# Xharlie/pointnerf

Measured on AMD Instinct MI355X. Metric: rays/sec (render+bwd) NeRF-synth lego 800^2, K=8, 128 samp/ray, higher is better.
Workload: dtype f32 in / out / accumulate; forward GEMM operands as 2 x f16 planes (22-bit) on the f16 MFMA, 3 products per multiply-add; input-gradient GEMMs: f16 leading product + e4m3 cross terms (csrc/mixq.h), 2 product equivalents; weight-gradient GEMM operands as one f16 plane each

## Files before the change

include/pnerf.h:

```cpp
#ifndef PNERF_H
#define PNERF_H
#include <stddef.h>
#include <stdint.h>

#ifdef __cplusplus
extern "C" {
#endif

#define PNERF_E_INVAL   (-1)
#define PNERF_E_WS      (-2)
#define PNERF_E_LAUNCH  (-3)
#define PNERF_E_UNSUP   (-4)

#define PNERF_MAX_K 16

typedef struct pnerf_grid_params {
    float ranges[6];
    float vsize[3];
    int32_t vdim[3];
    int32_t kernel_size[3];
    int32_t query_size[3];
    int32_t P;
    int32_t max_o;
    float radius;
} pnerf_grid_params;

enum { PNERF_GI_N_IN_GRID = 0, PNERF_GI_N_OCC = 1, PNERF_GI_MAX_CNT = 2, PNERF_GI_CELL0 = 3,
       PNERF_GI_FIRST_IDX = 4, PNERF_GI_OSTART_OFF = 5 , PNERF_GI_LEN = 8 };

int pnerf_version(void);
const char *pnerf_arch(void);

size_t pnerf_grid_workspace_bytes(const pnerf_grid_params *gp, int n_points);
int pnerf_grid_build(const pnerf_grid_params *gp, const float *d_xyz, int n_points,
                     void *d_grid_ws, size_t ws_bytes, void *stream);
int pnerf_grid_info(const void *d_grid_ws, int32_t *host_info, void *stream);
int pnerf_points_minmax(const float *d_xyz, int64_t n_points, float *d_out6, void *stream);

size_t pnerf_query_workspace_bytes(int R, int SR);
int pnerf_query(const pnerf_grid_params *gp, const void *d_grid_ws,
                const float *d_raypos,
                const float *campos3_host, const float *d_raydir, const float *d_mid,
                float near_depth, float far_depth, float jitter, uint64_t seed,
                int R, int D, int SR, int K,
                float *d_sample_loc, int32_t *d_sample_pidx, int32_t *d_sample_nn,
                int32_t *d_ray_hit, int32_t *d_valid_list, int32_t *d_counters,
                void *d_query_ws, size_t ws_bytes, void *stream);

int pnerf_gather_rows(const float *d_src, int n_src, int width, const int32_t *d_idx, int64_t n_idx,
                      float *d_dst, void *stream);
int pnerf_scatter_add_rows(const float *d_grad_rows, const int32_t *d_idx, int64_t n_idx, int width,
                           float *d_grad_src, int n_src, void *stream);

int pnerf_zero_one_blocks(int64_t n_idx);
int pnerf_zero_one_forward(const float *d_conf, int n_points, const int32_t *d_idx, int64_t n_idx, float eps,
                           float *d_partial, void *stream);
int pnerf_zero_one_backward(const float *d_conf, int n_points, const int32_t *d_idx, int64_t n_idx, float eps,
                            const float *d_gscale, float *d_grad_conf, void *stream);
int pnerf_zero_one_forward_rays(const float *d_conf, int n_points, const int32_t *d_idx, const int32_t *d_ray_hit, int R, int slots_per_ray, float eps,
                                float *d_partial, void *stream);
int pnerf_zero_one_backward_rays(const float *d_conf, int n_points, const int32_t *d_idx, const int32_t *d_ray_hit, int R, int slots_per_ray, float eps,
                                 const float *d_gscale, float *d_grad_conf, void *stream);
int pnerf_color_loss_blocks(int R);
int pnerf_color_loss_forward_rays(const float *d_ray_color, const float *d_gt, const int32_t *d_ray_hit, int R, float *d_partial, void *stream);
int pnerf_color_loss_backward_rays(const float *d_ray_color, const float *d_gt, const int32_t *d_ray_hit, int R, const float *d_gscale,
                                   float *d_grad_ray_color, void *stream);


#define PNERF_MLP_NTENSORS 18
int pnerf_mlp_layout(int feat_dim, int64_t *offsets );
size_t pnerf_mlp_packed_bytes(void);
int pnerf_mlp_pack(const float *d_params, void *d_packed, void *stream);

typedef struct pnerf_camera {
    float campos[3];
    float camrot[9];
    float rw2c[9];
    float vsize_z;
    int32_t raydist_mode_unit;
    float bg[3];
    int32_t has_bg;
} pnerf_camera;

typedef struct pnerf_points {
    const float *xyz;
    const float *embedding;
    const float *conf;
    const float *dir;
    const float *color;
    int32_t n, feat_dim;
    const float *frames;
} pnerf_points;

typedef struct pnerf_point_grads {
    float *embedding, *conf, *dir, *color;
    void *ready_event;
    const float *zero_one_gscale;
    float zero_one_eps;
    float *xyz;
} pnerf_point_grads;

typedef struct pnerf_step {
    const float *raydir;
    const float *sample_loc;
    const int32_t *sample_pidx;
    const int32_t *sample_nn;
    const int32_t *valid_list;
    const int32_t *counters;
    const float *xyz_pers;
    const float *loc_pers;
    const float *params;
    const void *packed_mlp;
    int32_t R, SR, K;
    int64_t n_valid_max;
} pnerf_step;

size_t pnerf_agg_saved_bytes(int64_t n_valid_samples, int K);
size_t pnerf_agg_workspace_bytes(int64_t n_valid_max, int K);
size_t pnerf_render_backward_workspace_bytes(int R, int SR);

int pnerf_render_forward(const pnerf_camera *cam, const pnerf_points *pts, const pnerf_step *step,
                         float *d_decoded, float *d_weight, float *d_ray_color, float *d_opacity,
                         float *d_bg_trans, float *d_blend_w,
                         void *d_saved, void *d_ws, size_t ws_bytes, void *stream);

size_t pnerf_render_cut_workspace_bytes(int R, int SR);
int pnerf_render_forward_cut(const pnerf_camera *cam, const pnerf_points *pts, const pnerf_step *step, float cutoff, int stage_samples,
                             float *d_decoded, float *d_weight, float *d_ray_color, float *d_opacity, float *d_bg_trans, float *d_blend_w,
                             int32_t *d_cut_counters, void *d_ws, size_t ws_bytes, void *d_cut_ws, size_t cut_ws_bytes, void *stream);
int pnerf_cut_stage(const pnerf_camera *cam, const float *d_sample_loc, const int32_t *d_sample_nn, const int32_t *d_ray_hit,
                    const float *d_decoded, int R, int SR, float cutoff, int stage_samples, int stage,
                    float *d_trans, float *d_depth_max, int32_t *d_alive, int32_t *d_flags, int32_t *d_list, int32_t *d_counters,
                    void *d_ws, size_t ws_bytes, void *stream);

int pnerf_set_inference_products(int n);

int pnerf_set_wgrad_planes(int n);
int pnerf_set_cross_terms(int bits);
int pnerf_set_cross_terms_where(int mask);
int pnerf_get_arithmetic(int32_t out[4]);

int pnerf_render_backward(const pnerf_camera *cam, const pnerf_points *pts, const pnerf_step *step,
                          const float *d_decoded, const float *d_weight, const float *d_grad_ray_color,
                          void *d_saved, float *d_grad_params, const pnerf_point_grads *pg,
                          void *d_ws, size_t ws_bytes, void *stream);


size_t pnerf_compact_workspace_bytes(int64_t n);
int pnerf_touched_flags(const int32_t *d_pidx, int64_t n, int32_t n_points, int32_t *d_flags, void *stream);
int pnerf_compact_valid(const int32_t *d_nn, int64_t n, int32_t *d_list, int32_t *d_counters, void *d_ws, size_t ws_bytes, void *stream);

int pnerf_agg_forward(const pnerf_camera *cam, const pnerf_points *pts, const pnerf_step *step, float *d_decoded, float *d_weight,
                      void *d_saved, void *d_ws, size_t ws_bytes, void *stream);
int pnerf_agg_backward(const pnerf_camera *cam, const pnerf_points *pts, const pnerf_step *step,
                       const float *d_decoded, const float *d_weight, const float *d_grad_decoded,
                       void *d_saved, float *d_grad_params, const pnerf_point_grads *pg, void *d_ws, size_t ws_bytes, void *stream);

int pnerf_raymarch_forward(const float *d_ray_dist, const uint8_t *d_ray_valid, const float *d_features, const float *bg3_host,
                           int R, int SR, float *d_ray_color, float *d_opacity, float *d_acc_trans, float *d_blend_w,
                           float *d_bg_trans, void *stream);
int pnerf_raymarch_backward(const float *d_ray_dist, const uint8_t *d_ray_valid, const float *d_features, const float *bg3_host,
                            int R, int SR, const float *d_grad_ray_color, float *d_grad_features, void *stream);

int pnerf_adam_step(float *d_param, const float *d_grad, float *d_exp_avg, float *d_exp_avg_sq, int64_t n,
                    double lr, double beta1, double beta2, double eps, int64_t step, void *stream);
typedef struct pnerf_adam_tensor {
    float *param; const float *grad; float *exp_avg; float *exp_avg_sq;
    int64_t n; double lr; int64_t step;
} pnerf_adam_tensor;
int pnerf_adam_step_multi(const pnerf_adam_tensor *tensors, int count, double beta1, double beta2, double eps, void *stream);

size_t pnerf_voxel_downsample_workspace_bytes(int64_t n_points, int rx, int ry, int rz);
int pnerf_voxel_downsample(const float *d_xyz, int64_t n_points, const float *space_min3_host, const float *vox_size3_host,
                           int rx, int ry, int rz, float *d_centroid, int32_t *d_grid_idx, int64_t *d_min_idx, int32_t *d_counts,
                           void *d_ws, size_t ws_bytes, void *stream);

#define PNERF_EX2D_MAX_VIEWS 8
#define PNERF_EX2D_MAX_MAPS 32
typedef struct pnerf_view_desc {
    float c2w[16];
    float w2c[16];
    float intrinsic[9];
    int32_t has_w2c;
} pnerf_view_desc;
typedef struct pnerf_map_desc {
    const float *d_map;
    int32_t view;
    int32_t C, H, W;
    int32_t out_col;
    int32_t is_color;
    int32_t first_of_view;
} pnerf_map_desc;
size_t pnerf_extract_2d_workspace_bytes(int64_t n_points, int n_views, int HD, int WD, int depth_occ);
int pnerf_extract_2d(const float *d_cam_xyz, int64_t n_points, const pnerf_view_desc *views, int n_views, const pnerf_map_desc *maps,
                     int n_maps, int HD, int WD, int depth_occ, float tolerate, float *d_feats, int feat_cols, float *d_colors,
                     int color_cols, uint8_t *d_mask, void *d_ws, size_t ws_bytes, void *stream);
int pnerf_point_dirs(const float *d_cam_xyz, int64_t n_points, const float *cam_pos_cam_host, int n_views, const float *rot1_host9,
                     const float *rot2_host9, float *d_dirs, void *stream);

size_t pnerf_image_metrics_workspace_bytes(int H, int W, int win);
int pnerf_image_metrics(const float *d_img, const float *d_gt, int H, int W, int win, double data_range, int quantize8, double *d_out4,
                        void *d_ws, size_t ws_bytes, void *stream);

int pnerf_probe_rays(const pnerf_points *pts, const float *d_opacity, const float *d_weight, const float *d_sample_loc,
                     const int32_t *d_sample_pidx, const int32_t *d_ray_hit, int R, int SR, int K, float *d_max_opacity, float *d_loc3,
                     float *d_far_dist, float *d_avg_color3, float *d_avg_dir3, float *d_avg_conf, float *d_avg_emb32, void *stream);
int pnerf_probe_hole_mask(const int8_t *d_ray_mask, const float *d_max_opacity, const float *d_far_dist, const float *d_raycolor,
                          const float *d_gt, const uint8_t *d_edge, const float *bg3_host, int H, int W, float opacity_thresh,
                          float far_thresh, int32_t *d_flags, void *stream);

int pnerf_ray_geometry(const pnerf_camera *cam, const float *d_sample_loc, const int32_t *d_sample_nn, const int32_t *d_ray_hit,
                       const float *d_opacity, const float *d_blend_w, int R, int SR, float *d_acc, float *d_depth_sum, float *d_depth,
                       float *d_median_depth, int32_t *d_median_slot, void *stream);
int pnerf_geometry_canvas(const int32_t *d_pixel_idx, const int8_t *d_ray_mask, const float *d_depth, const float *d_median_depth,
                          const float *d_acc, int n_rays, int H, int W, float *d_depth_canvas, float *d_median_canvas, float *d_acc_canvas,
                          int32_t *d_flag, void *stream);

int pnerf_debug_mfma_f16(const void *d_a, const void *d_b, float *d_out, void *stream);
int pnerf_debug_mix_gemm(const float *d_w, int K, const float *d_x, void *d_img, float *d_out, void *stream);
int pnerf_debug_mfma_rate(int mode, int iters, float *d_scratch, double *flop_out, void *stream);
int pnerf_debug_uniform(uint64_t seed, uint64_t first, int64_t n, float *d_out, void *stream);
int pnerf_debug_split(const float *d_x, int64_t n, void *d_h, void *d_m, int sat, void *stream);
int pnerf_debug_pe(const float *d_x, int64_t n, int nfreq, float *d_out, void *stream);

int pnerf_prof_enable(int on);
int pnerf_prof_kernel_count(void);
const char *pnerf_prof_kernel_name(int id);
int pnerf_prof_collect(double *total_ms, int64_t *launches);

#ifdef __cplusplus
}
#endif
#endif
```

pointnerf_amd/_lib.py:

```python
import ctypes
import os

import torch

_HERE = os.path.dirname(os.path.abspath(__file__))
LIB_PATH = os.path.join(_HERE, "libpnerf_hip.so")

c_int, c_i64, c_f32, c_void_p, c_size_t = ctypes.c_int, ctypes.c_int64, ctypes.c_float, ctypes.c_void_p, ctypes.c_size_t

ABI_VERSION = 1003
PNERF_MAX_K = 16
GI_N_IN_GRID, GI_N_OCC, GI_MAX_CNT, GI_CELL0, GI_FIRST_IDX, GI_LEN = 0, 1, 2, 3, 4, 8
MLP_NTENSORS = 18

ERRORS = {-1: "PNERF_E_INVAL (bad argument)", -2: "PNERF_E_WS (workspace too small)",
          -3: "PNERF_E_LAUNCH (HIP launch/runtime error)", -4: "PNERF_E_UNSUP (unsupported configuration)"}


class GridParams(ctypes.Structure):
    _fields_ = [("ranges", c_f32 * 6), ("vsize", c_f32 * 3), ("vdim", ctypes.c_int32 * 3),
                ("kernel_size", ctypes.c_int32 * 3), ("query_size", ctypes.c_int32 * 3),
                ("P", ctypes.c_int32), ("max_o", ctypes.c_int32), ("radius", c_f32)]


class Camera(ctypes.Structure):
    _fields_ = [("campos", c_f32 * 3), ("camrot", c_f32 * 9), ("rw2c", c_f32 * 9), ("vsize_z", c_f32),
                ("raydist_mode_unit", ctypes.c_int32), ("bg", c_f32 * 3), ("has_bg", ctypes.c_int32)]


class Points(ctypes.Structure):
    _fields_ = [("xyz", c_void_p), ("embedding", c_void_p), ("conf", c_void_p), ("dir", c_void_p),
                ("color", c_void_p), ("n", ctypes.c_int32), ("feat_dim", ctypes.c_int32), ("frames", c_void_p)]


class AdamTensor(ctypes.Structure):
    _fields_ = [("param", c_void_p), ("grad", c_void_p), ("exp_avg", c_void_p), ("exp_avg_sq", c_void_p),
                ("n", ctypes.c_int64), ("lr", ctypes.c_double), ("step", ctypes.c_int64)]


class ViewDesc(ctypes.Structure):
    _fields_ = [("c2w", c_f32 * 16), ("w2c", c_f32 * 16), ("intrinsic", c_f32 * 9), ("has_w2c", ctypes.c_int32)]


class MapDesc(ctypes.Structure):
    _fields_ = [("d_map", c_void_p), ("view", ctypes.c_int32), ("C", ctypes.c_int32), ("H", ctypes.c_int32), ("W", ctypes.c_int32),
                ("out_col", ctypes.c_int32), ("is_color", ctypes.c_int32), ("first_of_view", ctypes.c_int32)]


class PointGrads(ctypes.Structure):
    _fields_ = [("embedding", c_void_p), ("conf", c_void_p), ("dir", c_void_p), ("color", c_void_p), ("ready_event", c_void_p),
                ("zero_one_gscale", c_void_p), ("zero_one_eps", c_f32), ("xyz", c_void_p)]


class Step(ctypes.Structure):
    _fields_ = [("raydir", c_void_p), ("sample_loc", c_void_p), ("sample_pidx", c_void_p), ("sample_nn", c_void_p), ("valid_list", c_void_p),
                ("counters", c_void_p), ("xyz_pers", c_void_p), ("loc_pers", c_void_p), ("params", c_void_p), ("packed_mlp", c_void_p),
                ("R", ctypes.c_int32), ("SR", ctypes.c_int32), ("K", ctypes.c_int32), ("n_valid_max", ctypes.c_int64)]


_STEP_ARGS = [ctypes.POINTER(Camera), ctypes.POINTER(Points), ctypes.POINTER(Step)]
PROTOTYPES = {
    "pnerf_version": (c_int, []),
    "pnerf_arch": (ctypes.c_char_p, []),
    "pnerf_grid_workspace_bytes": (c_size_t, [ctypes.POINTER(GridParams), c_int]),
    "pnerf_grid_build": (c_int, [ctypes.POINTER(GridParams), c_void_p, c_int, c_void_p, c_size_t, c_void_p]),
    "pnerf_grid_info": (c_int, [c_void_p, ctypes.POINTER(ctypes.c_int32), c_void_p]),
    "pnerf_points_minmax": (c_int, [c_void_p, c_i64, c_void_p, c_void_p]),
    "pnerf_query_workspace_bytes": (c_size_t, [c_int, c_int]),
    "pnerf_query": (c_int, [ctypes.POINTER(GridParams), c_void_p, c_void_p, ctypes.POINTER(c_f32), c_void_p, c_void_p,
                            c_f32, c_f32, c_f32, ctypes.c_uint64, c_int, c_int, c_int, c_int,
                            c_void_p, c_void_p, c_void_p, c_void_p, c_void_p, c_void_p, c_void_p, c_size_t, c_void_p]),
    "pnerf_gather_rows": (c_int, [c_void_p, c_int, c_int, c_void_p, c_i64, c_void_p, c_void_p]),
    "pnerf_scatter_add_rows": (c_int, [c_void_p, c_void_p, c_i64, c_int, c_void_p, c_int, c_void_p]),
    "pnerf_zero_one_blocks": (c_int, [c_i64]),
    "pnerf_zero_one_forward": (c_int, [c_void_p, c_int, c_void_p, c_i64, c_f32, c_void_p, c_void_p]),
    "pnerf_zero_one_backward": (c_int, [c_void_p, c_int, c_void_p, c_i64, c_f32, c_void_p, c_void_p, c_void_p]),
    "pnerf_color_loss_blocks": (c_int, [c_int]),
    "pnerf_color_loss_forward_rays": (c_int, [c_void_p, c_void_p, c_void_p, c_int, c_void_p, c_void_p]),
    "pnerf_color_loss_backward_rays": (c_int, [c_void_p, c_void_p, c_void_p, c_int, c_void_p, c_void_p, c_void_p]),
    "pnerf_zero_one_forward_rays": (c_int, [c_void_p, c_int, c_void_p, c_void_p, c_int, c_int, c_f32, c_void_p, c_void_p]),
    "pnerf_zero_one_backward_rays": (c_int, [c_void_p, c_int, c_void_p, c_void_p, c_int, c_int, c_f32, c_void_p, c_void_p, c_void_p]),
    "pnerf_voxel_downsample_workspace_bytes": (c_size_t, [c_i64, c_int, c_int, c_int]),
    "pnerf_voxel_downsample": (c_int, [c_void_p, c_i64, c_void_p, c_void_p, c_int, c_int, c_int, c_void_p, c_void_p, c_void_p, c_void_p, c_void_p, c_size_t, c_void_p]),
    "pnerf_extract_2d_workspace_bytes": (c_size_t, [c_i64, c_int, c_int, c_int, c_int]),
    "pnerf_extract_2d": (c_int, [c_void_p, c_i64, ctypes.POINTER(ViewDesc), c_int, ctypes.POINTER(MapDesc), c_int, c_int, c_int, c_int, c_f32,
                                 c_void_p, c_int, c_void_p, c_int, c_void_p, c_void_p, c_size_t, c_void_p]),
    "pnerf_point_dirs": (c_int, [c_void_p, c_i64, ctypes.POINTER(c_f32), c_int, ctypes.POINTER(c_f32), ctypes.POINTER(c_f32), c_void_p, c_void_p]),
    "pnerf_adam_step": (c_int, [c_void_p, c_void_p, c_void_p, c_void_p, c_i64, ctypes.c_double, ctypes.c_double, ctypes.c_double, ctypes.c_double, c_i64, c_void_p]),
    "pnerf_adam_step_multi": (c_int, [ctypes.POINTER(AdamTensor), c_int, ctypes.c_double, ctypes.c_double, ctypes.c_double, c_void_p]),
    "pnerf_mlp_layout": (c_int, [c_int, ctypes.POINTER(c_i64)]),
    "pnerf_mlp_packed_bytes": (c_size_t, []),
    "pnerf_mlp_pack": (c_int, [c_void_p, c_void_p, c_void_p]),
    "pnerf_agg_saved_bytes": (c_size_t, [c_i64, c_int]),
    "pnerf_agg_workspace_bytes": (c_size_t, [c_i64, c_int]),
    "pnerf_render_backward_workspace_bytes": (c_size_t, [c_int, c_int]),
    "pnerf_render_forward": (c_int, _STEP_ARGS + [c_void_p, c_void_p, c_void_p, c_void_p, c_void_p, c_void_p, c_void_p, c_void_p, c_size_t, c_void_p]),
    "pnerf_render_cut_workspace_bytes": (c_size_t, [c_int, c_int]),
    "pnerf_render_forward_cut": (c_int, _STEP_ARGS + [c_f32, c_int, c_void_p, c_void_p, c_void_p, c_void_p, c_void_p, c_void_p, c_void_p,
                                                      c_void_p, c_size_t, c_void_p, c_size_t, c_void_p]),
    "pnerf_cut_stage": (c_int, [ctypes.POINTER(Camera), c_void_p, c_void_p, c_void_p, c_void_p, c_int, c_int, c_f32, c_int, c_int,
                                c_void_p, c_void_p, c_void_p, c_void_p, c_void_p, c_void_p, c_void_p, c_size_t, c_void_p]),
    "pnerf_set_inference_products": (c_int, [c_int]),
    "pnerf_set_wgrad_planes": (c_int, [c_int]),
    "pnerf_set_cross_terms": (c_int, [c_int]),
    "pnerf_set_cross_terms_where": (c_int, [c_int]),
    "pnerf_get_arithmetic": (c_int, [ctypes.POINTER(ctypes.c_int32)]),
    "pnerf_compact_workspace_bytes": (c_size_t, [c_i64]),
    "pnerf_touched_flags": (c_int, [c_void_p, c_i64, c_int, c_void_p, c_void_p]),
    "pnerf_compact_valid": (c_int, [c_void_p, c_i64, c_void_p, c_void_p, c_void_p, c_size_t, c_void_p]),
    "pnerf_agg_forward": (c_int, _STEP_ARGS + [c_void_p, c_void_p, c_void_p, c_void_p, c_size_t, c_void_p]),
    "pnerf_agg_backward": (c_int, _STEP_ARGS + [c_void_p, c_void_p, c_void_p, c_void_p, c_void_p, ctypes.POINTER(PointGrads), c_void_p, c_size_t, c_void_p]),
    "pnerf_raymarch_forward": (c_int, [c_void_p, c_void_p, c_void_p, ctypes.POINTER(c_f32), c_int, c_int,
                                       c_void_p, c_void_p, c_void_p, c_void_p, c_void_p, c_void_p]),
    "pnerf_raymarch_backward": (c_int, [c_void_p, c_void_p, c_void_p, ctypes.POINTER(c_f32), c_int, c_int,
                                        c_void_p, c_void_p, c_void_p]),
    "pnerf_image_metrics_workspace_bytes": (c_size_t, [c_int, c_int, c_int]),
    "pnerf_image_metrics": (c_int, [c_void_p, c_void_p, c_int, c_int, c_int, ctypes.c_double, c_int, c_void_p, c_void_p, c_size_t, c_void_p]),
    "pnerf_probe_rays": (c_int, [ctypes.POINTER(Points), c_void_p, c_void_p, c_void_p, c_void_p, c_void_p, c_int, c_int, c_int,
                                 c_void_p, c_void_p, c_void_p, c_void_p, c_void_p, c_void_p, c_void_p, c_void_p]),
    "pnerf_probe_hole_mask": (c_int, [c_void_p, c_void_p, c_void_p, c_void_p, c_void_p, c_void_p, ctypes.POINTER(c_f32), c_int, c_int,
                                      c_f32, c_f32, c_void_p, c_void_p]),
    "pnerf_ray_geometry": (c_int, [ctypes.POINTER(Camera), c_void_p, c_void_p, c_void_p, c_void_p, c_void_p, c_int, c_int,
                                   c_void_p, c_void_p, c_void_p, c_void_p, c_void_p, c_void_p]),
    "pnerf_geometry_canvas": (c_int, [c_void_p, c_void_p, c_void_p, c_void_p, c_void_p, c_int, c_int, c_int,
                                      c_void_p, c_void_p, c_void_p, c_void_p, c_void_p]),
    "pnerf_debug_mfma_f16": (c_int, [c_void_p, c_void_p, c_void_p, c_void_p]),
    "pnerf_debug_mix_gemm": (c_int, [c_void_p, c_int, c_void_p, c_void_p, c_void_p, c_void_p]),
    "pnerf_debug_mfma_rate": (c_int, [c_int, c_int, c_void_p, ctypes.POINTER(ctypes.c_double), c_void_p]),
    "pnerf_debug_uniform": (c_int, [ctypes.c_uint64, ctypes.c_uint64, c_i64, c_void_p, c_void_p]),
    "pnerf_debug_split": (c_int, [c_void_p, c_i64, c_void_p, c_void_p, c_int, c_void_p]),
    "pnerf_debug_pe": (c_int, [c_void_p, c_i64, c_int, c_void_p, c_void_p]),
    "pnerf_prof_enable": (c_int, [c_int]),
    "pnerf_prof_kernel_count": (c_int, []),
    "pnerf_prof_kernel_name": (ctypes.c_char_p, [c_int]),
    "pnerf_prof_collect": (c_int, [ctypes.POINTER(ctypes.c_double), ctypes.POINTER(c_i64)]),
    "pnerf_render_backward": (c_int, _STEP_ARGS + [c_void_p, c_void_p, c_void_p, c_void_p, c_void_p, ctypes.POINTER(PointGrads), c_void_p, c_size_t, c_void_p]),
}

_lib = None


def bind(handle, path):
    for name, (res, args) in PROTOTYPES.items():
        try:
            fn = getattr(handle, name)
        except AttributeError as e:
            raise RuntimeError("pointnerf_amd: %s lacks symbol %s (stale build?)" % (os.path.basename(path), name)) from e
        fn.restype, fn.argtypes = res, args
    got = handle.pnerf_version()
    if got != ABI_VERSION:
        raise RuntimeError("pointnerf_amd: %s reports pnerf_version() %d, this binding is written for %d (stale build?)"
                           % (os.path.basename(path), got, ABI_VERSION))
    return handle


def lib():
    global _lib
    if _lib is None:
        if not os.path.exists(LIB_PATH):
            raise RuntimeError(
                "pointnerf_amd: %s not found. Build it with `python -c 'import __graft_entry__ as g; g.build()'` "
                "(hipcc --offload-arch=gfx950). There is no CPU/PyTorch fallback for this path." % LIB_PATH)
        _lib = bind(ctypes.CDLL(LIB_PATH), LIB_PATH)
    return _lib


def check(rc, what):
    if rc != 0:
        raise RuntimeError("pointnerf_amd: %s failed: %s" % (what, ERRORS.get(rc, rc)))
```

pointnerf_amd/csrc/aggregate.hip:

```cpp
#include "mixq.h"
#include <stdlib.h>

extern "C" int pnerf_mlp_layout(int feat_dim, int64_t *offsets) {
    if (feat_dim != PN_F || !offsets) return PNERF_E_UNSUP;
    const int64_t o[PNERF_MLP_NTENSORS + 1] = {PO_W1, PO_B1, PO_W2, PO_B2, PO_W3, PO_B3, PO_W4, PO_B4, PO_W5, PO_B5,
                                               PO_WC1, PO_BC1, PO_WC2, PO_BC2, PO_WC3, PO_BC3, PO_WC4, PO_BC4, PO_TOTAL};
    for (int i = 0; i <= PNERF_MLP_NTENSORS; ++i) offsets[i] = o[i];
    return 0;
}
extern "C" size_t pnerf_mlp_packed_bytes(void) { return (size_t)PKX_END; }

namespace {
struct PackHDesc { int src, ld, trans, Mreal, Kreal, NCH, MB, dst; };
struct PackHTable { PackHDesc d[15]; };
__global__ __launch_bounds__(256) void k_pack_h(PackHTable t, const float *__restrict__ params, char *__restrict__ packed) {
    const PackHDesc d = t.d[blockIdx.y];
    const int total = d.NCH * d.MB * 64;
    for (int e = blockIdx.x * 256 + threadIdx.x; e < total; e += gridDim.x * 256) {
        const int lane = e & 63, mb = (e >> 6) % d.MB, c = (e >> 6) / d.MB;
        const int m = 32 * mb + (lane & 31), k0 = 16 * c + 8 * (lane >> 5);
        unsigned h[4], lo[4];
#pragma unroll
        for (int j = 0; j < 4; ++j) {
            float v[2];
// ... 105 lines not shown
        {PO_W2, PN_H, 1, PN_H, PN_H, 16, 8, PKH_D2},
        {PO_W1, PN_IN1, 1, 32 * PN_MB_D1, PN_H, 16, PN_MB_D1, PKH_D1},
        {PO_WC1, PN_INC, 0, PN_HC, PN_INC, 18, 4, PKH_FC1},
        {PO_WC2, PN_HC, 0, PN_HC, PN_HC, 8, 4, PKH_FC2},
        {PO_WC3, PN_HC, 0, PN_HC, PN_HC, 8, 4, PKH_FC3},
        {PO_WC3, PN_HC, 1, PN_HC, PN_HC, 8, 4, PKH_DC3},
        {PO_WC2, PN_HC, 1, PN_HC, PN_HC, 8, 4, PKH_DC2},
        {PO_WC1, PN_INC, 1, PN_H, PN_HC, 8, 8, PKH_DC1},
        {PO_W1 + 32 * PN_MB_D1, PN_IN1, 1, PN_IN1 - 32 * PN_MB_D1, PN_H, 16, 2, PKH_D1T},
    }};
    PnProfScope prof(PNK_PACK, (hipStream_t)stream);
    hipLaunchKernelGGL(k_pack_h, dim3(40, 15), dim3(256), 0, (hipStream_t)stream, th, d_params, (char *)d_packed);
    PackMTable tm = {{
        {PO_W1, PN_IN1, 0, PN_H, PN_IN1, 2, 8, PKM_F1},
        {PO_W2, PN_H, 0, PN_H, PN_H, 0, 8, PKM_F2},
        {PO_W3, PN_IN3, 0, PN_H, PN_IN3, 1, 8, PKM_F3},
        {PO_W4, PN_H, 0, PN_H, PN_H, 0, 8, PKM_F4},
        {PO_W4, PN_H, 1, PN_H, PN_H, 0, 8, PKM_D4},
        {PO_W3, PN_IN3, 1, PN_IN3, PN_H, 0, 9, PKM_D3},
        {PO_W2, PN_H, 1, PN_H, PN_H, 0, 8, PKM_D2},
        {PO_W1, PN_IN1, 1, 32 * PN_MB_D1, PN_H, 0, PN_MB_D1, PKM_D1},
        {PO_W1 + 32 * PN_MB_D1, PN_IN1, 1, PN_IN1 - 32 * PN_MB_D1, PN_H, 0, 2, PKM_D1T},
    }};
    hipLaunchKernelGGL(k_pack_mix, dim3(12, 9), dim3(256), 0, (hipStream_t)stream, tm, d_params, (char *)d_packed);
    PN_CHECK_LAUNCH();
    return 0;
}

namespace {
template <int NT>
__global__ __launch_bounds__(256) void k_debug_mix_gemm(const float *__restrict__ x, const char *__restrict__ img, float *__restrict__ out) {
    extern __shared__ __attribute__((aligned(16))) char smem_d[];
    pn_mode_saturate();
    constexpr int K = 256 + 16 * NT;
    char *X = smem_d;
    const int tid = threadIdx.x, lane = tid & 63, wave = __builtin_amdgcn_readfirstlane(tid >> 6);
    for (int e = tid; e < PN_TILE * (K / 4); e += 256) {
        const int row = e / (K / 4), col = 4 * (e % (K / 4));
        const float4 v = *reinterpret_cast<const float4 *>(x + row * K + col);
        if (col < 256) pn_xq_store4(X, row, col, v.x, v.y, v.z, v.w);
        else pn_xt_store4(X, row, col, v.x, v.y, v.z, v.w);
    }
    __syncthreads();
    f32x16 acc[2][2];
    pn_acc_zero(acc);
    pn_gemm_mix<PN_MIX_NS, NT, 8, 2>(X, img, 2 * wave, lane, acc);
#pragma unroll
    for (int fb = 0; fb < 2; ++fb)
#pragma unroll
        for (int rb = 0; rb < 2; ++rb)
#pragma unroll
            for (int g = 0; g < 4; ++g)
#pragma unroll
                for (int i = 0; i < 4; ++i) out[(32 * rb + (lane & 31)) * PN_H + pn_d_feat(2 * wave + fb, g, lane) + i] = acc[fb][rb][4 * g + i];
}
}

extern "C" int pnerf_debug_mix_gemm(const float *d_w, int K, const float *d_x, void *d_img, float *d_out, void *stream) {
    if (!d_w || !d_x || !d_img || !d_out || (K != 256 && K != 272 && K != 288)) return PNERF_E_INVAL;
    hipStream_t s = (hipStream_t)stream;
    const int NT = (K - 256) / 16;
    PackMTable tm = {{{0, K, 0, PN_H, K, NT, 8, 0}}};
    hipLaunchKernelGGL(k_pack_mix, dim3(12, 1), dim3(256), 0, s, tm, d_w, (char *)d_img);
    const void *fn = NT == 0 ? (const void *)k_debug_mix_gemm<0> : NT == 1 ? (const void *)k_debug_mix_gemm<1> : (const void *)k_debug_mix_gemm<2>;
    if (hipFuncSetAttribute(fn, hipFuncAttributeMaxDynamicSharedMemorySize, PN_XBYTES) != hipSuccess) return PNERF_E_LAUNCH;
    if (NT == 0) hipLaunchKernelGGL(k_debug_mix_gemm<0>, dim3(1), dim3(256), PN_XBYTES, s, d_x, (const char *)d_img, d_out);
    else if (NT == 1) hipLaunchKernelGGL(k_debug_mix_gemm<1>, dim3(1), dim3(256), PN_XBYTES, s, d_x, (const char *)d_img, d_out);
    else hipLaunchKernelGGL(k_debug_mix_gemm<2>, dim3(1), dim3(256), PN_XBYTES, s, d_x, (const char *)d_img, d_out);
    PN_CHECK_LAUNCH();
    return 0;
}

namespace {
__global__ __launch_bounds__(64) void k_debug_mfma_f16(const uint4 *__restrict__ a, const uint4 *__restrict__ b, float *__restrict__ d) {
    f32x16 acc;
#pragma unroll
    for (int r = 0; r < 16; ++r) acc[r] = 0.f;
    acc = __builtin_amdgcn_mfma_f32_32x32x16_f16(__builtin_bit_cast(pn_h8, a[threadIdx.x]), __builtin_bit_cast(pn_h8, b[threadIdx.x]), acc, 0, 0, 0);
#pragma unroll
    for (int r = 0; r < 16; ++r) d[threadIdx.x * 16 + r] = acc[r];
}
}
namespace {
__global__ __launch_bounds__(256) void k_debug_split(const float *__restrict__ x, long long n, unsigned *__restrict__ h, unsigned *__restrict__ m, int sat) {
    for (long long i = (long long)blockIdx.x * 256 + threadIdx.x; 2 * i < n; i += (long long)gridDim.x * 256) {
        unsigned hh, mm;
        if (sat) pn_split2_sat(x[2 * i], x[2 * i + 1], hh, mm);
        else pn_split2(x[2 * i], x[2 * i + 1], hh, mm);
        h[i] = hh; m[i] = mm;
    }
}
}
extern "C" int pnerf_debug_split(const float *d_x, int64_t n, void *d_h, void *d_m, int sat, void *stream) {
    if (!d_x || !d_h || !d_m || n < 0 || (n & 1)) return PNERF_E_INVAL;
    if (n == 0) return 0;
    hipLaunchKernelGGL(k_debug_split, dim3(64), dim3(256), 0, (hipStream_t)stream, d_x, (long long)n, (unsigned *)d_h, (unsigned *)d_m, sat);
    PN_CHECK_LAUNCH();
    return 0;
}

namespace {
template <int NF> __global__ __launch_bounds__(256) void k_debug_pe(const float *__restrict__ x, long long n, float *__restrict__ out) {
    for (long long i = (long long)blockIdx.x * 256 + threadIdx.x; i < n; i += (long long)gridDim.x * 256) {
        float s[NF], c[NF];
        pn_pe_octaves<NF>(x[i], s, c);
#pragma unroll
        for (int f = 0; f < NF; ++f) { out[(i * NF + f) * 2] = s[f]; out[(i * NF + f) * 2 + 1] = c[f]; }
    }
}
}
extern "C" int pnerf_debug_pe(const float *d_x, int64_t n, int nfreq, float *d_out, void *stream) {
    if (!d_x || !d_out || n < 0 || nfreq < 1 || nfreq > 5) return PNERF_E_INVAL;
    if (n == 0) return 0;
    hipStream_t s = (hipStream_t)stream;
    switch (nfreq) {
        case 1: hipLaunchKernelGGL(k_debug_pe<1>, dim3(64), dim3(256), 0, s, d_x, (long long)n, d_out); break;
        case 2: hipLaunchKernelGGL(k_debug_pe<2>, dim3(64), dim3(256), 0, s, d_x, (long long)n, d_out); break;
        case 3: hipLaunchKernelGGL(k_debug_pe<3>, dim3(64), dim3(256), 0, s, d_x, (long long)n, d_out); break;
        case 4: hipLaunchKernelGGL(k_debug_pe<4>, dim3(64), dim3(256), 0, s, d_x, (long long)n, d_out); break;
        default: hipLaunchKernelGGL(k_debug_pe<5>, dim3(64), dim3(256), 0, s, d_x, (long long)n, d_out); break;
    }
    PN_CHECK_LAUNCH();
    return 0;
}

extern "C" int pnerf_debug_mfma_f16(const void *d_a, const void *d_b, float *d_out, void *stream) {
    if (!d_a || !d_b || !d_out) return PNERF_E_INVAL;
    hipLaunchKernelGGL(k_debug_mfma_f16, dim3(1), dim3(64), 0, (hipStream_t)stream, (const uint4 *)d_a, (const uint4 *)d_b, d_out);
    PN_CHECK_LAUNCH();
    return 0;
}

size_t pn_saved_walk(void *base, long long n_valid, int K, PnSaved &s) {
    const int TS = pn_tile_samples(K);
    const long long tiles = (n_valid + TS - 1) / TS + 2 * PN_NCLS + 1;
    s.rows = tiles * PN_TILE;
    s.samples = ((tiles * TS + PN_CTILE - 1) / PN_CTILE + 1) * PN_CTILE;
    PnCarver cv(base);
    const size_t rg = (size_t)s.rows / 8, rgc = (size_t)s.samples / 8;
    auto planes = [&](uint4 *&x0, uint4 *&h2, uint4 *&h1, uint4 *&h3, uint4 *&dy1, uint4 *&dy2, uint4 *&dy3, uint4 *&dy4) {
        x0 = cv.take<uint4>(rg * PN_NF1); h2 = cv.take<uint4>(rg * PN_NF1);
        h1 = cv.take<uint4>(rg * PN_H); h3 = cv.take<uint4>(rg * PN_H);
        dy1 = cv.take<uint4>(rg * PN_H); dy2 = cv.take<uint4>(rg * PN_H);
        dy3 = cv.take<uint4>(rg * PN_H); dy4 = cv.take<uint4>(rg * PN_H);
    };
    auto cplanes = [&](uint4 *&xc, uint4 *&c1, uint4 *&c2, uint4 *&dc1, uint4 *&dc2, uint4 *&dc3) {
        xc = cv.take<uint4>(rgc * PN_NF1); c1 = cv.take<uint4>(rgc * PN_HC); c2 = cv.take<uint4>(rgc * PN_HC);
        dc1 = cv.take<uint4>(rgc * PN_HC); dc2 = cv.take<uint4>(rgc * PN_HC); dc3 = cv.take<uint4>(rgc * PN_HC);
    };
    planes(s.x0k, s.h2k, s.h1k, s.h3k, s.dy1k, s.dy2k, s.dy3k, s.dy4k);
    s.h4r = cv.take<uint4>((size_t)s.rows * 32 * 2);
    s.arow = cv.take<float>((size_t)s.rows); s.rmeta = cv.take<int4>((size_t)s.rows);
    s.lmask = cv.take<unsigned>((size_t)tiles * 3 * 512);
    s.gscale = cv.take<unsigned>(4);
    s.fs = cv.take<float>((size_t)s.samples * PN_H); s.dfs = cv.take<float>((size_t)s.samples * PN_H);
    s.c3 = cv.take<float>((size_t)s.samples * PN_HC);
    cplanes(s.xck, s.c1k, s.c2k, s.dc1k, s.dc2k, s.dc3k);
    s.cmask = cv.take<unsigned>((size_t)s.samples / PN_CTILE * 2 * 256);
    s.wg2 = pn_arith().wgrad_planes == 2 ? 1 : 0;
    s.x0m = s.h1m = s.h2m = s.h3m = s.dy1m = s.dy2m = s.dy3m = s.dy4m = nullptr;
    s.xcm = s.c1m = s.c2m = s.dc1m = s.dc2m = s.dc3m = nullptr;
    if (s.wg2) {
        planes(s.x0m, s.h2m, s.h1m, s.h3m, s.dy1m, s.dy2m, s.dy3m, s.dy4m);
        cplanes(s.xcm, s.c1m, s.c2m, s.dc1m, s.dc2m, s.dc3m);
    }
    pn_cls_walk(cv, s);
    return cv.off;
}
void pn_cls_walk(PnCarver &cv, PnSaved &s) {
    s.cls_list = cv.take<int>((size_t)s.samples);
    s.cls_info = cv.take<int>(PN_CI_WORDS);
    s.cls_tmp = cv.take<int>((size_t)2 * s.samples + pn_scan_scratch_ints(s.samples) + 8);
}
size_t pn_saved_bytes(long long n_valid, int K) { PnSaved s; return pn_saved_walk(nullptr, n_valid, K, s); }
PnSaved pn_saved_carve(void *base, long long n_valid, int K) { PnSaved s; pn_saved_walk(base, n_valid, K, s); return s; }

extern "C" size_t pnerf_agg_saved_bytes(int64_t n_valid_samples, int K) {
    if (K <= 0 || K > PNERF_MAX_K || n_valid_samples < 0) return 0;
    return pn_saved_bytes(n_valid_samples, K);
}

namespace {
struct FwdArgs {
    pnerf_camera cam;
    const float *xyz, *emb, *conf, *dir, *color;
    const float *params;
    const float4 *packed;
    const float *raydir, *sample_loc;
    const float *xyz_pers, *loc_pers;
    const int *pidx, *valid_list, *counters;
    const int *cls_list, *cls_info;
    int cls, Kstride;
    int save_x0;
    int R, SR, K, TS;
    long long cap_samples;
    float *decoded, *weight;
    PnSaved sv;
};
struct FwdArgsF : FwdArgs { const float *frames; };
template <bool FRAMES> struct FwdArgsOf { using type = FwdArgs; };
template <> struct FwdArgsOf<true> { using type = FwdArgsF; };

namespace {
struct ClsArgs { const int *valid_list, *counters, *pidx; int K, n, ncls; int kc[PN_NCLS], ts[PN_NCLS]; };

__global__ void k_cls_flags(ClsArgs c, int which, int *__restrict__ flags) {
    const int vs = blockIdx.x * blockDim.x + threadIdx.x;
    if (vs >= c.n) return;
    const int Ns = c.counters[0] < c.n ? c.counters[0] : c.n;
    int f = 0;
    if (vs < Ns) {
        const long long si = c.valid_list[vs];
        int hv = 0;
        for (int k = 0; k < c.K; ++k)
            if (c.pidx[si * c.K + k] >= 0) hv = k + 1;
        int cl = 0;
        for (int j = 1; j < c.ncls; ++j)
            if (hv <= c.kc[j]) cl = j;
        f = cl == which;
    }
    flags[vs] = f;
}

__global__ void k_cls_gather(ClsArgs c, int which, const int *__restrict__ pos, const int *__restrict__ count, int *__restrict__ cls_list,
                             int *__restrict__ info) {
    const int n = *count, base = info[PN_CI_VBASE + which];
    for (int i = blockIdx.x * blockDim.x + threadIdx.x; i < n; i += gridDim.x * blockDim.x) cls_list[base + i] = c.valid_list[pos[i]];
    if (blockIdx.x == 0 && threadIdx.x == 0) {
        const int tiles = (n + c.ts[which] - 1) / c.ts[which], tb = info[PN_CI_TBASE + which];
        info[PN_CI_COUNT + which] = n;
        if (which + 1 < PN_NCLS) { info[PN_CI_VBASE + which + 1] = base + n; info[PN_CI_TBASE + which + 1] = tb + tiles + 1; }
        info[PN_CI_TILES] = tb + tiles + 1;
    }
}

__global__ void k_cls_zero_gaps(PnSaved sv, int ncls, int save_x0) {
    const int c = blockIdx.y;
    if (c >= ncls) return;
    if ((blockIdx.x == 0 && !save_x0) || (blockIdx.x == 8 && save_x0)) return;
    const long long gap = (c + 1 < PN_NCLS ? sv.cls_info[PN_CI_TBASE + c + 1] : sv.cls_info[PN_CI_TILES]) - 1;
    uint4 *arrs[9] = {sv.x0k, sv.h2k, sv.h1k, sv.h3k, sv.dy1k, sv.dy2k, sv.dy3k, sv.dy4k, sv.x0k};
    uint4 *arrm[9] = {sv.x0m, sv.h2m, sv.h1m, sv.h3m, sv.dy1m, sv.dy2m, sv.dy3m, sv.dy4m, nullptr};
    const int which = blockIdx.x;
    const int nf = which == 8 ? 64 : which < 2 ? PN_NF1 : PN_H;
    uint4 *p = arrs[which] + gap * 8 * nf;
    for (int i = threadIdx.x; i < 8 * nf; i += blockDim.x) p[i] = make_uint4(0u, 0u, 0u, 0u);
    if (sv.wg2 && arrm[which]) {
        uint4 *pm = arrm[which] + gap * 8 * nf;
        for (int i = threadIdx.x; i < 8 * nf; i += blockDim.x) pm[i] = make_uint4(0u, 0u, 0u, 0u);
    }
}
}

}

int pn_class_slots(int K, int kc[PN_NCLS]) {
    if (K % 4 == 0) { kc[0] = K; kc[1] = K / 2; kc[2] = K / 4; return 3; }
    kc[0] = K; kc[1] = kc[2] = 0;
    return 1;
}

int pn_classify(const PnSaved &sv, const int32_t *d_valid_list, const int32_t *d_counters, const int32_t *d_pidx, int K, long long n_valid,
                bool train, bool save_x0, hipStream_t s) {
    ClsArgs c;
    c.valid_list = d_valid_list; c.counters = d_counters; c.pidx = d_pidx; c.K = K; c.n = (int)n_valid;
    c.ncls = pn_class_slots(K, c.kc);
    for (int j = 0; j < PN_NCLS; ++j) c.ts[j] = c.kc[j] > 0 ? pn_tile_samples(c.kc[j]) : 1;
    if (hipMemsetAsync(sv.cls_info, 0, PN_CI_WORDS * sizeof(int), s) != hipSuccess) return PNERF_E_LAUNCH;
    if (n_valid <= 0) return 0;
    int *flags = sv.cls_tmp, *pos = flags + n_valid, *cnt = pos + n_valid, *scratch = cnt + 8;
    PnProfScope prof(PNK_COMPACT, s);
    for (int j = 0; j < c.ncls; ++j) {
        hipLaunchKernelGGL(k_cls_flags, dim3(pn_cdiv(n_valid, 256)), dim3(256), 0, s, c, j, flags);
        int rc = pn_compact_gt0_i32(flags, n_valid, pos, cnt, scratch, s);
        if (rc) return rc;
        hipLaunchKernelGGL(k_cls_gather, dim3(256), dim3(256), 0, s, c, j, pos, cnt, sv.cls_list, sv.cls_info);
    }
    if (train) hipLaunchKernelGGL(k_cls_zero_gaps, dim3(9, c.ncls), dim3(256), 0, s, sv, c.ncls, save_x0 ? 1 : 0);
    PN_CHECK_LAUNCH();
    return 0;
}


namespace {

constexpr int FL_EX = PN_XBYTES, FL_W5 = FL_EX + PN_TILE * 8 * 4, FL_ROW = FL_W5 + PN_H * 4, FL_BYTES = FL_ROW + 4 * PN_TILE * 4;
static_assert(2 * FL_BYTES <= 160 * 1024, "two forward workgroups must fit the 160 KB LDS");

struct FGather {
    float4 e0, e1;
    float px, py, pz, lx, ly, lz, cf;
    float ppx, ppy, ppz, lpx, lpy, lpz;
    float dxv, dyv, dzv, cx, cy, cz, rx, ry, rz;
    float fx, fy, fz, gx, gy, gz;
};

__device__ __forceinline__ int f_sample_of(const FwdArgs &a, long long tile, int row, int Ns, unsigned kinv) {
    const int ls = pn_row_div(row, kinv);
    const long long vs = tile * a.TS + ls;
    return (ls < a.TS && vs < Ns) ? a.valid_list[vs] : -1;
}

template <bool PERS, bool FRAMES = false>
__device__ __forceinline__ void f_gather(const FwdArgs &a, FGather &G, int si_, int p_, int q, const float *frames = nullptr) {
    const int p = p_ > 0 ? p_ : 0, si = si_ > 0 ? si_ : 0;
    const float *ep = a.emb + (long long)p * PN_F + PN_EPT * q;
    G.e0 = *reinterpret_cast<const float4 *>(ep); G.e1 = *reinterpret_cast<const float4 *>(ep + 4);
    G.px = a.xyz[3 * p]; G.py = a.xyz[3 * p + 1]; G.pz = a.xyz[3 * p + 2];
    G.lx = a.sample_loc[(long long)si * 3]; G.ly = a.sample_loc[(long long)si * 3 + 1]; G.lz = a.sample_loc[(long long)si * 3 + 2];
    if (PERS) {
        G.ppx = a.xyz_pers[3 * p]; G.ppy = a.xyz_pers[3 * p + 1]; G.ppz = a.xyz_pers[3 * p + 2];
        G.lpx = a.loc_pers[(long long)si * 3]; G.lpy = a.loc_pers[(long long)si * 3 + 1]; G.lpz = a.loc_pers[(long long)si * 3 + 2];
    }
    G.cf = a.conf[p];
    if (FRAMES) {
        const int r = si / a.SR, fr = q < 3 ? q : 2;
        const int ps_ = a.pidx[(long long)si * a.Kstride], ps = ps_ > 0 ? ps_ : 0;
        const float *fp = frames + (long long)p * 9 + 3 * fr, *gp = frames + (long long)ps * 9 + 3 * fr;
        G.fx = fp[0]; G.fy = fp[1]; G.fz = fp[2];
        G.gx = gp[0]; G.gy = gp[1]; G.gz = gp[2];
        G.dxv = a.dir[3 * p]; G.dyv = a.dir[3 * p + 1]; G.dzv = a.dir[3 * p + 2];
        G.rx = a.raydir[3 * r]; G.ry = a.raydir[3 * r + 1]; G.rz = a.raydir[3 * r + 2];
        if (q == 0) { G.cx = a.color[3 * p]; G.cy = a.color[3 * p + 1]; G.cz = a.color[3 * p + 2]; }
    } else if (q == 0) {
        const int r = si / a.SR;
        G.dxv = a.dir[3 * p]; G.dyv = a.dir[3 * p + 1]; G.dzv = a.dir[3 * p + 2];
        G.cx = a.color[3 * p]; G.cy = a.color[3 * p + 1]; G.cz = a.color[3 * p + 2];
        G.rx = a.raydir[3 * r]; G.ry = a.raydir[3 * r + 1]; G.rz = a.raydir[3 * r + 2];
    }
}

template <bool PERS, bool MIX = false, bool FRAMES = false>
__device__ __forceinline__ void f_build(const FwdArgs &a, const FGather &G, char *X, float *exb, float *wraw, int *sidx, int si, int p, int row, int q) {
    const float dwx = G.px - G.lx, dwy = G.py - G.ly, dwz = G.pz - G.lz;
    float ppx, ppy, pcz, spx, spy, scz;
    if (PERS) {
        ppx = G.ppx; ppy = G.ppy; pcz = G.ppz; spx = G.lpx; spy = G.lpy; scz = G.lpz;
    } else {
        float pcx, pcy, scx, scy;
        if (FRAMES) {
            const float *M = a.cam.camrot;
            const float x = G.px - a.cam.campos[0], y = G.py - a.cam.campos[1], z = G.pz - a.cam.campos[2];
            const float u = G.lx - a.cam.campos[0], v = G.ly - a.cam.campos[1], w = G.lz - a.cam.campos[2];
            pcx = __builtin_fmaf(z, M[6], __builtin_fmaf(y, M[3], x * M[0]));
            pcy = __builtin_fmaf(z, M[7], __builtin_fmaf(y, M[4], x * M[1]));
            pcz = __builtin_fmaf(z, M[8], __builtin_fmaf(y, M[5], x * M[2]));
            scx = __builtin_fmaf(w, M[6], __builtin_fmaf(u, M[0], v * M[3]));
            scy = __builtin_fmaf(w, M[7], __builtin_fmaf(u, M[1], v * M[4]));
            scz = __builtin_fmaf(w, M[8], __builtin_fmaf(u, M[2], v * M[5]));
        } else {
        rot3(a.cam.camrot, G.px - a.cam.campos[0], G.py - a.cam.campos[1], G.pz - a.cam.campos[2], false, pcx, pcy, pcz);
        rot3(a.cam.camrot, G.lx - a.cam.campos[0], G.ly - a.cam.campos[1], G.lz - a.cam.campos[2], false, scx, scy, scz);
        }
        ppx = pcx / pcz; ppy = pcy / pcz; spx = scx / scz; spy = scy / scz;
    }
    float d0, d1, d2;
    if (FRAMES) d0 = d1 = d2 = dwx * G.fx + dwy * G.fy + dwz * G.fz;
    else rot3(a.cam.rw2c, dwx, dwy, dwz, true, d0, d1, d2);
    const float d3 = ppx * pcz - spx * scz, d4 = ppy * pcz - spy * scz, d5 = pcz - scz;
    const float da = q == 0 ? d0 : q == 1 ? d1 : q == 2 ? d2 : d3;
    const float db = q == 0 ? d4 : d5;
    const float e[8] = {G.e0.x, G.e0.y, G.e0.z, G.e0.w, G.e1.x, G.e1.y, G.e1.z, G.e1.w};
    if (MIX) {
        pn_xq_store4(X, row, PN_EPT * q, e[0], e[1], e[2], e[3]);
        pn_xq_store4(X, row, PN_EPT * q + 4, e[4], e[5], e[6], e[7]);
#pragma unroll
        for (int i = 0; i < 8; i += 2) {
            const int col = PN_F + (PN_EPT * q + i) * 6;
            float s0[3], c0[3], s1[3], c1[3];
            pn_pe_octaves<3>(e[i], s0, c0);
            pn_pe_octaves<3>(e[i + 1], s1, c1);
            pn_xq_store4(X, row, col, s0[0], c0[0], s0[1], c0[1]);
            pn_xq_store4(X, row, col + 4, s0[2], c0[2], s1[0], c1[0]);
            pn_xq_store4(X, row, col + 8, s1[1], c1[1], s1[2], c1[2]);
        }
    } else {
    pn_xt_store4(X, row, PN_EPT * q, e[0], e[1], e[2], e[3]); pn_xt_store4(X, row, PN_EPT * q + 4, e[4], e[5], e[6], e[7]);
#pragma unroll
    for (int i = 0; i < 8; ++i) {
        const int dd = PN_EPT * q + i;
        float s[3], c[3];
        pn_pe_octaves<3>(e[i], s, c);
        pn_xt_store2(X, row, PN_F + dd * 6, s[0], c[0]);
        pn_xt_store2(X, row, PN_F + dd * 6 + 2, s[1], c[1]);
        pn_xt_store2(X, row, PN_F + dd * 6 + 4, s[2], c[2]);
    }
    }
#pragma unroll
    for (int j = 0; j < 2; ++j) {
        const int comp = q + 4 * j;
        if (comp < 6) {
            float s[5], c[5];
            pn_pe_octaves<5>(j == 0 ? da : db, s, c);
#pragma unroll
            for (int f = 0; f < 5; ++f) {
                if (MIX) pn_xa_store2(X, row, PN_F * 7 + (comp * 5 + f) * 2, s[f], c[f]);
                else pn_xt_store2(X, row, PN_F * 7 + (comp * 5 + f) * 2, s[f], c[f]);
            }
        }
    }
    if (q == 3) pn_xt_store4(X, row, PN_ONES1, 1.f, 0.f, 0.f, 0.f);
    float fvx = 0.f, fvy = 0.f, fvz = 0.f, fqx = 0.f, fqy = 0.f, fqz = 0.f;
    if (FRAMES) {
        fvx = G.rx * G.gx + G.ry * G.gy + G.rz * G.gz;
        fqx = G.dxv * G.fx + G.dyv * G.fy + G.dzv * G.fz;
        fvy = __shfl_down(fvx, 1, 64); fvz = __shfl_down(fvx, 2, 64);
        fqy = __shfl_down(fqx, 1, 64); fqz = __shfl_down(fqx, 2, 64);
    }
    if (q == 0) {
        float vx, vy, vz, qx, qy, qz;
        if (FRAMES) { vx = fvx; vy = fvy; vz = fvz; qx = fqx; qy = fqy; qz = fqz; }
        else {
        rot3(a.cam.rw2c, G.rx, G.ry, G.rz, true, vx, vy, vz);
        rot3(a.cam.rw2c, G.dxv, G.dyv, G.dzv, true, qx, qy, qz);
        }
        float *ex = exb + row * 8;
        *reinterpret_cast<float4 *>(ex) = make_float4(G.cx, G.cy, G.cz, qx - vx);
        if (FRAMES) {
            *reinterpret_cast<float4 *>(ex + 4) = make_float4(qy - vy, qz - vz, __builtin_fmaf(qz, vz, __builtin_fmaf(qx, vx, qy * vy)), 1.f);
            wraw[row] = p >= 0 ? 1.0f / fmaxf(sqrtf(__builtin_fmaf(dwz, dwz, __builtin_fmaf(dwx, dwx, dwy * dwy))), 1e-6f) : 0.f;
        } else {
        *reinterpret_cast<float4 *>(ex + 4) = make_float4(qy - vy, qz - vz, qx * vx + qy * vy + qz * vz, 1.f);
        wraw[row] = p >= 0 ? 1.0f / fmaxf(sqrtf(dwx * dwx + dwy * dwy + dwz * dwz), 1e-6f) : 0.f;
        }
        sidx[row] = si;
    }
}

__device__ __forceinline__ void f_acc_bias(const float *__restrict__ bias, int wave, int lane, f32x16 (&acc)[PN_NFB][2]) {
#pragma unroll
    for (int fb = 0; fb < PN_NFB; ++fb)
#pragma unroll
        for (int g = 0; g < 4; ++g) {
            const float4 b = *reinterpret_cast<const float4 *>(bias + pn_d_feat(PN_NFB * wave + fb, g, lane));
#pragma unroll
            for (int rb = 0; rb < 2; ++rb) { acc[fb][rb][4 * g] = b.x; acc[fb][rb][4 * g + 1] = b.y; acc[fb][rb][4 * g + 2] = b.z; acc[fb][rb][4 * g + 3] = b.w; }
        }
}
template <bool BITS, bool MIX = false, bool HR = false>
__device__ __forceinline__ void f_epilogue(const f32x16 (&acc)[PN_NFB][2], char *X, int wave, int lane, unsigned (&mw)[PN_NFB]) {
#pragma unroll
    for (int fb = 0; fb < PN_NFB; ++fb) mw[fb] = 0u;
#pragma unroll
    for (int fb = 0; fb < PN_NFB; ++fb)
#pragma unroll
        for (int rb = 0; rb < 2; ++rb)
#pragma unroll
            for (int g = 0; g < 4; ++g) {
                const int f0 = pn_d_feat(PN_NFB * wave + fb, g, lane);
                float v[4] = {acc[fb][rb][4 * g], acc[fb][rb][4 * g + 1], acc[fb][rb][4 * g + 2], acc[fb][rb][4 * g + 3]};
                if (BITS) {
#pragma unroll
                    for (int i = 0; i < 4; ++i) mw[fb] = __builtin_amdgcn_alignbit(mw[fb], __float_as_uint(v[i]), 31);
                }
#pragma unroll
                for (int i = 0; i < 4; ++i) v[i] = fmaxf(v[i], 0.01f * v[i]);
                if (MIX) pn_xq_store4(X, 32 * rb + (lane & 31), f0, v[0], v[1], v[2], v[3]);
                else if (HR) pn_xt_store4(X, 32 * rb + (lane & 31), f0, v[0], v[1], v[2], v[3]);
                else pn_x_store4<false>(X, 32 * rb + (lane & 31), f0, v[0], v[1], v[2], v[3]);
            }
}
__device__ __forceinline__ void f_store_masks(unsigned *__restrict__ lmask, long long gtile, int layer, int wave, int lane, const unsigned (&mw)[PN_NFB]) {
#pragma unroll
    for (int fb = 0; fb < PN_NFB; ++fb) lmask[((gtile * 3 + layer) * 8 + PN_NFB * wave + fb) * 64 + lane] = mw[fb];
}

template <int KC, bool TRAIN>
__device__ __forceinline__ void f_tail(const FwdArgs &a, const char *X, const float *w5s, const float *wrow, const int *sidx, float b5,
                                       long long tile, long long gtile, int tid, float *wraw = nullptr) {
    constexpr int NS = KC == 0 ? 1 : 8 / (KC == 0 ? 1 : KC);
    const int lane = tid & 63, cg = tid & 31, r0 = 8 * (tid >> 5);
    const float4 wa = *reinterpret_cast<const float4 *>(w5s + 8 * cg), wb = *reinterpret_cast<const float4 *>(w5s + 8 * cg + 4);
    float pa[8];
    float4 fa[NS], fb[NS];
#pragma unroll
    for (int j = 0; j < NS; ++j) fa[j] = fb[j] = make_float4(0.f, 0.f, 0.f, 0.f);
#pragma unroll
    for (int i = 0; i < 8; ++i) {
        const int r = r0 + i;
        const uint4 h = *reinterpret_cast<const uint4 *>(X + r * PN_XRS + cg * 16);
        const uint4 m = *reinterpret_cast<const uint4 *>(X + PN_XPLANE + r * PN_XRS + cg * 16);
        if (TRAIN) {
            pn_f4 th = {__uint_as_float(h.x), __uint_as_float(h.y), __uint_as_float(h.z), __uint_as_float(h.w)};
            pn_f4 tm = {__uint_as_float(m.x), __uint_as_float(m.y), __uint_as_float(m.z), __uint_as_float(m.w)};
            PN_STREAM_STORE(th, reinterpret_cast<pn_f4 *>(a.sv.h4r + (gtile * PN_TILE + r) * 32 + cg));
            PN_STREAM_STORE(tm, reinterpret_cast<pn_f4 *>(a.sv.h4r + (a.sv.rows + gtile * PN_TILE + r) * 32 + cg));
        }
        float s = 0.f;
        s = pn_fma2_lo(h.x, m.x, wa.x, s); s = pn_fma2_hi(h.x, m.x, wa.y, s); s = pn_fma2_lo(h.y, m.y, wa.z, s); s = pn_fma2_hi(h.y, m.y, wa.w, s);
        s = pn_fma2_lo(h.z, m.z, wb.x, s); s = pn_fma2_hi(h.z, m.z, wb.y, s); s = pn_fma2_lo(h.w, m.w, wb.z, s); s = pn_fma2_hi(h.w, m.w, wb.w, s);
        pa[i] = s;
        if (KC != 0) {
            const float w = wrow[r];
            float4 &f0 = fa[i / (KC == 0 ? 1 : KC)], &f1 = fb[i / (KC == 0 ? 1 : KC)];
            f0.x = pn_fma2_lo(h.x, m.x, w, f0.x); f0.y = pn_fma2_hi(h.x, m.x, w, f0.y); f0.z = pn_fma2_lo(h.y, m.y, w, f0.z); f0.w = pn_fma2_hi(h.y, m.y, w, f0.w);
            f1.x = pn_fma2_lo(h.z, m.z, w, f1.x); f1.y = pn_fma2_hi(h.z, m.z, w, f1.y); f1.z = pn_fma2_lo(h.w, m.w, w, f1.z); f1.w = pn_fma2_hi(h.w, m.w, w, f1.w);
        }
    }
#pragma unroll
    for (int j = 0; j < (KC == 0 ? 0 : NS); ++j) {
        const long long vs = tile * (PN_TILE / (KC == 0 ? 1 : KC)) + (r0 / (KC == 0 ? 1 : KC)) + j;
        if (vs < a.cap_samples) {
            *reinterpret_cast<float4 *>(a.sv.fs + vs * PN_H + 8 * cg) = fa[j];
            *reinterpret_cast<float4 *>(a.sv.fs + vs * PN_H + 8 * cg + 4) = fb[j];
        }
    }
    {
        const bool b4 = lane & 16, b3 = lane & 8, b2 = lane & 4;
#pragma unroll
        for (int j = 0; j < 4; ++j) { const float send = b4 ? pa[j] : pa[j + 4], keep = b4 ? pa[j + 4] : pa[j]; pa[j] = keep + __shfl_xor(send, 16, 64); }
#pragma unroll
        for (int j = 0; j < 2; ++j) { const float send = b3 ? pa[j] : pa[j + 2], keep = b3 ? pa[j + 2] : pa[j]; pa[j] = keep + __shfl_xor(send, 8, 64); }
        { const float send = b2 ? pa[0] : pa[1], keep = b2 ? pa[1] : pa[0]; pa[0] = keep + __shfl_xor(send, 4, 64); }
        pa[0] += __shfl_xor(pa[0], 2, 64);
        pa[0] += __shfl_xor(pa[0], 1, 64);
        const int i = ((lane >> 4) & 1) * 4 + ((lane >> 3) & 1) * 2 + ((lane >> 2) & 1), r = r0 + i;
        const float x = pa[0] + b5 - 1.0f;
        float sg = pn_softplus(x) * wrow[r];
        if (TRAIN && (lane & 3) == 0) a.sv.arow[gtile * PN_TILE + r] = x;
        if (KC == 0) {
            if ((lane & 3) == 0) wraw[r] = sg;
            return;
        }
        if (KC >= 2) sg += __shfl_xor(sg, 4, 64);
        if (KC >= 4) sg += __shfl_xor(sg, 8, 64);
        if (KC >= 8) sg += __shfl_xor(sg, 16, 64);
        if ((lane & 3) == 0 && (i % (KC == 0 ? 1 : KC)) == 0) {
            const int si = sidx[r];
            if (si >= 0) a.decoded[(long long)si * 4] = sg;
        }
    }
}

#ifdef PN_PHASE_TRACE
PN_TR_DECL(pn_trace_fwd);
#endif
template <bool TRAIN, bool PERS, int NP, bool WG2 = false, bool FRAMES = false>
__global__ __launch_bounds__(PN_NTHR, PN_NW / 2) void k_agg_forward(typename FwdArgsOf<FRAMES>::type a) {
    constexpr bool MIX = NP == 4;
    static_assert(!FRAMES || (!TRAIN && NP == 3), "per-point frames: the default inference arithmetic only");
    constexpr bool HR = !MIX;
    constexpr bool HC = TRAIN && !WG2;
    static_assert(!(MIX && WG2), "the two-plane weight-gradient mode keeps f16x3.h's arithmetic everywhere");
    pn_mode_saturate();
    extern __shared__ __attribute__((aligned(16))) char smem_f[];
    char *X = smem_f;
    float *exb = reinterpret_cast<float *>(smem_f + FL_EX), *w5s = reinterpret_cast<float *>(smem_f + FL_W5);
    float *wraw = reinterpret_cast<float *>(smem_f + FL_ROW), *wrow = wraw + PN_TILE, *wnrm = wrow + PN_TILE;
    int *sidx = reinterpret_cast<int *>(wnrm + PN_TILE);
    const float *frames = nullptr;
    if constexpr (FRAMES) frames = a.frames;
    const int tid0 = threadIdx.x;
    const int K = a.K, TS = a.TS;
    const unsigned kinv = pn_kinv(K);
    const int Ns = a.cls_info[PN_CI_COUNT + a.cls];
    const long long vb = a.cls_info[PN_CI_VBASE + a.cls], tb = a.cls_info[PN_CI_TBASE + a.cls];
    a.valid_list = a.cls_list + vb; a.cap_samples = Ns;
    a.sv.fs += vb * PN_H;
    const long long ntiles = ((long long)Ns + TS - 1) / TS;
    const float *P = a.params;
    const char *img = reinterpret_cast<const char *>(a.packed);
    if (tid0 < PN_H) w5s[tid0] = P[PO_W5 + tid0];
    const float b5 = P[PO_B5];
    const long long stride = gridDim.x, tile_first = blockIdx.x, tile_last = ntiles;
    if (tile_first >= tile_last) return;

    long long tile = tile_first;
    int si0, si1, si2, p0, p1;
    FGather G;
    {
        const int row = tid0 / PN_TPR, q = tid0 % PN_TPR, k = row - pn_row_div(row, kinv) * K;
        si0 = f_sample_of(a, tile, row, Ns, kinv); si1 = tile + stride < tile_last ? f_sample_of(a, tile + stride, row, Ns, kinv) : -1;
        si2 = tile + 2 * stride < tile_last ? f_sample_of(a, tile + 2 * stride, row, Ns, kinv) : -1;
        p0 = si0 >= 0 ? a.pidx[(long long)si0 * a.Kstride + k] : -1;
        p1 = si1 >= 0 ? a.pidx[(long long)si1 * a.Kstride + k] : -1;
        f_gather<PERS, FRAMES>(a, G, si0, p0, q, frames);
    }

    f32x16 acc[PN_NFB][2];
    PN_TR_ITER_DECL;
    for (; tile < tile_last; tile += stride) {
        PN_TR_ITER_NEXT;
        int tid = threadIdx.x;
        asm volatile("" : "+v"(tid));
        const int lane = tid & 63, wave = __builtin_amdgcn_readfirstlane(tid >> 6);
        const int row = tid / PN_TPR, q = tid % PN_TPR, k = row - pn_row_div(row, kinv) * K;
        const long long gtile = tb + tile;
        PN_LDS_BARRIER();
        PN_TR(pn_trace_fwd, 0); PN_TR_HWID(pn_trace_fwd);
        f_build<PERS, MIX, FRAMES>(a, G, X, exb, wraw, sidx, si0, p0, row, q);
        f_acc_bias(P + PO_B1, wave, lane, acc);
        PnTileW<MIX, 2, 8, NP> W1;
        W1.prefetch(img, PKH_F1, PKM_F1, PN_NFB * wave, lane);
        PN_LDS_BARRIER();
        if (q == 0) {
            const int ls = pn_row_div(row, kinv);
            float wn = 0.f, w = 0.f;
            if (si0 >= 0) {
                float sum = 0.f;
                for (int kk = 0; kk < K; ++kk) sum += wraw[ls * K + kk];
                wn = wraw[row] / fmaxf(sum, 1e-8f);
                w = wn * fminf(fmaxf(G.cf, 1e-4f), 1.0f);
                a.weight[(long long)si0 * a.Kstride + k] = wn;
            }
            wnrm[row] = wn; wrow[row] = w;
            if (TRAIN) a.sv.rmeta[gtile * PN_TILE + row] = make_int4(si0, si0 >= 0 ? p0 : -1, __float_as_int(wn), __float_as_int(w));
        }
        unsigned mask[PN_NFB];
        PN_TR(pn_trace_fwd, 1);
        PN_TR(pn_trace_fwd, 2);
        W1.run(X, lane, acc);
        if (TRAIN) {
            if (HC) {
                if (a.save_x0) pn_copy_out_kmajor_h<PN_NF1>(X, a.sv.x0k, gtile * 8, tid);
                else pn_copy_out_kmajor_cols64_h<224>(X, a.sv.x0k, gtile * 8, tid);
            } else if (WG2) pn_copy_out_kmajor<PN_NF1, true>(X, a.sv.x0k, gtile * 8, tid, a.sv.x0m);
            else if (a.save_x0) pn_copy_out_kmajor<PN_NF1, false>(X, a.sv.x0k, gtile * 8, tid);
            else pn_copy_out_kmajor_cols64<224>(X, a.sv.x0k, gtile * 8, tid);
        }
        PN_LDS_BARRIER();
        PN_TR(pn_trace_fwd, 3);
        f_epilogue<TRAIN, MIX, HR>(acc, X, wave, lane, mask);
        if (TRAIN) f_store_masks(a.sv.lmask, gtile, 0, wave, lane, mask);
        f_acc_bias(P + PO_B2, wave, lane, acc);
        PnTileW<MIX, 0, 8, NP> W2;
        W2.prefetch(img, PKH_F2, PKM_F2, PN_NFB * wave, lane);
        PN_LDS_BARRIER();
        PN_TR(pn_trace_fwd, 4);
        PN_TR(pn_trace_fwd, 5);
        W2.run(X, lane, acc);
        if (TRAIN) {
            if (HC) pn_copy_out_kmajor_h<PN_H>(X, a.sv.h1k, gtile * 8, tid);
            else pn_copy_out_kmajor<PN_H, WG2>(X, a.sv.h1k, gtile * 8, tid, a.sv.h1m);
        }
        PN_LDS_BARRIER();
        PN_TR(pn_trace_fwd, 6);
        f_epilogue<TRAIN, MIX, HR>(acc, X, wave, lane, mask);
        if (TRAIN) f_store_masks(a.sv.lmask, gtile, 1, wave, lane, mask);
        if (tid < PN_TILE) {
            const float4 u = *reinterpret_cast<const float4 *>(exb + tid * 8), v = *reinterpret_cast<const float4 *>(exb + tid * 8 + 4);
            pn_xt_store4(X, tid, PN_H, u.x, u.y, u.z, u.w);
            pn_xt_store4(X, tid, PN_H + 4, v.x, v.y, v.z, v.w);
            pn_xt_store4(X, tid, PN_H + 8, 0.f, 0.f, 0.f, 0.f);
            pn_xt_store4(X, tid, PN_H + 12, 0.f, 0.f, 0.f, 0.f);
        }
        f_acc_bias(P + PO_B3, wave, lane, acc);
        PnTileW<MIX, 1, 8, NP> W3;
        W3.prefetch(img, PKH_F3, PKM_F3, PN_NFB * wave, lane);
        PN_LDS_BARRIER();
        PN_TR(pn_trace_fwd, 7);
        PN_TR(pn_trace_fwd, 8);
        W3.run(X, lane, acc);
        if (TRAIN) {
            if (HC) pn_copy_out_kmajor_h<PN_NF1>(X, a.sv.h2k, gtile * 8, tid);
            else pn_copy_out_kmajor<PN_NF1, WG2>(X, a.sv.h2k, gtile * 8, tid, a.sv.h2m);
        }
        PN_LDS_BARRIER();
        PN_TR(pn_trace_fwd, 9);
        f_epilogue<TRAIN, MIX, HR>(acc, X, wave, lane, mask);
        if (TRAIN) f_store_masks(a.sv.lmask, gtile, 2, wave, lane, mask);
        f_acc_bias(P + PO_B4, wave, lane, acc);
        PnTileW<MIX, 0, 8, NP> W4;
        W4.prefetch(img, PKH_F4, PKM_F4, PN_NFB * wave, lane);
        PN_LDS_BARRIER();
        PN_TR(pn_trace_fwd, 10);
        PN_TR(pn_trace_fwd, 11);
        W4.run(X, lane, acc);
        if (TRAIN) {
            if (HC) pn_copy_out_kmajor_h<PN_H>(X, a.sv.h3k, gtile * 8, tid);
            else pn_copy_out_kmajor<PN_H, WG2>(X, a.sv.h3k, gtile * 8, tid, a.sv.h3m);
        }
        PN_TR(pn_trace_fwd, 12);
        const int si_next = si1, p_next = p1;
        if (tile + stride < tile_last) f_gather<PERS, FRAMES>(a, G, si1, p1, q, frames);
        const int p2 = si2 >= 0 ? a.pidx[(long long)si2 * a.Kstride + k] : -1;
        const int si3 = tile + 3 * stride < tile_last ? f_sample_of(a, tile + 3 * stride, row, Ns, kinv) : -1;
        PN_LDS_BARRIER();
        PN_TR(pn_trace_fwd, 13);
        f_epilogue<false>(acc, X, wave, lane, mask);
        PN_LDS_BARRIER();
        PN_TR(pn_trace_fwd, 14);
        if (K == 8 || K == 4 || K == 2 || K == 1) {
            if (K == 8) f_tail<8, TRAIN>(a, X, w5s, wrow, sidx, b5, tile, gtile, tid);
            else if (K == 4) f_tail<4, TRAIN>(a, X, w5s, wrow, sidx, b5, tile, gtile, tid);
            else if (K == 2) f_tail<2, TRAIN>(a, X, w5s, wrow, sidx, b5, tile, gtile, tid);
            else f_tail<1, TRAIN>(a, X, w5s, wrow, sidx, b5, tile, gtile, tid);
            PN_TR(pn_trace_fwd, 15);
        } else {
        f_tail<0, TRAIN>(a, X, w5s, wrow, sidx, b5, tile, gtile, tid, wraw);
        PN_LDS_BARRIER();
        PN_TR(pn_trace_fwd, 15);
        for (int e = tid; e < TS * 32; e += PN_NTHR) {
            const int ls = e >> 5, cg = e & 31;
            float4 f0 = make_float4(0.f, 0.f, 0.f, 0.f), f1 = f0;
            for (int kk = 0; kk < K; ++kk) {
                const int r = ls * K + kk;
                const uint4 h = *reinterpret_cast<const uint4 *>(X + r * PN_XRS + cg * 16);
                const uint4 m = *reinterpret_cast<const uint4 *>(X + PN_XPLANE + r * PN_XRS + cg * 16);
                const float w = wrow[r];
                f0.x = pn_fma2_lo(h.x, m.x, w, f0.x); f0.y = pn_fma2_hi(h.x, m.x, w, f0.y); f0.z = pn_fma2_lo(h.y, m.y, w, f0.z); f0.w = pn_fma2_hi(h.y, m.y, w, f0.w);
                f1.x = pn_fma2_lo(h.z, m.z, w, f1.x); f1.y = pn_fma2_hi(h.z, m.z, w, f1.y); f1.z = pn_fma2_lo(h.w, m.w, w, f1.z); f1.w = pn_fma2_hi(h.w, m.w, w, f1.w);
            }
            const long long vs = tile * TS + ls;
            if (vs < a.cap_samples) {
                *reinterpret_cast<float4 *>(a.sv.fs + vs * PN_H + 8 * cg) = f0;
                *reinterpret_cast<float4 *>(a.sv.fs + vs * PN_H + 8 * cg + 4) = f1;
            }
        }
        if (tid < TS) {
            const int si = sidx[tid * K];
            if (si >= 0) {
                float sg = 0.f;
                for (int kk = 0; kk < K; ++kk) sg += wraw[tid * K + kk];
                a.decoded[(long long)si * 4] = sg;
            }
        }
        }
        si0 = si_next; p0 = p_next; si1 = si2; p1 = p2; si2 = si3;
        PN_TR(pn_trace_fwd, 16);
    }
}

constexpr int CL_W4 = PN_XBYTES, CL_BYTES = CL_W4 + 3 * PN_HC * 4;
static_assert(2 * CL_BYTES <= 160 * 1024, "two colour workgroups must fit the 160 KB LDS");

__device__ __forceinline__ void c_load_bias(const float *__restrict__ bias, int wave, int lane, float4 (&b)[4]) {
#pragma unroll
    for (int g = 0; g < 4; ++g) {
        const float *p = bias + pn_d_feat(wave, g, lane);
        b[g] = make_float4(p[0], p[1], p[2], p[3]);
    }
}
template <bool TRAIN, bool SAVE32>
__device__ __forceinline__ unsigned c_epilogue(const f32x16 (&acc)[2][2], const float4 (&bias)[4], char *X, int wave, int lane, float *__restrict__ save, long long grow0) {
    unsigned mw = 0u;
#pragma unroll
    for (int rb = 0; rb < 2; ++rb)
#pragma unroll
        for (int g = 0; g < 4; ++g) {
            const int f0 = pn_d_feat(wave, g, lane), row = 32 * rb + (lane & 31);
            const float4 b = bias[g];
            float v[4] = {acc[0][rb][4 * g] + b.x, acc[0][rb][4 * g + 1] + b.y, acc[0][rb][4 * g + 2] + b.z, acc[0][rb][4 * g + 3] + b.w};
            if (TRAIN && !SAVE32) {
#pragma unroll
                for (int i = 0; i < 4; ++i) mw = __builtin_amdgcn_alignbit(mw, __float_as_uint(v[i]), 31);
            }
#pragma unroll
            for (int i = 0; i < 4; ++i) v[i] = fmaxf(v[i], 0.01f * v[i]);
            if (TRAIN && SAVE32) {
                pn_f4 t = {v[0], v[1], v[2], v[3]};
                PN_REG_STORE(t, reinterpret_cast<pn_f4 *>(save + (grow0 + row) * PN_HC + f0));
            }
            pn_x_store4<false>(X, row, f0, v[0], v[1], v[2], v[3]);
        }
    return mw;
}

template <bool TRAIN, int NP, bool WG2 = false, bool FRAMES = false>
__global__ __launch_bounds__(256, 2) void k_color_forward(typename FwdArgsOf<FRAMES>::type a) {
    extern __shared__ __attribute__((aligned(16))) char smem_c[];
    char *X = smem_c;
    float *w4s = reinterpret_cast<float *>(smem_c + CL_W4);
    const int Ns = a.counters[0] < a.cap_samples ? a.counters[0] : (int)a.cap_samples;
    const float *P = a.params;
    const char *img = reinterpret_cast<const char *>(a.packed);
    for (int i = threadIdx.x; i < 3 * PN_HC; i += 256) w4s[i] = P[PO_WC4 + i];
    const float b40 = P[PO_BC4], b41 = P[PO_BC4 + 1], b42 = P[PO_BC4 + 2];

    f32x16 acc[2][2];
    for (long long tile = blockIdx.x; tile * PN_CTILE < Ns; tile += gridDim.x) {
        int tid = threadIdx.x;
        asm volatile("" : "+v"(tid));
        const int lane = tid & 63, wave = __builtin_amdgcn_readfirstlane(tid >> 6), row = tid >> 2, q = tid & 3;
        const long long grow0 = tile * PN_CTILE, vs = grow0 + row;
        const int si = vs < Ns ? a.valid_list[vs] : -1;
        PnGemmW<18, 4, 1, 7, NP> WC1;
        WC1.prefetch(reinterpret_cast<const uint4 *>(img + PKH_FC1), wave, lane);
        PN_LDS_BARRIER();
        if (si >= 0) {
            const float4 *f = reinterpret_cast<const float4 *>(a.sv.fs + vs * PN_H);
            float4 fv[16];
#pragma unroll
            for (int c = 0; c < 16; ++c) fv[c] = f[4 * c + q];
#pragma unroll
            for (int c = 0; c < 16; ++c) pn_x_store4<false>(X, row, 16 * c + 4 * q, fv[c].x, fv[c].y, fv[c].z, fv[c].w);
            {
                const int r = si / a.SR;
                float v[3], sn[4], cs[4];
                if constexpr (FRAMES) {
                    const int ps_ = a.pidx[(long long)si * a.Kstride], ps = ps_ > 0 ? ps_ : 0;
                    const float *fp = a.frames + (long long)ps * 9;
                    const float fm[9] = {fp[0], fp[1], fp[2], fp[3], fp[4], fp[5], fp[6], fp[7], fp[8]};
                    rot3(fm, a.raydir[3 * r], a.raydir[3 * r + 1], a.raydir[3 * r + 2], true, v[0], v[1], v[2]);
                } else
                rot3(a.cam.rw2c, a.raydir[3 * r], a.raydir[3 * r + 1], a.raydir[3 * r + 2], true, v[0], v[1], v[2]);
                const float vq = q == 0 ? v[0] : (q == 1 ? v[1] : v[2]);
                pn_pe_octaves<4>(vq, sn, cs);
                if (q < 3) {
                    pn_x_store4<false>(X, row, PN_H + 4 * q, sn[0], sn[1], sn[2], sn[3]);
                    pn_x_store4<false>(X, row, PN_H + 12 + 4 * q, cs[0], cs[1], cs[2], cs[3]);
                } else {
                    pn_x_store4<false>(X, row, PN_H + 24, 0.f, 0.f, 0.f, 0.f);
                    pn_x_store4<false>(X, row, PN_H + 28, 0.f, 0.f, 0.f, 0.f);
                }
            }
        } else {
#pragma unroll
            for (int c = 0; c < 18; ++c) pn_x_store4<false>(X, row, 16 * c + 4 * q, 0.f, 0.f, 0.f, 0.f);
        }
        PN_LDS_BARRIER();
        float4 bias[4];
        if (TRAIN) pn_copy_out_kmajor<PN_NF1, WG2>(X, a.sv.xck, tile * 8, tid, a.sv.xcm);
        pn_acc_zero(acc);
        pn_gemm_f16x3_run<18, 4, 1, 7, NP>(X, WC1, lane, acc);
        c_load_bias(P + PO_BC1, wave, lane, bias);
        PN_LDS_BARRIER();
        unsigned mw = c_epilogue<TRAIN, false>(acc, bias, X, wave, lane, nullptr, grow0);
        if (TRAIN) a.sv.cmask[(tile * 2 + 0) * 256 + tid] = mw;
        PnGemmW<8, 4, 1, 7, NP> WC2;
        WC2.prefetch(reinterpret_cast<const uint4 *>(img + PKH_FC2), wave, lane);
        PN_LDS_BARRIER();
        if (TRAIN) pn_copy_out_kmajor<PN_HC, WG2>(X, a.sv.c1k, tile * 8, tid, a.sv.c1m);
        pn_acc_zero(acc);
        pn_gemm_f16x3_run<8, 4, 1, 7, NP>(X, WC2, lane, acc);
        c_load_bias(P + PO_BC2, wave, lane, bias);
        PN_LDS_BARRIER();
        mw = c_epilogue<TRAIN, false>(acc, bias, X, wave, lane, nullptr, grow0);
        if (TRAIN) a.sv.cmask[(tile * 2 + 1) * 256 + tid] = mw;
        PnGemmW<8, 4, 1, 7, NP> WC3;
        WC3.prefetch(reinterpret_cast<const uint4 *>(img + PKH_FC3), wave, lane);
        PN_LDS_BARRIER();
        if (TRAIN) pn_copy_out_kmajor<PN_HC, WG2>(X, a.sv.c2k, tile * 8, tid, a.sv.c2m);
        pn_acc_zero(acc);
        pn_gemm_f16x3_run<8, 4, 1, 7, NP>(X, WC3, lane, acc);
        c_load_bias(P + PO_BC3, wave, lane, bias);
        PN_LDS_BARRIER();
        c_epilogue<TRAIN, true>(acc, bias, X, wave, lane, a.sv.c3, grow0);
        PN_LDS_BARRIER();
        {
            float o0 = 0.f, o1 = 0.f, o2 = 0.f;
#pragma unroll
            for (int j = 0; j < 4; ++j) {
                const int c0 = q * 32 + 8 * j;
                o0 = pn_x_dot8(X, row, c0, *reinterpret_cast<const float4 *>(w4s + c0), *reinterpret_cast<const float4 *>(w4s + c0 + 4), o0);
                o1 = pn_x_dot8(X, row, c0, *reinterpret_cast<const float4 *>(w4s + PN_HC + c0), *reinterpret_cast<const float4 *>(w4s + PN_HC + c0 + 4), o1);
                o2 = pn_x_dot8(X, row, c0, *reinterpret_cast<const float4 *>(w4s + 2 * PN_HC + c0), *reinterpret_cast<const float4 *>(w4s + 2 * PN_HC + c0 + 4), o2);
            }
            o0 = group_sum<4>(o0); o1 = group_sum<4>(o1); o2 = group_sum<4>(o2);
            if (q == 0 && si >= 0) {
                float *o = a.decoded + (long long)si * 4;
                o[1] = 1.0f / (1.0f + expf(-(o0 + b40))) * 1.002f - 0.001f;
                o[2] = 1.0f / (1.0f + expf(-(o1 + b41))) * 1.002f - 0.001f;
                o[3] = 1.0f / (1.0f + expf(-(o2 + b42))) * 1.002f - 0.001f;
            }
        }
    }
}
}

#ifndef PN_MIX_DEFAULT_MASK
#define PN_MIX_DEFAULT_MASK 4
#endif
static PnArith &pn_arith_record() {
    static PnArith a = [] {
        const char *e = getenv("PNERF_MIX_MASK");
        return PnArith{3, 1, 8, e ? atoi(e) & 7 : PN_MIX_DEFAULT_MASK};
    }();
    return a;
}
PnArith pn_arith() { return pn_arith_record(); }
static int pn_arith_set(int PnArith::*field, int v, bool valid) {
    if (!valid) return PNERF_E_INVAL;
    const int old = pn_arith_record().*field;
    pn_arith_record().*field = v;
    return old;
}
extern "C" int pnerf_set_inference_products(int n) { return pn_arith_set(&PnArith::products, n, n == 2 || n == 3); }
extern "C" int pnerf_set_wgrad_planes(int n) { return pn_arith_set(&PnArith::wgrad_planes, n, n == 1 || n == 2); }
extern "C" int pnerf_set_cross_terms(int bits) { return pn_arith_set(&PnArith::cross_terms, bits, bits == 8 || bits == 16); }
extern "C" int pnerf_set_cross_terms_where(int mask) { return pn_arith_set(&PnArith::mix_where, mask, mask >= 0 && mask <= 7); }
extern "C" int pnerf_get_arithmetic(int32_t out[4]) {
    if (!out) return PNERF_E_INVAL;
    const PnArith a = pn_arith();
    out[0] = a.products; out[1] = a.wgrad_planes; out[2] = a.cross_terms; out[3] = a.mix_where;
    return 0;
}

int pn_agg_forward_launch(const pnerf_camera *cam, const pnerf_points *pts, const pnerf_step &st, float *d_decoded, float *d_weight,
                          const PnSaved &sv, bool train, bool save_x0, hipStream_t s) {
    const int K = st.K;
    const long long cap_samples = st.n_valid_max;
    const PnArith ar = pn_arith();
    FwdArgs a;
    const bool wg2 = train && sv.wg2;
    if (wg2) save_x0 = true;
    a.save_x0 = save_x0 ? 1 : 0;
    a.cam = *cam;
    a.xyz = pts->xyz; a.emb = pts->embedding; a.conf = pts->conf; a.dir = pts->dir; a.color = pts->color;
    a.params = st.params; a.packed = (const float4 *)st.packed_mlp;
    a.raydir = st.raydir; a.sample_loc = st.sample_loc; a.xyz_pers = st.xyz_pers; a.loc_pers = st.loc_pers; a.pidx = st.sample_pidx; a.valid_list = st.valid_list; a.counters = st.counters;
    a.R = st.R; a.SR = st.SR; a.K = K; a.TS = pn_tile_samples(K);
    a.cap_samples = cap_samples;
    a.decoded = d_decoded; a.weight = d_weight; a.sv = sv;
    const bool frames = pts->frames != nullptr;
    if (frames && train) return PNERF_E_INVAL;
    const int ncu = pn_cu_count();
    if (!ncu) return PNERF_E_LAUNCH;
    const int grid_c = pn_capped_grid((cap_samples + PN_CTILE - 1) / PN_CTILE, 2LL * ncu);
    const size_t lds_a = FL_BYTES, lds_c = CL_BYTES;
    const bool pers = st.xyz_pers != nullptr;
    const bool np2 = !train && ar.products == 2;
    const bool mix = !wg2 && !np2 && (ar.mix_mask() & (train ? 2 : 1));
    if (frames && (np2 || mix)) return PNERF_E_UNSUP;
    using FwdKernel = void (*)(FwdArgs);
    using FwdKernelF = void (*)(FwdArgsF);
    const FwdKernelF kfnf = pers ? k_agg_forward<false, true, 3, false, true> : k_agg_forward<false, false, 3, false, true>;
    const FwdKernelF cfnf = k_color_forward<false, 3, false, true>;
    const FwdKernel kfn = wg2   ? (pers ? k_agg_forward<true, true, 3, true> : k_agg_forward<true, false, 3, true>)
                        : mix   ? (train ? (pers ? k_agg_forward<true, true, 4> : k_agg_forward<true, false, 4>)
                                         : (pers ? k_agg_forward<false, true, 4> : k_agg_forward<false, false, 4>))
                        : train ? (pers ? k_agg_forward<true, true, 3> : k_agg_forward<true, false, 3>)
                        : np2   ? (pers ? k_agg_forward<false, true, 2> : k_agg_forward<false, false, 2>)
                                : (pers ? k_agg_forward<false, true, 3> : k_agg_forward<false, false, 3>);
    const FwdKernel cfn = wg2 ? k_color_forward<true, 3, true> : train ? k_color_forward<true, 3> : np2 ? k_color_forward<false, 2> : k_color_forward<false, 3>;
    if (hipFuncSetAttribute(frames ? reinterpret_cast<const void *>(kfnf) : reinterpret_cast<const void *>(kfn), hipFuncAttributeMaxDynamicSharedMemorySize, (int)lds_a) != hipSuccess) return PNERF_E_LAUNCH;
    if (hipFuncSetAttribute(frames ? reinterpret_cast<const void *>(cfnf) : reinterpret_cast<const void *>(cfn), hipFuncAttributeMaxDynamicSharedMemorySize, (int)lds_c) != hipSuccess) return PNERF_E_LAUNCH;
    int rc = pn_classify(sv, st.valid_list, st.counters, st.sample_pidx, K, cap_samples, train, save_x0, s);
    if (rc) return rc;
    a.cls_list = sv.cls_list; a.cls_info = sv.cls_info; a.Kstride = K;
    int kc[PN_NCLS];
    const int ncls = pn_class_slots(K, kc);
    {
        PnProfScope prof(PNK_AGG_FWD, s);
        for (int j = 0; j < ncls; ++j) {
            a.cls = j; a.K = kc[j]; a.TS = pn_tile_samples(kc[j]);
            const int grid_a = pn_capped_grid((cap_samples + a.TS - 1) / a.TS, 2LL * ncu);
            if (frames) { FwdArgsF af; static_cast<FwdArgs &>(af) = a; af.frames = pts->frames; hipLaunchKernelGGL(kfnf, dim3(grid_a), dim3(PN_NTHR), lds_a, s, af); }
            else hipLaunchKernelGGL(kfn, dim3(grid_a), dim3(PN_NTHR), lds_a, s, a);
        }
    }
    a.K = K; a.TS = pn_tile_samples(K); a.valid_list = sv.cls_list;
    {
        PnProfScope prof(PNK_COLOR_FWD, s);
        if (frames) { FwdArgsF af; static_cast<FwdArgs &>(af) = a; af.frames = pts->frames; hipLaunchKernelGGL(cfnf, dim3(grid_c), dim3(256), lds_c, s, af); }
        else hipLaunchKernelGGL(cfn, dim3(grid_c), dim3(256), lds_c, s, a);
    }
    PN_CHECK_LAUNCH();
    return 0;
}

#ifdef PN_PHASE_TRACE
extern "C" int pnerf_debug_trace_fwd(void *host, size_t bytes) {
    return hipMemcpyFromSymbol(host, HIP_SYMBOL(pn_trace_fwd), bytes < sizeof(pn_trace_fwd) ? bytes : sizeof(pn_trace_fwd)) == hipSuccess ? 0 : -1;
}
#endif
```

pointnerf_amd/csrc/backward.hip:

```cpp
#include "mixq.h"

namespace {
constexpr int WG_CHUNKS = 256;
constexpr size_t PARTIAL_FLOATS = (size_t)WG_CHUNKS * PN_H * PN_IN1P;

struct BwdArgs {
    pnerf_camera cam;
    const float *params;
    const float4 *packed;
    const float *raydir;
    const int *pidx, *valid_list, *counters;
    const int *cls_list, *cls_info;
    int cls;
    int SR, K, TS;
    long long cap_samples;
    const float *decoded, *weight, *grad_decoded;
    PnSaved sv;
    const float *emb;
    float *gparams;
    float *g_emb, *g_conf, *g_dir, *g_color;
    const float *conf, *zo_gs;
    float zo_eps;
};
struct BwdXArgs : BwdArgs {
// ... 117 lines not shown
}

template <bool WG2>
__global__ __launch_bounds__(256, 3) void k_color_backward(BwdArgs a) {
    extern __shared__ __attribute__((aligned(16))) char smem_cb[];
    char *X = smem_cb;
    float *draw = reinterpret_cast<float *>(smem_cb + CB_DRAW);
    const PnRowScale rs{reinterpret_cast<float *>(smem_cb + CB_RSC)};
    const int Ns = a.counters[0] < a.cap_samples ? a.counters[0] : (int)a.cap_samples;
    const float *P = a.params;
    const char *img = reinterpret_cast<const char *>(a.packed);
    float S, invS;
    pn_scale_from_bits(a.sv.gscale[0], S, invS);
    if (blockIdx.x == 0 && threadIdx.x == 0) a.sv.cls_info[PN_CI_CTILES] = (Ns + PN_CTILE - 1) / PN_CTILE;
    float *gacc = reinterpret_cast<float *>(smem_cb + CB_GACC);
    for (int i = threadIdx.x; i < 4 * CB_GSUMS; i += 256) gacc[i] = 0.f;
    float *gaccw = gacc + (threadIdx.x >> 6) * CB_GSUMS;
    float gb4x = 0.f, gb4y = 0.f, gb4z = 0.f;
    auto row_sample = [&](long long t) -> long long {
        const long long vs = t * PN_CTILE + threadIdx.x;
        return (threadIdx.x < PN_CTILE && vs < Ns) ? (long long)a.valid_list[vs] : -1;
    };
    float po[3] = {0.f, 0.f, 0.f}, pg[3] = {0.f, 0.f, 0.f}, pgs = 0.f;
    auto row_values = [&](long long si) {
        if (si >= 0) {
            const float *o = a.decoded + si * 4, *g = a.grad_decoded + si * 4;
            po[0] = o[1]; po[1] = o[2]; po[2] = o[3]; pgs = g[0]; pg[0] = g[1]; pg[1] = g[2]; pg[2] = g[3];
        }
    };
    long long si_cur = row_sample(blockIdx.x);
    row_values(si_cur);
    float *w4s = reinterpret_cast<float *>(smem_cb + CB_W4);
    for (int i = threadIdx.x; i < 3 * PN_HC; i += 256) w4s[i] = P[PO_WC4 + i];

    f32x16 acc[2][2];
    for (long long tile = blockIdx.x; tile * PN_CTILE < Ns; tile += gridDim.x) {
        int tid = threadIdx.x;
        asm volatile("" : "+v"(tid));
        const int lane = tid & 63, wave = __builtin_amdgcn_readfirstlane(tid >> 6);
        const long long grow0 = tile * PN_CTILE;
        float4 c3v[8];
#pragma unroll
        for (int rr = 0; rr < 8; ++rr) c3v[rr] = *reinterpret_cast<const float4 *>(a.sv.c3 + (grow0 + 8 * (tid >> 5) + rr) * PN_HC + 4 * (tid & 31));
        const unsigned mw2 = a.sv.cmask[(tile * 2 + 1) * 256 + tid], mw1 = a.sv.cmask[(tile * 2 + 0) * 256 + tid];
        PN_LDS_BARRIER();
        if (tid < PN_CTILE) {
            float d0 = 0.f, d1 = 0.f, d2 = 0.f, Si = S, invSi = invS;
            if (si_cur >= 0) {
                pn_sample_scale(make_float4(pgs, pg[0], pg[1], pg[2]), S, invS, Si, invSi);
                const float s0 = (po[0] + 0.001f) / 1.002f, s1 = (po[1] + 0.001f) / 1.002f, s2 = (po[2] + 0.001f) / 1.002f;
                d0 = pg[0] * 1.002f * s0 * (1.f - s0); d1 = pg[1] * 1.002f * s1 * (1.f - s1); d2 = pg[2] * 1.002f * s2 * (1.f - s2);
            }
            *reinterpret_cast<float4 *>(draw + tid * 4) = make_float4(d0, d1, d2, Si);
            rs.set(tid, Si, invSi, S);
            gb4x += d0; gb4y += d1; gb4z += d2;
        }
        const long long si_next = row_sample(tile + gridDim.x);
        PN_LDS_BARRIER();
        {
            const int c4 = tid & 31, rg = tid >> 5;
            float w4[3][4], gw4[3][4], gb3[4] = {0.f, 0.f, 0.f, 0.f};
#pragma unroll
            for (int k = 0; k < 3; ++k) {
                const float4 w = *reinterpret_cast<const float4 *>(w4s + k * PN_HC + 4 * c4);
                w4[k][0] = w.x; w4[k][1] = w.y; w4[k][2] = w.z; w4[k][3] = w.w;
#pragma unroll
                for (int i = 0; i < 4; ++i) gw4[k][i] = 0.f;
            }
#pragma unroll
            for (int rr = 0; rr < 8; ++rr) {
                const int row = 8 * rg + rr;
                const float4 d = *reinterpret_cast<const float4 *>(draw + row * 4);
                const float c[4] = {c3v[rr].x, c3v[rr].y, c3v[rr].z, c3v[rr].w};
                float u[4];
#pragma unroll
                for (int i = 0; i < 4; ++i) {
                    u[i] = (d.x * w4[0][i] + d.y * w4[1][i] + d.z * w4[2][i]) * pn_lrelu_grad(c[i]);
                    gw4[0][i] += d.x * c[i]; gw4[1][i] += d.y * c[i]; gw4[2][i] += d.z * c[i];
                    gb3[i] += u[i];
                }
                pn_x_store4<true, CB_XRS, CB_XPL>(X, row, 4 * c4, u[0] * d.w, u[1] * d.w, u[2] * d.w, u[3] * d.w);
            }
#pragma unroll
            for (int i = 0; i < 4; ++i) {
#pragma unroll
                for (int k = 0; k < 3; ++k) gw4[k][i] += __shfl_xor(gw4[k][i], 32, 64);
                gb3[i] += __shfl_xor(gb3[i], 32, 64);
            }
            if (lane < 32) {
#pragma unroll
                for (int k = 0; k < 3; ++k) cb_add4(gaccw + k * PN_HC + 4 * c4, gw4[k]);
                cb_add4(gaccw + 3 * PN_HC + 4 * c4, gb3);
            }
        }
        PnGemmW<8, 4, 1, 4, 3> WD3;
        WD3.prefetch(reinterpret_cast<const uint4 *>(img + PKH_DC3), wave, lane);
        PN_LDS_BARRIER();
        pn_copy_out_kmajor_hs<PN_HC, CB_XRS>(X, rs, a.sv.dc3k, tile * 8, tid);
        if (WG2) pn_copy_out_kmajor_hs<PN_HC, CB_XRS>(X + CB_XPL, rs, a.sv.dc3m, tile * 8, tid);
        pn_acc_zero(acc);
        pn_gemm_f16x3_run<8, 4, 1, 4, 3, CB_XRS, CB_XPL>(X, WD3, lane, acc);
        row_values(si_next);
        si_cur = si_next;
        PN_LDS_BARRIER();
        cb_epilogue(acc, mw2, X, wave, lane);
        PnGemmW<8, 4, 1, 4, 3> WD2;
        WD2.prefetch(reinterpret_cast<const uint4 *>(img + PKH_DC2), wave, lane);
        PN_LDS_BARRIER();
        cb_bias_sums(X, rs, tid, gaccw + 4 * PN_HC);
        pn_copy_out_kmajor_hs<PN_HC, CB_XRS>(X, rs, a.sv.dc2k, tile * 8, tid);
        if (WG2) pn_copy_out_kmajor_hs<PN_HC, CB_XRS>(X + CB_XPL, rs, a.sv.dc2m, tile * 8, tid);
        pn_acc_zero(acc);
        pn_gemm_f16x3_run<8, 4, 1, 4, 3, CB_XRS, CB_XPL>(X, WD2, lane, acc);
        PN_LDS_BARRIER();
        cb_epilogue(acc, mw1, X, wave, lane);
        PnGemmW<8, 8, 2, 1, 3> WD1;
        WD1.prefetch(reinterpret_cast<const uint4 *>(img + PKH_DC1), 2 * wave, lane);
        PN_LDS_BARRIER();
        cb_bias_sums(X, rs, tid, gaccw + 5 * PN_HC);
        pn_copy_out_kmajor_hs<PN_HC, CB_XRS>(X, rs, a.sv.dc1k, tile * 8, tid);
        if (WG2) pn_copy_out_kmajor_hs<PN_HC, CB_XRS>(X + CB_XPL, rs, a.sv.dc1m, tile * 8, tid);
        pn_acc_zero(acc);
        pn_gemm_f16x3_run<8, 8, 2, 1, 3, CB_XRS, CB_XPL>(X, WD1, lane, acc);
#pragma unroll
        for (int fb = 0; fb < 2; ++fb)
#pragma unroll
            for (int rb = 0; rb < 2; ++rb) {
                const float ri = rs.inv(32 * rb + (lane & 31));
#pragma unroll
                for (int g = 0; g < 4; ++g) {
                    pn_f4 t = {acc[fb][rb][4 * g] * ri, acc[fb][rb][4 * g + 1] * ri, acc[fb][rb][4 * g + 2] * ri, acc[fb][rb][4 * g + 3] * ri};
                    PN_REG_STORE(t, reinterpret_cast<pn_f4 *>(a.sv.dfs + (grow0 + 32 * rb + (lane & 31)) * PN_H + pn_d_feat(2 * wave + fb, g, lane)));
                }
            }
    }
    PN_LDS_BARRIER();
    {
        const int tid = threadIdx.x;
        auto total = [&](int i) { return (gacc[i] + gacc[CB_GSUMS + i]) + (gacc[2 * CB_GSUMS + i] + gacc[3 * CB_GSUMS + i]); };
        for (int i = tid; i < 3 * PN_HC; i += 256) atomicAdd(&a.gparams[PO_WC4 + i], total(i));
        if (tid < PN_HC) {
            atomicAdd(&a.gparams[PO_BC3 + tid], total(3 * PN_HC + tid));
            atomicAdd(&a.gparams[PO_BC2 + tid], total(4 * PN_HC + tid) * invS);
            atomicAdd(&a.gparams[PO_BC1 + tid], total(5 * PN_HC + tid) * invS);
        }
        if (tid < PN_CTILE) {
#pragma unroll
            for (int off = 32; off > 0; off >>= 1) { gb4x += __shfl_xor(gb4x, off, 64); gb4y += __shfl_xor(gb4y, off, 64); gb4z += __shfl_xor(gb4z, off, 64); }
            if (tid == 0) { atomicAdd(&a.gparams[PO_BC4], gb4x); atomicAdd(&a.gparams[PO_BC4 + 1], gb4y); atomicAdd(&a.gparams[PO_BC4 + 2], gb4z); }
        }
    }
}

constexpr int BL_ROW = PN_XBYTES, BL_RSC = BL_ROW + 10 * PN_TILE * 4, BL_W5 = BL_RSC + PN_RSC_BYTES, BL_BYTES = BL_W5 + PN_H * 4;
constexpr int LDDX = 228;
static_assert(2 * BL_BYTES <= 160 * 1024, "two backward workgroups must fit the 160 KB LDS");
static_assert(PN_TILE * LDDX * 4 <= PN_XBYTES, "d X0 tile");
constexpr int LDDX_X = 292, BL_GW = BL_BYTES, BL_BYTES_X = BL_GW + PN_TILE * 4;
static_assert(2 * BL_BYTES_X <= 160 * 1024, "two xyz_grad backward workgroups must fit the 160 KB LDS");
static_assert(PN_TILE * LDDX_X * 4 <= PN_XBYTES, "d X0 tile (xyz_grad)");

template <bool MIX = false>
__device__ __forceinline__ void b_epilogue(const f32x16 (&acc)[PN_NFB][2], const unsigned (&mask)[PN_NFB], char *X, int wave, int lane) {
#pragma unroll
    for (int fb = 0; fb < PN_NFB; ++fb) {
        const unsigned mw = mask[fb];
#pragma unroll
        for (int rb = 0; rb < 2; ++rb)
#pragma unroll
            for (int g = 0; g < 4; ++g) {
                float v[4];
#pragma unroll
                for (int i = 0; i < 4; ++i) {
                    const int e = (rb * 4 + g) * 4 + i;
                    v[i] = acc[fb][rb][4 * g + i] * ((int)(mw << e) < 0 ? 0.01f : 1.f);
                }
                if (MIX) pn_xq_store4(X, 32 * rb + (lane & 31), pn_d_feat(PN_NFB * wave + fb, g, lane), v[0], v[1], v[2], v[3]);
                else pn_x_store4<true>(X, 32 * rb + (lane & 31), pn_d_feat(PN_NFB * wave + fb, g, lane), v[0], v[1], v[2], v[3]);
            }
    }
}

#ifdef PN_EMU
#define PN_WAVE_LDS_SYNC() __syncthreads()
#else
#define PN_WAVE_LDS_SYNC() asm volatile("s_waitcnt lgkmcnt(0)" ::: "memory")
#endif

template <int KC, bool MIX = false, bool XG = false>
__device__ __forceinline__ void b_front(const BwdArgs &a, char *X, const float *w5s, const float *wrow, const float *wnrm, const float *dsg, const float *xrow,
                                        float *draw, const int *sidx, const int *prow, const float4 (&dfr)[4], const float *dfb0, const PnRowScale &rs, int tid,
                                        float (&gw5)[8], float &gb5t, unsigned kinv = 0u, float *gwf = nullptr) {
    const int lane = tid & 63, cg = tid & 31, r0 = 8 * (tid >> 5);
    const int j0 = KC == 0 ? pn_row_div(r0, kinv) : 0;
    float zo_conf = 0.f;
    if (a.zo_gs && (lane & 3) == 0) {
        const int rz = prow[r0 + ((lane >> 4) & 1) * 4 + ((lane >> 3) & 1) * 2 + ((lane >> 2) & 1)];
        if (rz >= 0) zo_conf = a.conf[rz];
    }
    auto df_of = [&](int j, float4 &ga, float4 &gb) {
        if (KC >= 4) { ga = dfr[2 * j]; gb = dfr[2 * j + 1]; }
        else { ga = *reinterpret_cast<const float4 *>(dfb0 + j * PN_H); gb = *reinterpret_cast<const float4 *>(dfb0 + j * PN_H + 4); }
    };
    float pd[8];
#pragma unroll
    for (int i = 0; i < 8; ++i) {
        const int r = r0 + i, j = KC == 0 ? pn_row_div(r, kinv) - j0 : i / (KC == 0 ? 1 : KC);
        const uint4 h = *reinterpret_cast<const uint4 *>(X + r * PN_XRS + cg * 16);
        const uint4 m = *reinterpret_cast<const uint4 *>(X + PN_XPLANE + r * PN_XRS + cg * 16);
        float4 ga, gb;
        df_of(j, ga, gb);
        float s = 0.f;
        s = pn_fma2_lo(h.x, m.x, ga.x, s); s = pn_fma2_hi(h.x, m.x, ga.y, s); s = pn_fma2_lo(h.y, m.y, ga.z, s); s = pn_fma2_hi(h.y, m.y, ga.w, s);
        s = pn_fma2_lo(h.z, m.z, gb.x, s); s = pn_fma2_hi(h.z, m.z, gb.y, s); s = pn_fma2_lo(h.w, m.w, gb.z, s); s = pn_fma2_hi(h.w, m.w, gb.w, s);
        pd[i] = s;
    }
    {
        const bool b4 = lane & 16, b3 = lane & 8, b2 = lane & 4;
#pragma unroll
        for (int j = 0; j < 4; ++j) { const float send = b4 ? pd[j] : pd[j + 4], keep = b4 ? pd[j + 4] : pd[j]; pd[j] = keep + __shfl_xor(send, 16, 64); }
#pragma unroll
        for (int j = 0; j < 2; ++j) { const float send = b3 ? pd[j] : pd[j + 2], keep = b3 ? pd[j + 2] : pd[j]; pd[j] = keep + __shfl_xor(send, 8, 64); }
        { const float send = b2 ? pd[0] : pd[1], keep = b2 ? pd[1] : pd[0]; pd[0] = keep + __shfl_xor(send, 4, 64); }
        pd[0] += __shfl_xor(pd[0], 2, 64);
        pd[0] += __shfl_xor(pd[0], 1, 64);
        const int r = r0 + ((lane >> 4) & 1) * 4 + ((lane >> 3) & 1) * 2 + ((lane >> 2) & 1);
        if ((lane & 3) == 0) {
            float dr = 0.f, gw = 0.f;
            if (sidx[r] >= 0) {
                const float x = xrow[r], dotf = pd[0] * rs.S(r);
                const float alpha = pn_softplus(x), sg = pn_sigmoid(x);
                const int rp = prow[r];
                if (rp >= 0) atomicAdd(&a.g_conf[rp], (dsg[r] * alpha + dotf) * wnrm[r] * rs.inv(r) + (a.zo_gs ? PnZeroOne(zo_conf, a.zo_eps).grad(a.zo_gs[0]) : 0.f));
                if (XG && rp >= 0) gw = dsg[r] * alpha + dotf;
                dr = dsg[r] * wrow[r] * sg;
            }
            draw[r] = dr;
            if (XG) gwf[r] = gw;
        }
    }
    PN_WAVE_LDS_SYNC();
    const float4 wa = *reinterpret_cast<const float4 *>(w5s + 8 * cg), wb = *reinterpret_cast<const float4 *>(w5s + 8 * cg + 4);
    const float w5[8] = {wa.x, wa.y, wa.z, wa.w, wb.x, wb.y, wb.z, wb.w};
    float drsum = 0.f;
#pragma unroll
    for (int i = 0; i < 8; ++i) {
        const int r = r0 + i, j = KC == 0 ? pn_row_div(r, kinv) - j0 : i / (KC == 0 ? 1 : KC);
        const uint4 h = *reinterpret_cast<const uint4 *>(X + r * PN_XRS + cg * 16);
        const uint4 m = *reinterpret_cast<const uint4 *>(X + PN_XPLANE + r * PN_XRS + cg * 16);
        const bool live = sidx[r] >= 0;
        const float dr = draw[r], w = rs.wS(r), drc = dr * rs.to_call(r);
        drsum += drc;
        const float hv[8] = {pn_h_lo(h.x) + pn_h_lo(m.x), pn_h_hi(h.x) + pn_h_hi(m.x), pn_h_lo(h.y) + pn_h_lo(m.y), pn_h_hi(h.y) + pn_h_hi(m.y),
                             pn_h_lo(h.z) + pn_h_lo(m.z), pn_h_hi(h.z) + pn_h_hi(m.z), pn_h_lo(h.w) + pn_h_lo(m.w), pn_h_hi(h.w) + pn_h_hi(m.w)};
        float4 ga, gb;
        df_of(j, ga, gb);
        const float g[8] = {ga.x, ga.y, ga.z, ga.w, gb.x, gb.y, gb.z, gb.w};
        float o[8];
#pragma unroll
        for (int c = 0; c < 8; ++c) {
            o[c] = live ? (w * g[c] + dr * w5[c]) * pn_lrelu_grad(hv[c]) : 0.f;
            gw5[c] += drc * hv[c];
        }
        unsigned oh[4], om[4];
#pragma unroll
        for (int c = 0; c < 4; ++c) pn_split2_sat(o[2 * c], o[2 * c + 1], oh[c], om[c]);
        *reinterpret_cast<uint4 *>(X + r * PN_XRS + cg * 16) = make_uint4(oh[0], oh[1], oh[2], oh[3]);
        if (MIX) *reinterpret_cast<uint4 *>(X + PN_XPLANE + r * PN_XRS + cg * 16) =
                     make_uint4(pn_q8x4(oh[0], oh[1], 1.0f), pn_q8x4(oh[2], oh[3], 1.0f), pn_q8x4(om[0], om[1], PN_MIX_MSC), pn_q8x4(om[2], om[3], PN_MIX_MSC));
        else *reinterpret_cast<uint4 *>(X + PN_XPLANE + r * PN_XRS + cg * 16) = make_uint4(om[0], om[1], om[2], om[3]);
    }
    if (cg == 0) gb5t += drsum;
}

__device__ __forceinline__ void b_xyz_row(const BwdXArgs &a, const float *dxr, const float *gwf, const float *wrow, const float *wnrm, const int *sidx,
                                          int rp, int row, int q, int K, unsigned kinv, float invS) {
    float u[6] = {0.f, 0.f, 0.f, 0.f, 0.f, 0.f}, t = 0.f;
    float dwx = 0.f, dwy = 0.f, dwz = 0.f;
    if (rp >= 0) {
        const long long si = sidx[row];
        const float px = a.xyz[3 * rp], py = a.xyz[3 * rp + 1], pz = a.xyz[3 * rp + 2];
        const float lx = a.sample_loc[si * 3], ly = a.sample_loc[si * 3 + 1], lz = a.sample_loc[si * 3 + 2];
        dwx = px - lx; dwy = py - ly; dwz = pz - lz;
        float pcx, pcy, pcz, scx, scy, scz, d0, d1, d2;
        rot3(a.cam.camrot, px - a.cam.campos[0], py - a.cam.campos[1], pz - a.cam.campos[2], false, pcx, pcy, pcz);
        rot3(a.cam.camrot, lx - a.cam.campos[0], ly - a.cam.campos[1], lz - a.cam.campos[2], false, scx, scy, scz);
        rot3(a.cam.rw2c, dwx, dwy, dwz, true, d0, d1, d2);
        const float d3 = (pcx / pcz) * pcz - (scx / scz) * scz, d4 = (pcy / pcz) * pcz - (scy / scz) * scz, d5 = pcz - scz;
#pragma unroll
        for (int j = 0; j < 2; ++j) {
            const int c = q + 4 * j;
            if (c < 6) {
                float sn[5], cs[5];
                pn_pe_octaves<5>(j == 0 ? (q == 0 ? d0 : q == 1 ? d1 : q == 2 ? d2 : d3) : (q == 0 ? d4 : d5), sn, cs);
                float g = 0.f, fr = 1.f;
#pragma unroll
                for (int f = 0; f < 5; ++f) {
                    const float2 x = *reinterpret_cast<const float2 *>(dxr + PN_F * 7 + (c * 5 + f) * 2);
                    g += fr * (x.x * cs[f] - x.y * sn[f]);
                    fr *= 2.f;
                }
#pragma unroll
                for (int i = 0; i < 6; ++i) u[i] = c == i ? g : u[i];
            }
        }
        const int k0 = pn_row_div(row, kinv) * K;
        for (int k = q; k < K; k += 4) t += gwf[k0 + k] * wrow[k0 + k];
    }
#pragma unroll
    for (int i = 0; i < 6; ++i) u[i] = group_sum<4>(u[i]);
    t = group_sum<4>(t);
    if (rp >= 0 && q < 3) {
        float gx, gy, gz, hx, hy, hz;
        rot3(a.cam.rw2c, u[0], u[1], u[2], false, gx, gy, gz);
        rot3(a.cam.camrot, u[3], u[4], u[5], true, hx, hy, hz);
        const float len = sqrtf(dwx * dwx + dwy * dwy + dwz * dwz);
        const float cw = len >= 1e-6f ? -(gwf[row] * wrow[row] - t * wnrm[row]) / (len * len) : 0.f;
        const float v = q == 0 ? gx + hx + cw * dwx : q == 1 ? gy + hy + cw * dwy : gz + hz + cw * dwz;
        atomicAdd(&a.g_xyz[3 * rp + q], v * invS);
    }
}

#ifdef PN_PHASE_TRACE
PN_TR_DECL(pn_trace_bwd);
#endif
template <bool WG2, bool MIX = false, bool XYZG = false>
__global__ __launch_bounds__(PN_NTHR, PN_NW / 2) void k_agg_backward(typename BwdArgsOf<XYZG>::T a) {
    static_assert(!(MIX && WG2), "the two-plane weight-gradient mode keeps f16x3.h's arithmetic everywhere");
    constexpr int LDX = XYZG ? LDDX_X : LDDX;
    pn_mode_saturate();
    extern __shared__ __attribute__((aligned(16))) char smem_b[];
    char *X = smem_b;
    float *wrow = reinterpret_cast<float *>(smem_b + BL_ROW), *wnrm = wrow + PN_TILE, *draw = wnrm + PN_TILE, *dsg = draw + PN_TILE, *xrow = dsg + PN_TILE;
    const PnRowScale rs{reinterpret_cast<float *>(smem_b + BL_RSC)};
    int *sidx = reinterpret_cast<int *>(xrow + PN_TILE), *prow = sidx + PN_TILE;
    float *rdir = reinterpret_cast<float *>(prow + PN_TILE);
    float *w5s = reinterpret_cast<float *>(smem_b + BL_W5);
    float *dx = reinterpret_cast<float *>(smem_b);
    float *gwf = XYZG ? reinterpret_cast<float *>(smem_b + BL_GW) : nullptr;
    const int tid0 = threadIdx.x;
    const int K = a.K, TS = a.TS;
    const unsigned kinv = pn_kinv(K);
    const int Ns = a.cls_info[PN_CI_COUNT + a.cls];
    const long long vb = a.cls_info[PN_CI_VBASE + a.cls], tb = a.cls_info[PN_CI_TBASE + a.cls];
    a.sv.dfs += vb * PN_H;
    const long long ntiles = ((long long)Ns + TS - 1) / TS;
    const float *P = a.params;
    const char *img = reinterpret_cast<const char *>(a.packed);
    float S, invS;
    pn_scale_from_bits(a.sv.gscale[0], S, invS);
    if (tid0 < PN_H) w5s[tid0] = P[PO_W5 + tid0];
    float gw5[8] = {0.f, 0.f, 0.f, 0.f, 0.f, 0.f, 0.f, 0.f};
    float gb5t = 0.f;
    f32x16 acc[PN_NFB][2];
    const long long stride = gridDim.x, tile_first = blockIdx.x, tile_last = ntiles;
    int4 rm_cur = make_int4(-1, -1, 0, 0);
    float ar_cur = 0.f;
    if (tid0 < PN_TILE && tile_first < tile_last) {
        rm_cur = a.sv.rmeta[(tb + tile_first) * PN_TILE + tid0];
        ar_cur = a.sv.arow[(tb + tile_first) * PN_TILE + tid0];
    }
    PN_TR_ITER_DECL;
    for (long long tile = tile_first; tile < tile_last; tile += stride) {
        PN_TR_ITER_NEXT;
        int tid = threadIdx.x;
        asm volatile("" : "+v"(tid));
        const int lane = tid & 63, wave = __builtin_amdgcn_readfirstlane(tid >> 6);
        const int row = tid / PN_TPR, q = tid % PN_TPR;
        const long long gtile = tb + tile;
        PN_LDS_BARRIER();
        PN_TR(pn_trace_bwd, 0); PN_TR_HWID(pn_trace_bwd);
        unsigned m1[PN_NFB], m2[PN_NFB], m3[PN_NFB];
#pragma unroll
        for (int fb = 0; fb < PN_NFB; ++fb) {
            const long long o = (long long)(PN_NFB * wave + fb) * 64 + lane;
            m1[fb] = a.sv.lmask[(gtile * 3 + 0) * 512 + o]; m2[fb] = a.sv.lmask[(gtile * 3 + 1) * 512 + o]; m3[fb] = a.sv.lmask[(gtile * 3 + 2) * 512 + o];
        }
        float4 gd_v = make_float4(0.f, 0.f, 0.f, 0.f);
        float rdx = 0.f, rdy = 0.f, rdz = 0.f;
        if (tid < PN_TILE && rm_cur.x >= 0) {
            gd_v = *reinterpret_cast<const float4 *>(a.grad_decoded + (long long)rm_cur.x * 4);
            const int r = rm_cur.x / a.SR;
            rdx = a.raydir[3 * r]; rdy = a.raydir[3 * r + 1]; rdz = a.raydir[3 * r + 2];
        }
        pn_f4 h4v[2 * PN_TILE * 32 / PN_NTHR];
#pragma unroll
        for (int i = 0; i < 2 * PN_TILE * 32 / PN_NTHR; ++i) {
            const int e = tid + PN_NTHR * i, plane = e >> 11, r = (e >> 5) & 63, u = e & 31;
            h4v[i] = *reinterpret_cast<const pn_f4 *>(a.sv.h4r + ((long long)plane * a.sv.rows + gtile * PN_TILE + r) * 32 + u);
        }
        int4 rm_nxt = make_int4(-1, -1, 0, 0);
        float ar_nxt = 0.f;
        if (tid < PN_TILE && tile + stride < tile_last) {
            rm_nxt = a.sv.rmeta[(gtile + stride) * PN_TILE + tid];
            ar_nxt = a.sv.arow[(gtile + stride) * PN_TILE + tid];
        }
        __builtin_amdgcn_sched_barrier(0);
        if (tid < PN_TILE) {
            sidx[tid] = rm_cur.x; prow[tid] = rm_cur.y;
            wnrm[tid] = __int_as_float(rm_cur.z); wrow[tid] = __int_as_float(rm_cur.w);
            xrow[tid] = ar_cur;
            float Si, invSi;
            pn_sample_scale(gd_v, S, invS, Si, invSi);
            rs.set(tid, Si, invSi, S, __int_as_float(rm_cur.w));
            dsg[tid] = gd_v.x * Si;
            rdir[tid] = rdx; rdir[PN_TILE + tid] = rdy; rdir[2 * PN_TILE + tid] = rdz;
        }
#pragma unroll
        for (int i = 0; i < 2 * PN_TILE * 32 / PN_NTHR; ++i) {
            const int e = tid + PN_NTHR * i, plane = e >> 11, r = (e >> 5) & 63, u = e & 31;
            *reinterpret_cast<pn_f4 *>(X + plane * PN_XPLANE + r * PN_XRS + u * 16) = h4v[i];
        }
        __builtin_amdgcn_sched_barrier(0);
        float4 dfr[4];
        const float *dfb0 = a.sv.dfs + (tile * TS + pn_row_div(8 * ((tid >> 5) & 7), kinv)) * PN_H + 8 * (tid & 31);
        if (K == 8 || K == 4) {
            dfr[0] = *reinterpret_cast<const float4 *>(dfb0); dfr[1] = *reinterpret_cast<const float4 *>(dfb0 + 4);
            if (K == 4) { dfr[2] = *reinterpret_cast<const float4 *>(dfb0 + PN_H); dfr[3] = *reinterpret_cast<const float4 *>(dfb0 + PN_H + 4); }
        }
        __builtin_amdgcn_sched_barrier(0);
        rm_cur = rm_nxt; ar_cur = ar_nxt;
        PN_LDS_BARRIER();
        PN_TR(pn_trace_bwd, 1);
        const int rp = prow[row];
        float4 e0 = make_float4(0.f, 0.f, 0.f, 0.f), e1 = e0;
        if (rp >= 0) {
            const float *ep = a.emb + (long long)rp * PN_F + PN_EPT * q;
            e0 = *reinterpret_cast<const float4 *>(ep); e1 = *reinterpret_cast<const float4 *>(ep + 4);
        }
        {
            if (K == 8) b_front<8, MIX, XYZG>(a, X, w5s, wrow, wnrm, dsg, xrow, draw, sidx, prow, dfr, dfb0, rs, tid, gw5, gb5t, 0u, gwf);
            else if (K == 4) b_front<4, MIX, XYZG>(a, X, w5s, wrow, wnrm, dsg, xrow, draw, sidx, prow, dfr, dfb0, rs, tid, gw5, gb5t, 0u, gwf);
            else if (K == 2) b_front<2, MIX, XYZG>(a, X, w5s, wrow, wnrm, dsg, xrow, draw, sidx, prow, dfr, dfb0, rs, tid, gw5, gb5t, 0u, gwf);
            else if (K == 1) b_front<1, MIX, XYZG>(a, X, w5s, wrow, wnrm, dsg, xrow, draw, sidx, prow, dfr, dfb0, rs, tid, gw5, gb5t, 0u, gwf);
            else b_front<0, MIX, XYZG>(a, X, w5s, wrow, wnrm, dsg, xrow, draw, sidx, prow, dfr, dfb0, rs, tid, gw5, gb5t, kinv, gwf);
            PN_TR(pn_trace_bwd, 2);
        }
        PnTileW<MIX, 0, 8> W4;
        W4.prefetch(img, PKH_D4, PKM_D4, PN_NFB * wave, lane);
        PN_LDS_BARRIER();
        PN_TR(pn_trace_bwd, 3);
        pn_acc_zero(acc);
        PN_TR(pn_trace_bwd, 4);
        W4.run(X, lane, acc);
        pn_copy_out_kmajor_hs<PN_H>(X, rs, a.sv.dy4k, gtile * 8, tid);
        if (WG2) pn_copy_out_kmajor_hs<PN_H>(X + PN_XPLANE, rs, a.sv.dy4m, gtile * 8, tid);
        PN_LDS_BARRIER();
        PN_TR(pn_trace_bwd, 5);
        b_epilogue<MIX>(acc, m3, X, wave, lane);
        PnTileW<MIX, 0, 9> W3;
        W3.prefetch(img, PKH_D3, PKM_D3, PN_NFB * wave, lane);
        PN_LDS_BARRIER();
        PN_TR(pn_trace_bwd, 6);
        pn_acc_zero(acc);
        PN_TR(pn_trace_bwd, 7);
        if (wave < PN_NW) {
            f32x16 acce[1][2];
            pn_acc_zero(acce);
            if constexpr (MIX) pn_gemm_mix<1, 0, 9, 1>(X, img + PKM_D3, 8, lane, acce, wave);
            else pn_gemm_f16x3<4, 9, 1>(X, reinterpret_cast<const uint4 *>(img + PKH_D3), 8, lane, acce, 4 * wave);
#pragma unroll
            for (int rb = 0; rb < 2; ++rb)
                *reinterpret_cast<float4 *>(X + (wave >> 1) * PN_XPLANE + (32 * rb + (lane & 31)) * PN_XRS + 512 + (wave & 1) * 32 + (lane >> 5) * 16) =
                    make_float4(acce[0][rb][0], acce[0][rb][1], acce[0][rb][2], acce[0][rb][3]);
        }
        W3.run(X, lane, acc);
        pn_copy_out_kmajor_hs<PN_H>(X, rs, a.sv.dy3k, gtile * 8, tid);
        if (WG2) pn_copy_out_kmajor_hs<PN_H>(X + PN_XPLANE, rs, a.sv.dy3m, gtile * 8, tid);
        PN_LDS_BARRIER();
        PN_TR(pn_trace_bwd, 8);
        b_epilogue<MIX>(acc, m2, X, wave, lane);
        PN_LDS_BARRIER();
        if (tid < PN_TILE) {
            const int p = prow[tid];
            float4 u = make_float4(0.f, 0.f, 0.f, 0.f), v = u;
#pragma unroll
            for (int w = 0; w < 4; ++w) {
                const float4 a0 = *reinterpret_cast<const float4 *>(X + (w >> 1) * PN_XPLANE + tid * PN_XRS + 512 + (w & 1) * 32);
                const float4 a1 = *reinterpret_cast<const float4 *>(X + (w >> 1) * PN_XPLANE + tid * PN_XRS + 512 + (w & 1) * 32 + 16);
                u.x += a0.x; u.y += a0.y; u.z += a0.z; u.w += a0.w; v.x += a1.x; v.y += a1.y; v.z += a1.z; v.w += a1.w;
            }
            float vx, vy, vz, gx = 0.f, gy = 0.f, gz = 0.f;
            if (p >= 0) {
                rot3(a.cam.rw2c, rdir[tid], rdir[PN_TILE + tid], rdir[2 * PN_TILE + tid], true, vx, vy, vz);
                rot3(a.cam.rw2c, u.w + v.z * vx, v.x + v.z * vy, v.y + v.z * vz, false, gx, gy, gz);
            }
            float *slot = reinterpret_cast<float *>(X + tid * PN_XRS + 512);
            const float ri = rs.inv(tid);
            *reinterpret_cast<float4 *>(slot) = make_float4(u.x * ri, u.y * ri, u.z * ri, gx * ri);
            *reinterpret_cast<float2 *>(slot + 4) = make_float2(gy * ri, gz * ri);
        }
        PN_WAVE_LDS_SYNC();
        if (tid < PN_TILE) {
#pragma unroll
            for (int j = 0; j < 3; ++j) {
                const int e = 64 * j + tid, r = (e * 21846) >> 16, c = e - 3 * r;
                const int p = prow[r];
                if (p >= 0) {
                    const float *slot = reinterpret_cast<const float *>(X + r * PN_XRS + 512);
                    atomicAdd(&a.g_color[3 * p + c], slot[c]);
                    atomicAdd(&a.g_dir[3 * p + c], slot[3 + c]);
                }
            }
        }
        PnTileW<MIX, 0, 8> W2;
        W2.prefetch(img, PKH_D2, PKM_D2, PN_NFB * wave, lane);
        PN_LDS_BARRIER();
        PN_TR(pn_trace_bwd, 9);
        pn_acc_zero(acc);
        PN_TR(pn_trace_bwd, 10);
        W2.run(X, lane, acc);
        pn_copy_out_kmajor_hs<PN_H>(X, rs, a.sv.dy2k, gtile * 8, tid);
        if (WG2) pn_copy_out_kmajor_hs<PN_H>(X + PN_XPLANE, rs, a.sv.dy2m, gtile * 8, tid);
        PN_LDS_BARRIER();
        PN_TR(pn_trace_bwd, 11);
        b_epilogue<MIX>(acc, m1, X, wave, lane);
        PN_LDS_BARRIER();
        PN_TR(pn_trace_bwd, 12);
        pn_acc_zero(acc);
        PN_TR(pn_trace_bwd, 13);
        [[maybe_unused]] f32x16 acx[1][2];
        [[maybe_unused]] f32x16 (&acc1)[1][2] = *reinterpret_cast<f32x16 (*)[1][2]>(&acc[PN_NFB - 1]);
        if constexpr (MIX) {
            if (wave < 3) pn_gemm_mix<PN_MIX_NS, 0, PN_MB_D1, PN_NFB>(X, img + PKM_D1, 2 * wave, lane, acc);
            else {
                pn_gemm_mix<PN_MIX_NS, 0, PN_MB_D1, 1>(X, img + PKM_D1, 6, lane, acc);
                if constexpr (XYZG) {
                    pn_gemm_mix<PN_MIX_NS, 0, 2, 1>(X, img + PKM_D1T, 0, lane, acc1);
                    pn_acc_zero(acx);
                    pn_gemm_mix<PN_MIX_NS, 0, 2, 1>(X, img + PKM_D1T, 1, lane, acx);
                }
            }
        } else {
            if (wave < 3) pn_gemm_f16x3<16, PN_MB_D1, PN_NFB>(X, reinterpret_cast<const uint4 *>(img + PKH_D1), 2 * wave, lane, acc);
            else {
                pn_gemm_f16x3<16, PN_MB_D1, 1>(X, reinterpret_cast<const uint4 *>(img + PKH_D1), 6, lane, acc);
                if constexpr (XYZG) {
                    pn_gemm_f16x3<16, 2, 1>(X, reinterpret_cast<const uint4 *>(img + PKH_D1T), 0, lane, acc1);
                    pn_acc_zero(acx);
                    pn_gemm_f16x3<16, 2, 1>(X, reinterpret_cast<const uint4 *>(img + PKH_D1T), 1, lane, acx);
                }
            }
        }
        pn_copy_out_kmajor_hs<PN_H>(X, rs, a.sv.dy1k, gtile * 8, tid);
        if (WG2) pn_copy_out_kmajor_hs<PN_H>(X + PN_XPLANE, rs, a.sv.dy1m, gtile * 8, tid);
        PN_LDS_BARRIER();
        PN_TR(pn_trace_bwd, 14);
#pragma unroll
        for (int fb = 0; fb < PN_NFB; ++fb)
            if (PN_NFB * wave + fb < PN_MB_D1) {
#pragma unroll
                for (int rb = 0; rb < 2; ++rb)
#pragma unroll
                    for (int g = 0; g < 4; ++g)
                        *reinterpret_cast<float4 *>(dx + (32 * rb + (lane & 31)) * LDX + pn_d_feat(PN_NFB * wave + fb, g, lane)) =
                            make_float4(acc[fb][rb][4 * g], acc[fb][rb][4 * g + 1], acc[fb][rb][4 * g + 2], acc[fb][rb][4 * g + 3]);
            }
        if constexpr (XYZG) {
            if (wave == 3) {
#pragma unroll
                for (int fb = 0; fb < 2; ++fb)
#pragma unroll
                    for (int rb = 0; rb < 2; ++rb)
#pragma unroll
                        for (int g = 0; g < 4; ++g) {
                            const f32x16 &v = fb == 0 ? acc1[0][rb] : acx[0][rb];
                            *reinterpret_cast<float4 *>(dx + (32 * rb + (lane & 31)) * LDX + pn_d_feat(PN_MB_D1 + fb, g, lane)) =
                                make_float4(v[4 * g], v[4 * g + 1], v[4 * g + 2], v[4 * g + 3]);
                        }
            }
        }
        PN_LDS_BARRIER();
        PN_TR(pn_trace_bwd, 15);
        if (rp >= 0) {
            float *dr_ = dx + row * LDX;
            const float e[8] = {e0.x, e0.y, e0.z, e0.w, e1.x, e1.y, e1.z, e1.w};
            float go[PN_EPT];
            const float ri = rs.inv(row);
#pragma unroll
            for (int i = 0; i < PN_EPT; ++i) {
                const int dd = PN_EPT * q + i;
                float s[3], c[3];
                pn_pe_octaves<3>(e[i], s, c);
                float g = dr_[dd], fr = 1.f;
#pragma unroll
                for (int f = 0; f < 3; ++f) {
                    const float2 t = *reinterpret_cast<const float2 *>(dr_ + PN_F + dd * 6 + 2 * f);
                    g += fr * (t.x * c[f] - t.y * s[f]);
                    fr *= 2.f;
                }
                go[i] = g * ri;
            }
#pragma unroll
            for (int i = 0; i < PN_EPT; i += 4) *reinterpret_cast<float4 *>(dr_ + PN_EPT * q + i) = make_float4(go[i], go[i + 1], go[i + 2], go[i + 3]);
        }
        PN_WAVE_LDS_SYNC();
        const int r0w = (row & ~15) + (lane >> 5), col = lane & 31;
#pragma unroll
        for (int j = 0; j < 8; ++j) {
            const int r = r0w + 2 * j, p = prow[r];
            if (p >= 0) atomicAdd(&a.g_emb[(long long)p * PN_F + col], dx[r * LDX + col]);
        }
        if constexpr (XYZG) b_xyz_row(a, dx + row * LDX, gwf, wrow, wnrm, sidx, rp, row, q, K, kinv, rs.inv(row));
        PN_TR(pn_trace_bwd, 16);
    }
    if (tile_first >= tile_last) return;
    {
        const int cg = tid0 & 31, rs = tid0 >> 5;
        float *red = reinterpret_cast<float *>(smem_b);
        PN_LDS_BARRIER();
        if (tid0 < PN_NTHR) {
#pragma unroll
            for (int c = 0; c < 8; ++c) red[rs * PN_H + 8 * cg + c] = gw5[c];
            if (cg == 0) red[8 * PN_H + rs] = gb5t;
        }
        PN_LDS_BARRIER();
        if (tid0 >= PN_H) return;
        float t = 0.f;
#pragma unroll
        for (int r = 0; r < 8; ++r) t += red[r * PN_H + tid0];
        atomicAdd(&a.gparams[PO_W5 + tid0], t * invS);
        if (tid0 == 0) {
            float b = 0.f;
            for (int r = 0; r < 8; ++r) b += red[8 * PN_H + r];
            atomicAdd(&a.gparams[PO_B5], b * invS);
        }
    }
}

#ifdef PN_EMU
#define PN_WAIT_VMCNT(n) ((void)0)
#else
#define PN_WAIT_VMCNT(n) asm volatile("s_waitcnt vmcnt(%0)" ::"n"(n) : "memory")
#endif
#ifndef PN_WG_AUX
#define PN_WG_AUX 2
#endif
#ifndef PN_WX_AUX
#define PN_WX_AUX 2
#endif
#ifndef PN_WG_RS
#define PN_WG_RS 32
#endif
#ifndef PN_WG_NST
#define PN_WG_NST 4
#endif
#ifndef PN_WGC_RS
#define PN_WGC_RS 32
#endif
template <int N> __device__ __forceinline__ void pn_wait_vm_stages(int stages) {
    if (stages >= 3) PN_WAIT_VMCNT(3 * N);
    else if (stages == 2) PN_WAIT_VMCNT(2 * N);
    else if (stages == 1) PN_WAIT_VMCNT(N);
    else PN_WAIT_VMCNT(0);
}
template <int NFB, int MF, int RS, int NST, bool TWO = false>
__global__ __launch_bounds__(512) void k_wgrad_f16(const uint4 *__restrict__ A, const uint4 *__restrict__ B,
                                                   const int *__restrict__ d_tiles, float *__restrict__ partial,
                                                   const uint4 *__restrict__ Am = nullptr, const uint4 *__restrict__ Bm = nullptr) {
    constexpr int RG = RS / 8;
    constexpr int AU = RG * MF, BU = RG * NFB;
    constexpr int HALF = AU + BU;
    constexpr int STAGE = TWO ? 2 * HALF : HALF;
    constexpr int NI = STAGE / 64, NIW = (NI + 7) / 8;
    static_assert((NST - 2) * NIW <= 63 && NST >= 3 && NST <= 5, "vmcnt is a 6-bit count");
    constexpr int MTW = MF / 64, NTW = NFB >= 256 ? 2 : 1;
    constexpr int NMAIN = 4 * NTW * 32;
    constexpr bool TAIL_B = NFB > NMAIN, TAIL_ONES = !TAIL_B && MF == 256;
    static_assert(STAGE % 64 == 0, "a stage is a whole number of 1 KB wave copies");
    extern __shared__ __attribute__((aligned(16))) uint4 smem_w[];
    const int tid = threadIdx.x, lane = tid & 63, wave = __builtin_amdgcn_readfirstlane(tid >> 6);
    const int wm = wave >> 2, wn = wave & 3;
    const long long stages = (long long)(*d_tiles) * (PN_TILE / RS);
    const int nst = stages > (long long)blockIdx.x ? (int)((stages - blockIdx.x + gridDim.x - 1) / gridDim.x) : 0;
    f32x16 acc[MTW][NTW], acct;
#pragma unroll
    for (int r = 0; r < 16; ++r) {
        acct[r] = 0.f;
#pragma unroll
        for (int i = 0; i < MTW; ++i)
#pragma unroll
            for (int j = 0; j < NTW; ++j) acc[i][j][r] = 0.f;
    }
    auto issue = [&](int s, int buf) {
        const long long rg = (long long)RG * ((long long)blockIdx.x + (long long)gridDim.x * s);
#pragma unroll
        for (int i = 0; i < NIW; ++i) {
            const bool pad = wave + 8 * i >= NI;
            const int j = pad ? 0 : wave + 8 * i, u0 = 64 * j;
            const uint4 *dst = smem_w + (pad ? NST * STAGE : buf * STAGE + u0);
            const uint4 *src;
            if (u0 < AU) src = A + rg * MF + u0;
            else if (u0 < HALF) src = B + rg * NFB + (u0 - AU);
            else if (u0 < HALF + AU) src = Am + rg * MF + (u0 - HALF);
            else src = Bm + rg * NFB + (u0 - HALF - AU);
            __builtin_amdgcn_global_load_lds(src + lane, (__attribute__((address_space(3))) void *)dst, 16, 0, PN_WG_AUX);
        }
    };
    pn_h8 ones = {0, 0, 0, 0, 0, 0, 0, 0};
    if ((lane & 31) == 0) ones = pn_h8{1, 1, 1, 1, 1, 1, 1, 1};
    const bool has_tail = (TAIL_B || TAIL_ONES) && (MF == 256 || wn < 2);
    if (nst > 0) {
#pragma unroll
        for (int i = 0; i < NST - 1; ++i) if (nst > i) issue(i, i);
        for (int s = 0; s < nst; ++s) {
            pn_wait_vm_stages<NIW>(nst - 1 - s < NST - 2 ? nst - 1 - s : NST - 2);
            __builtin_amdgcn_s_barrier();
            if (s + NST - 1 < nst) issue(s + NST - 1, (s + NST - 1) % NST);
            const uint4 *st = smem_w + (s % NST) * STAGE;
#pragma unroll
            for (int kk = 0; kk < RS / 16; ++kk) {
                const uint4 *fa = st + (2 * kk + (lane >> 5)) * MF + (lane & 31);
                const uint4 *fb = st + AU + (2 * kk + (lane >> 5)) * NFB + (lane & 31);
                pn_h8 ah[MTW], bh[NTW], am[TWO ? MTW : 1], bm[TWO ? NTW : 1];
#pragma unroll
                for (int i = 0; i < MTW; ++i) ah[i] = __builtin_bit_cast(pn_h8, fa[(MTW * wm + i) * 32]);
#pragma unroll
                for (int i = 0; i < NTW; ++i) bh[i] = __builtin_bit_cast(pn_h8, fb[(NTW * wn + i) * 32]);
                if (TWO) {
#pragma unroll
                    for (int i = 0; i < MTW; ++i) am[i] = __builtin_bit_cast(pn_h8, fa[HALF + (MTW * wm + i) * 32]);
#pragma unroll
                    for (int i = 0; i < NTW; ++i) bm[i] = __builtin_bit_cast(pn_h8, fb[HALF + (NTW * wn + i) * 32]);
                }
#pragma unroll
                for (int i = 0; i < MTW; ++i)
#pragma unroll
                    for (int j = 0; j < NTW; ++j)
                        acc[i][j] = __builtin_amdgcn_mfma_f32_32x32x16_f16(ah[i], bh[j], acc[i][j], 0, 0, 0);
                if (TWO) {
#pragma unroll
                    for (int i = 0; i < MTW; ++i)
#pragma unroll
                        for (int j = 0; j < NTW; ++j)
                            acc[i][j] = __builtin_amdgcn_mfma_f32_32x32x16_f16(ah[i], bm[j], acc[i][j], 0, 0, 0);
#pragma unroll
                    for (int i = 0; i < MTW; ++i)
#pragma unroll
                        for (int j = 0; j < NTW; ++j)
                            acc[i][j] = __builtin_amdgcn_mfma_f32_32x32x16_f16(am[i], bh[j], acc[i][j], 0, 0, 0);
                }
                if (has_tail) {
                    pn_h8 tah, tam = ah[0];
                    if (MF == 256) tah = wn == 0 ? ah[0] : wn == 1 ? ah[1] : wn == 2 ? ah[MTW > 2 ? 2 : 0] : ah[MTW > 3 ? 3 : 0];
                    else tah = wn == 0 ? ah[0] : ah[MTW > 1 ? 1 : 0];
                    if (TWO) {
                        if (MF == 256) tam = wn == 0 ? am[0] : wn == 1 ? am[TWO && MTW > 1 ? 1 : 0] : wn == 2 ? am[TWO && MTW > 2 ? 2 : 0] : am[TWO && MTW > 3 ? 3 : 0];
                        else tam = wn == 0 ? am[0] : am[TWO && MTW > 1 ? 1 : 0];
                    }
                    if (TAIL_B) {
                        acct = __builtin_amdgcn_mfma_f32_32x32x16_f16(tah, __builtin_bit_cast(pn_h8, fb[NMAIN]), acct, 0, 0, 0);
                        if (TWO) {
                            acct = __builtin_amdgcn_mfma_f32_32x32x16_f16(tah, __builtin_bit_cast(pn_h8, fb[HALF + NMAIN]), acct, 0, 0, 0);
                            acct = __builtin_amdgcn_mfma_f32_32x32x16_f16(tam, __builtin_bit_cast(pn_h8, fb[NMAIN]), acct, 0, 0, 0);
                        }
                    } else {
                        acct = __builtin_amdgcn_mfma_f32_32x32x16_f16(tah, ones, acct, 0, 0, 0);
// ... 175 lines not shown
            const float e = __builtin_amdgcn_fmed3f(*reinterpret_cast<const float *>(slot + rg * 1024 + ((d >> 2) * 8 + rlow) * 16 + (d & 3) * 4), -65504.f, 65504.f);
            float sn[3], cs[3];
            pn_pe_octaves<3>(e, sn, cs);
            const int f = PN_F + d * 6;
            wx_store_h16(buf, rg, d, rlow, (_Float16)e);
#pragma unroll
            for (int o = 0; o < 3; ++o) { wx_store_h16(buf, rg, f + 2 * o, rlow, (_Float16)sn[o]); wx_store_h16(buf, rg, f + 2 * o + 1, rlow, (_Float16)cs[o]); }
        }
    };
    auto build = [&](int s) {
        build_into(lds + (size_t)(WX_OFF_B + (s & 1) * WX_BU) * 16, lds + (size_t)(WX_OFF_G + (s % WX_G_SLOTS) * WX_GU) * 16);
    };
    if (nst > 0) {
        if (wave == 0)
            for (int s = 0; s < WX_RM_SLOTS; ++s) issue_second(s, 0);
        PN_WAIT_VMCNT(0);
        __syncthreads();
        for (int s = 0; s < WX_D; ++s) issue_a(s);
        if (wave >= 1 && wave <= WX_RG)
            for (int s = 0; s < WX_GD; ++s) { next_point(s); issue_second(0, s); }
        PN_WAIT_VMCNT(0);
        __syncthreads();
        if (wave == 0)
            for (int s = WX_RM_SLOTS; s < WX_RMD; ++s) issue_second(s, 0);
        PN_WAIT_VMCNT(0);
        __syncthreads();
        build(0);
        next_point(WX_GD);
        const long long stride_a = (long long)WX_RG * gridDim.x * MF, stride_t = (long long)WX_RG * gridDim.x * 64, stride_rm = (long long)WX_RG * gridDim.x * 8;
        const uint4 *pa = A + stage_rg(WX_D) * MF + 64 * wave + lane;
        const uint4 *pt = g.x0t + (stage_rg(WX_D) + wave) * 64 + lane;
        const int4 *prm = g.rmeta + stage_rg(WX_RMD) * 8 + (lane & (WX_RS - 1));
        int ia = WX_D % WX_NST, ig = WX_GD % WX_G_SLOTS, irm = WX_RMD % WX_RM_SLOTS;
        int ra = 0, rgs = 1 % WX_G_SLOTS, rrm = (1 + WX_GD) % WX_RM_SLOTS;
        const int n_main = nst - WX_RMD > 0 ? nst - WX_RMD : 0;
        auto bump = [](int &c, int n) { c = c + 1 == n ? 0 : c + 1; };
        for (int s = 0; s < nst; ++s) {
            PN_WAIT_VMCNT(WX_L * (WX_D - 1));
            PN_LDS_BARRIER();
            if (s < n_main) {
#pragma unroll
                for (int i = 0; i < WX_NA; ++i)
                    __builtin_amdgcn_global_load_lds(pa + 512 * i, (__attribute__((address_space(3))) void *)(smem_x + ia * WX_AU + 64 * (wave + 8 * i)), 16, 0, PN_WX_AUX);
                if (wave < WX_RG) __builtin_amdgcn_global_load_lds(pt, (__attribute__((address_space(3))) void *)(smem_x + WX_OFF_T + ia * WX_TU + wave * 64), 16, 0, PN_WX_AUX);
                else __builtin_amdgcn_global_load_lds(A + lane, (__attribute__((address_space(3))) void *)(smem_x + WX_OFF_PAD), 16, 0, 0);
                if (wave == 0) {
                    if (lane < WX_RS) __builtin_amdgcn_global_load_lds(prm, (__attribute__((address_space(3))) void *)(smem_x + WX_OFF_RM + irm * WX_RS), 16, 0, 0);
                } else if (wave <= WX_RG) {
                    __builtin_amdgcn_global_load_lds(g.emb + (long long)p_gather * PN_F + (lane >> 3) * 4,
                                                     (__attribute__((address_space(3))) void *)(smem_x + WX_OFF_G + ig * WX_GU + (wave - 1) * 64), 16, 0, 0);
                } else {
                    __builtin_amdgcn_global_load_lds(A + lane, (__attribute__((address_space(3))) void *)(smem_x + WX_OFF_PAD), 16, 0, 0);
                }
            } else {
                issue_a(s + WX_D);
                issue_second(s + WX_RMD, s + WX_GD);
            }
            pa += stride_a; pt += stride_t; prm += stride_rm;
#pragma unroll
            for (int kk = 0; kk < WX_RS / 16; ++kk) {
                const uint4 *fa = smem_x + ra * WX_AU + (2 * kk + (lane >> 5)) * MF + (lane & 31);
                const uint4 *fb = smem_x + WX_OFF_B + (s & 1) * WX_BU + (2 * kk + (lane >> 5)) * WX_NB + (lane & 31);
                const uint4 *ft = smem_x + WX_OFF_T + ra * WX_TU + (2 * kk + (lane >> 5)) * 64 + (lane & 31);
                pn_h8 ah[MTW], bh[2];
#pragma unroll
                for (int i = 0; i < MTW; ++i) ah[i] = __builtin_bit_cast(pn_h8, fa[(MTW * wm + i) * 32]);
                const pn_h8 tah = __builtin_bit_cast(pn_h8, fa[(MTW * wm + wn) * 32]);
                bh[0] = __builtin_bit_cast(pn_h8, fb[(2 * wn) * 32]);
                bh[1] = __builtin_bit_cast(pn_h8, wn < 3 ? fb[(2 * wn + 1) * 32] : ft[0]);
#pragma unroll
                for (int i = 0; i < MTW; ++i)
#pragma unroll
                    for (int j = 0; j < 2; ++j)
                        acc[i][j] = __builtin_amdgcn_mfma_f32_32x32x16_f16(ah[i], bh[j], acc[i][j], 0, 0, 0);
                acct = __builtin_amdgcn_mfma_f32_32x32x16_f16(tah, __builtin_bit_cast(pn_h8, ft[32]), acct, 0, 0, 0);
            }
            build_into(lds + (size_t)(WX_OFF_B + ((s + 1) & 1) * WX_BU) * 16, lds + (size_t)(WX_OFF_G + rgs * WX_GU) * 16);
            if (wave >= 1 && wave <= WX_RG && s + 1 + WX_GD < nst) {
                const int p = reinterpret_cast<const int4 *>(smem_x + WX_OFF_RM + rrm * WX_RS)[8 * (wave - 1) + (lane & 7)].y;
                p_gather = p < 0 ? 0 : (p >= g.n_points ? g.n_points - 1 : p);
            }
            bump(ia, WX_NST); bump(ig, WX_G_SLOTS); bump(irm, WX_RM_SLOTS); bump(ra, WX_NST); bump(rgs, WX_G_SLOTS); bump(rrm, WX_RM_SLOTS);
        }
    }
    float *out = partial + (size_t)blockIdx.x * 256 * 288;
#pragma unroll
    for (int i = 0; i < MTW; ++i)
#pragma unroll
        for (int j = 0; j < 2; ++j)
#pragma unroll
            for (int r = 0; r < 16; ++r) {
                const int m = (MTW * wm + i) * 32 + (r & 3) + 8 * (r >> 2) + 4 * (lane >> 5);
                out[(size_t)m * 288 + (2 * wn + j) * 32 + (lane & 31)] = acc[i][j][r];
            }
#pragma unroll
    for (int r = 0; r < 16; ++r) {
        const int m = (MTW * wm + wn) * 32 + (r & 3) + 8 * (r >> 2) + 4 * (lane >> 5);
        out[(size_t)m * 288 + 256 + (lane & 31)] = acct[r];
    }
}

int launch_wgrad_x0(const uint4 *A, const WgX0Args &g, const int *d_tiles, long long rows_max, float *partial, const unsigned *gscale,
                    float *grad, hipStream_t s) {
    int chunks = WG_CHUNKS;
    const long long tiles = rows_max / PN_TILE;
    if (tiles < chunks) chunks = (int)(tiles > 0 ? tiles : 1);
    if ((size_t)chunks * 256 * 288 > PARTIAL_FLOATS) return PNERF_E_WS;
    constexpr size_t lds = (size_t)WX_UNITS * 16;
    if (hipFuncSetAttribute((const void *)k_wgrad_x0, hipFuncAttributeMaxDynamicSharedMemorySize, (int)lds) != hipSuccess) return PNERF_E_LAUNCH;
    { PnProfScope prof(PNK_WGRAD, s);
    hipLaunchKernelGGL(k_wgrad_x0, dim3(chunks), dim3(512), lds, s, A, g, d_tiles, partial); }
    PnProfScope prof(PNK_WGRAD_REDUCE, s);
    hipLaunchKernelGGL(k_wgrad_reduce_f16, dim3(pn_cdiv((long long)PN_H * 288, 64)), dim3(256), 0, s, partial, chunks, PN_H, PN_IN1, PN_ONES1, gscale, grad, (int)PO_W1, (int)PN_IN1, (int)PO_B1);
    PN_CHECK_LAUNCH();
    return 0;
}
}

size_t pn_wgrad_partials_bytes() { return pn_align(PARTIAL_FLOATS * sizeof(float)); }

namespace {
__global__ void k_zero_one_empty(const float *__restrict__ conf, const int *__restrict__ counters, long long slots_per_ray, const float *__restrict__ gs, float eps,
                                 float *__restrict__ g_conf) {
    const long long n_empty = (long long)counters[1] * slots_per_ray - (long long)counters[3];
    if (n_empty <= 0) return;
    const float g = PnZeroOne(conf[0], eps).grad(gs[0]);
    if (g != 0.f) atomicAdd(&g_conf[0], g * (float)n_empty);
}
}

int pn_agg_backward_launch(const pnerf_camera *cam, const pnerf_points *pts, const pnerf_step &st, const float *d_decoded, const float *d_weight,
                           const float *d_grad_decoded, const PnSaved &sv, float *d_grad_params, const pnerf_point_grads *pg,
                           float *d_partials, bool x0_saved, hipStream_t s) {
    const int K = st.K;
    const long long n_valid = st.n_valid_max;
    const PnArith ar = pn_arith();
    BwdArgs a;
    a.cam = *cam; a.params = st.params; a.packed = (const float4 *)st.packed_mlp; a.raydir = st.raydir;
    a.pidx = st.sample_pidx; a.valid_list = st.valid_list; a.counters = st.counters;
    a.SR = st.SR; a.K = K; a.TS = pn_tile_samples(K); a.cap_samples = n_valid;
    a.decoded = d_decoded; a.weight = d_weight; a.grad_decoded = d_grad_decoded; a.sv = sv;
    a.emb = pts->embedding;
    a.gparams = d_grad_params; a.g_emb = pg->embedding; a.g_conf = pg->conf; a.g_dir = pg->dir; a.g_color = pg->color;
    a.conf = pts->conf; a.zo_gs = x0_saved ? nullptr : pg->zero_one_gscale; a.zo_eps = pg->zero_one_eps;
    if (a.zo_gs && !a.conf) return PNERF_E_INVAL;
    if (!a.g_emb || !a.g_conf || !a.g_dir || !a.g_color) return PNERF_E_INVAL;
    BwdXArgs ax;
    ax.xyz = pts->xyz; ax.sample_loc = st.sample_loc; ax.g_xyz = pg->xyz;
    const bool xg = ax.g_xyz != nullptr;
    if (xg && x0_saved) return PNERF_E_UNSUP;
    if (xg && (!ax.xyz || !ax.sample_loc)) return PNERF_E_INVAL;
    const int ncu = pn_cu_count();
    if (!ncu) return PNERF_E_LAUNCH;
    const int grid_c = pn_capped_grid((n_valid + PN_CTILE - 1) / PN_CTILE, 3LL * ncu);
    const size_t lds_c = CB_BYTES, lds_a = xg ? BL_BYTES_X : BL_BYTES;
    const bool wg2 = sv.wg2 != 0;
    if (wg2) x0_saved = true;
    const bool mix = !wg2 && (ar.mix_mask() & 4);
    void (*const kcb)(BwdArgs) = wg2 ? k_color_backward<true> : k_color_backward<false>;
    void (*const kab)(BwdArgs) = wg2 ? k_agg_backward<true> : mix ? k_agg_backward<false, true> : k_agg_backward<false>;
    void (*const kax)(BwdXArgs) = wg2 ? k_agg_backward<true, false, true> : mix ? k_agg_backward<false, true, true> : k_agg_backward<false, false, true>;
    if (hipFuncSetAttribute(reinterpret_cast<const void *>(kcb), hipFuncAttributeMaxDynamicSharedMemorySize, (int)lds_c) != hipSuccess) return PNERF_E_LAUNCH;
    if (hipFuncSetAttribute(xg ? reinterpret_cast<const void *>(kax) : reinterpret_cast<const void *>(kab), hipFuncAttributeMaxDynamicSharedMemorySize, (int)lds_a) != hipSuccess) return PNERF_E_LAUNCH;
    a.cls_list = sv.cls_list; a.cls_info = sv.cls_info; a.valid_list = sv.cls_list;
    if (hipMemsetAsync(sv.gscale, 0, 4 * sizeof(unsigned), s) != hipSuccess) return PNERF_E_LAUNCH;
    hipLaunchKernelGGL(k_grad_max, dim3(pn_capped_grid((n_valid + 255) / 256, 1024)), dim3(256), 0, s, sv.cls_list, st.counters, n_valid, d_grad_decoded, sv.gscale);
    if (a.zo_gs) hipLaunchKernelGGL(k_zero_one_empty, dim3(1), dim3(1), 0, s, a.conf, st.counters, (long long)st.SR * K, a.zo_gs, a.zo_eps, a.g_conf);
    { PnProfScope prof(PNK_COLOR_BWD, s);
      hipLaunchKernelGGL(kcb, dim3(grid_c), dim3(256), lds_c, s, a); }
    int kc[PN_NCLS];
    const int ncls = pn_class_slots(K, kc);
    { PnProfScope prof(PNK_AGG_BWD, s);
      for (int j = 0; j < ncls; ++j) {
          a.cls = j; a.K = kc[j]; a.TS = pn_tile_samples(kc[j]);
          const int grid_a = pn_capped_grid((n_valid + a.TS - 1) / a.TS, 2LL * ncu);
          if (xg) { static_cast<BwdArgs &>(ax) = a; hipLaunchKernelGGL(kax, dim3(grid_a), dim3(PN_NTHR), lds_a, s, ax); }
          else hipLaunchKernelGGL(kab, dim3(grid_a), dim3(PN_NTHR), lds_a, s, a);
      } }
    PN_CHECK_LAUNCH();
    if (pg->ready_event && hipEventRecord((hipEvent_t)pg->ready_event, s) != hipSuccess) return PNERF_E_LAUNCH;
    const long long rows = sv.rows, smps = sv.samples;
    const int *dt = sv.cls_info + PN_CI_TILES, *ct = sv.cls_info + PN_CI_CTILES;
    const WgLayer layers[7] = {
        {WG_288x256, sv.dy1k, sv.x0k, sv.dy1m, sv.x0m, dt, rows, PO_W1, PN_IN1, PN_IN1, PN_ONES1, PO_B1},
        {WG_256x256, sv.dy2k, sv.h1k, sv.dy2m, sv.h1m, dt, rows, PO_W2, PN_H, PN_H, PN_H, PO_B2},
        {WG_288x256, sv.dy3k, sv.h2k, sv.dy3m, sv.h2m, dt, rows, PO_W3, PN_IN3, PN_IN3, PN_ONES3, PO_B3},
        {WG_256x256, sv.dy4k, sv.h3k, sv.dy4m, sv.h3m, dt, rows, PO_W4, PN_H, PN_H, PN_H, PO_B4},
        {WG_288x128, sv.dc1k, sv.xck, sv.dc1m, sv.xcm, ct, smps, PO_WC1, PN_INC, PN_INC, -1, 0},
        {WG_128x128, sv.dc2k, sv.c1k, sv.dc2m, sv.c1m, ct, smps, PO_WC2, PN_HC, PN_HC, -1, 0},
        {WG_128x128, sv.dc3k, sv.c2k, sv.dc3m, sv.c2m, ct, smps, PO_WC3, PN_HC, PN_HC, -1, 0},
    };
    for (const WgLayer &L : layers) {
        int rc;
        if (&L == layers && !x0_saved) {
            WgX0Args wa;
            wa.rmeta = sv.rmeta; wa.emb = pts->embedding; wa.x0t = sv.x0k; wa.n_points = pts->n;
            rc = launch_wgrad_x0(L.dy, wa, dt, rows, d_partials, sv.gscale, d_grad_params, s);
        } else {
            rc = wg2 ? launch_wgrad_layer<true>(L, d_partials, sv.gscale, d_grad_params, s) : launch_wgrad_layer<false>(L, d_partials, sv.gscale, d_grad_params, s);
        }
        if (rc) return rc;
    }
    return 0;
}

#ifdef PN_PHASE_TRACE
extern "C" int pnerf_debug_trace_bwd(void *host, size_t bytes) {
    return hipMemcpyFromSymbol(host, HIP_SYMBOL(pn_trace_bwd), bytes < sizeof(pn_trace_bwd) ? bytes : sizeof(pn_trace_bwd)) == hipSuccess ? 0 : -1;
}
#endif
```

pointnerf_amd/csrc/grid.hip:

```cpp
#include <limits.h>
#include "pn_common.h"

PnGridLayout pn_grid_layout(const pnerf_grid_params *gp, int n) {
    PnGridLayout L;
    L.G = (long long)gp->vdim[0] * gp->vdim[1] * gp->vdim[2];
    L.NB = (long long)pn_cdiv(gp->vdim[0], 4) * pn_cdiv(gp->vdim[1], 4) * pn_cdiv(gp->vdim[2], 4);
    const size_t np = (size_t)(n > 0 ? n : 1);
    size_t off = 0;
    auto take = [&](size_t bytes) { size_t o = off; off += pn_align(bytes); return o; };
    L.info = take(PNERF_GI_LEN * sizeof(int));
    L.bricks = take((size_t)L.NB * sizeof(uint4));
    L.occ = take((size_t)((L.G + 31) / 32) * sizeof(uint32_t));
    L.pts = take(np * sizeof(float4));
    L.ostart = take((np + 2) * sizeof(int));
    L.keys = take(np * sizeof(int));
    L.cnt = take((size_t)L.NB * 64 * sizeof(int));
    L.tmp_idx = take(np * sizeof(int));
    L.ocell = take((np + 1) * sizeof(int));
    L.bocc = take((size_t)(L.NB + 1) * sizeof(int));
    L.bpts = take((size_t)(L.NB + 1) * sizeof(int));
    L.brank = take((size_t)(L.NB + 1) * sizeof(int));
    L.bbase = take((size_t)(L.NB + 1) * sizeof(int));
    L.scan = take(pn_scan_scratch_ints(L.NB) * sizeof(int));
    L.total = off;
// ... 90 lines not shown
    int pre = c;
#pragma unroll
    for (int d = 1; d < 64; d <<= 1) { const int v = __shfl_up(pre, d, 64); if (lane >= d) pre += v; }
    if (c > 0) {
        const int o = rank0 + __popcll(bits & ((1ull << lane) - 1ull));
        const int st = base0 + pre - c;
        ostart[o] = st;
        ocell[o] = key;
        cnt[key] = st;
    }
}

__global__ __launch_bounds__(TPB) void k_grid_scatter(const int *__restrict__ keys, int n, int *__restrict__ cursor, int *__restrict__ tmp_idx) {
    int i = blockIdx.x * TPB + threadIdx.x;
    if (i >= n) return;
    int key = keys[i];
    if (key < 0) return;
    tmp_idx[atomicAdd(&cursor[key], 1)] = i;
}

__global__ __launch_bounds__(TPB) void k_grid_finalize(GP g, int n, const float *__restrict__ xyz, const int *__restrict__ ostart,
                                                       const int *__restrict__ ocell, int *__restrict__ tmp_idx,
                                                       float4 *__restrict__ pts, uint32_t *__restrict__ occ, const int *info) {
    const int o = blockIdx.x * TPB + threadIdx.x;
    if (o >= n || o >= info[PNERF_GI_N_OCC]) return;
    const int s = ostart[o], m = ostart[o + 1] - s;
    for (int a = 1; a < m; ++a) {
        int v = tmp_idx[s + a];
        int b = a - 1;
        while (b >= 0 && tmp_idx[s + b] > v) { tmp_idx[s + b + 1] = tmp_idx[s + b]; --b; }
        tmp_idx[s + b + 1] = v;
    }
    for (int a = 0; a < m; ++a) {
        int idx = tmp_idx[s + a];
        pts[s + a] = make_float4(xyz[3 * idx], xyz[3 * idx + 1], xyz[3 * idx + 2], __int_as_float(idx));
    }
    const int key = ocell[o], brick = key >> 6, local = key & 63;
    const int bzi = brick % g.bz, byi = (brick / g.bz) % g.by, bxi = brick / (g.bz * g.by);
    const int cx = bxi * 4 + (local >> 4), cy = byi * 4 + ((local >> 2) & 3), cz = bzi * 4 + (local & 3);
    int x0 = max(0, cx - g.qx / 2), x1 = min(g.gx, cx + (g.qx + 1) / 2);
    int y0 = max(0, cy - g.qy / 2), y1 = min(g.gy, cy + (g.qy + 1) / 2);
    int z0 = max(0, cz - g.qz / 2), z1 = min(g.gz, cz + (g.qz + 1) / 2);
    for (int x = x0; x < x1; ++x)
        for (int y = y0; y < y1; ++y)
            for (int z = z0; z < z1; ++z) {
                long long lin = (long long)x * (g.gy * g.gz) + (long long)y * g.gz + z;
                atomicOr(&occ[lin >> 5], 1u << (lin & 31));
            }
}
}

extern "C" size_t pnerf_grid_workspace_bytes(const pnerf_grid_params *gp, int n_points) {
    if (!gp) return 0;
    return pn_grid_layout(gp, n_points).total;
}

extern "C" int pnerf_grid_build(const pnerf_grid_params *gp, const float *d_xyz, int n, void *ws, size_t ws_bytes,
                                void *stream) {
    if (!gp || !ws || (n > 0 && !d_xyz) || n < 0) return PNERF_E_INVAL;
    for (int a = 0; a < 3; ++a)
        if (gp->vdim[a] <= 0 || !(gp->vsize[a] > 0.f) || gp->query_size[a] <= 0 || gp->kernel_size[a] <= 0) return PNERF_E_INVAL;
    PnGridLayout L = pn_grid_layout(gp, n);
    if (L.G <= 0 || L.G >= (1LL << 31) - 64 || L.NB * 64 >= (1LL << 31) - 64) return PNERF_E_UNSUP;
    if (ws_bytes < L.total) return PNERF_E_WS;
    hipStream_t s = (hipStream_t)stream;
    char *b = (char *)ws;
    int *info = (int *)(b + L.info), *ostart = (int *)(b + L.ostart), *keys = (int *)(b + L.keys), *cnt = (int *)(b + L.cnt);
    int *tmp_idx = (int *)(b + L.tmp_idx), *ocell = (int *)(b + L.ocell), *scan = (int *)(b + L.scan);
    int *bocc = (int *)(b + L.bocc), *bpts = (int *)(b + L.bpts), *brank = (int *)(b + L.brank), *bbase = (int *)(b + L.bbase);
    uint4 *bricks = (uint4 *)(b + L.bricks);
    uint32_t *occ = (uint32_t *)(b + L.occ);
    float4 *pts = (float4 *)(b + L.pts);
    GP g = {gp->ranges[0], gp->ranges[1], gp->ranges[2], gp->vsize[0], gp->vsize[1], gp->vsize[2],
            gp->vdim[0], gp->vdim[1], gp->vdim[2], gp->query_size[0], gp->query_size[1], gp->query_size[2],
            pn_cdiv(gp->vdim[1], 4), pn_cdiv(gp->vdim[2], 4)};

    PnProfScope prof(PNK_GRID, s);
    hipLaunchKernelGGL(k_grid_init, dim3(1), dim3(TPB), 0, s, info, (int)(L.ostart / 256));
    if (hipMemsetAsync(cnt, 0, (size_t)L.NB * 64 * sizeof(int), s) != hipSuccess) return PNERF_E_LAUNCH;
    if (hipMemsetAsync(occ, 0, (size_t)((L.G + 31) / 32) * sizeof(uint32_t), s) != hipSuccess) return PNERF_E_LAUNCH;
    if (n > 0) hipLaunchKernelGGL(k_grid_count, dim3(pn_cdiv(n, TPB)), dim3(TPB), 0, s, g, d_xyz, n, keys, cnt, info);
    hipLaunchKernelGGL(k_grid_cell0, dim3(1), dim3(1), 0, s, keys, n, info);
    const int nbw = (int)pn_cdiv(L.NB, TPB / 64);
    hipLaunchKernelGGL(k_brick_bits, dim3(nbw), dim3(TPB), 0, s, L.NB, cnt, bocc, bpts, info);
    int rc = pn_exclusive_scan_i32(bocc, brank, L.NB, scan, s);
    if (rc) return rc;
    rc = pn_exclusive_scan_i32(bpts, bbase, L.NB, scan, s);
    if (rc) return rc;
    hipLaunchKernelGGL(k_brick_fill, dim3(nbw), dim3(TPB), 0, s, L.NB, cnt, brank, bbase, bricks, ostart, ocell, info);
    if (n > 0) {
        hipLaunchKernelGGL(k_grid_scatter, dim3(pn_cdiv(n, TPB)), dim3(TPB), 0, s, keys, n, cnt, tmp_idx);
        hipLaunchKernelGGL(k_grid_finalize, dim3(pn_cdiv(n, TPB)), dim3(TPB), 0, s, g, n, d_xyz, ostart, ocell, tmp_idx, pts, occ, info);
    }
    PN_CHECK_LAUNCH();
    return 0;
}

extern "C" int pnerf_grid_info(const void *ws, int32_t *host_info, void *stream) {
    if (!ws || !host_info) return PNERF_E_INVAL;
    hipStream_t s = (hipStream_t)stream;
    if (hipMemcpyAsync(host_info, ws, PNERF_GI_LEN * sizeof(int), hipMemcpyDeviceToHost, s) != hipSuccess) return PNERF_E_LAUNCH;
    if (hipStreamSynchronize(s) != hipSuccess) return PNERF_E_LAUNCH;
    return 0;
}

namespace {
__device__ __forceinline__ unsigned pn_fkey(float f) { const unsigned b = __float_as_uint(f); return (b & 0x80000000u) ? ~b : (b | 0x80000000u); }
__device__ __forceinline__ float pn_fkey_inv(unsigned k) { return __uint_as_float((k & 0x80000000u) ? (k & 0x7fffffffu) : ~k); }
__global__ void k_minmax_init(unsigned *__restrict__ key) { if (threadIdx.x < 6) key[threadIdx.x] = threadIdx.x < 3 ? 0xffffffffu : 0u; }
__global__ __launch_bounds__(256) void k_minmax(const float *__restrict__ xyz, long long n, unsigned *__restrict__ key) {
    unsigned mn[3] = {0xffffffffu, 0xffffffffu, 0xffffffffu}, mx[3] = {0u, 0u, 0u};
    for (long long i = (long long)blockIdx.x * 256 + threadIdx.x; i < n; i += (long long)gridDim.x * 256) {
#pragma unroll
        for (int c = 0; c < 3; ++c) {
            const unsigned k = pn_fkey(xyz[3 * i + c]);
            mn[c] = min(mn[c], k); mx[c] = max(mx[c], k);
        }
    }
#pragma unroll
    for (int c = 0; c < 3; ++c) {
#pragma unroll
        for (int off = 32; off > 0; off >>= 1) { mn[c] = min(mn[c], __shfl_xor(mn[c], off, 64)); mx[c] = max(mx[c], __shfl_xor(mx[c], off, 64)); }
    }
    __shared__ unsigned red[4][6];
    if ((threadIdx.x & 63) == 0) {
#pragma unroll
        for (int c = 0; c < 3; ++c) { red[threadIdx.x >> 6][c] = mn[c]; red[threadIdx.x >> 6][3 + c] = mx[c]; }
    }
    __syncthreads();
    if (threadIdx.x < 6) {
        unsigned v = red[0][threadIdx.x];
        for (int w = 1; w < 4; ++w) v = threadIdx.x < 3 ? min(v, red[w][threadIdx.x]) : max(v, red[w][threadIdx.x]);
        if (threadIdx.x < 3) atomicMin(&key[threadIdx.x], v); else atomicMax(&key[threadIdx.x], v);
    }
}
__global__ void k_minmax_decode(unsigned *__restrict__ key) {
    if (threadIdx.x < 6) { const float f = pn_fkey_inv(key[threadIdx.x]); key[threadIdx.x] = __float_as_uint(f); }
}
}

extern "C" int pnerf_points_minmax(const float *d_xyz, int64_t n, float *d_out6, void *stream) {
    if (!d_xyz || !d_out6 || n <= 0) return PNERF_E_INVAL;
    hipStream_t s = (hipStream_t)stream;
    unsigned *key = reinterpret_cast<unsigned *>(d_out6);
    PnProfScope prof(PNK_GRID, s);
    hipLaunchKernelGGL(k_minmax_init, dim3(1), dim3(64), 0, s, key);
    const int blocks = (int)(n / 256 < 512 ? (n + 255) / 256 : 512);
    hipLaunchKernelGGL(k_minmax, dim3(blocks), dim3(256), 0, s, d_xyz, (long long)n, key);
    hipLaunchKernelGGL(k_minmax_decode, dim3(1), dim3(64), 0, s, key);
    PN_CHECK_LAUNCH();
    return 0;
}

extern "C" int pnerf_version(void) { return 1003; }
extern "C" const char *pnerf_arch(void) { return "gfx950"; }
```

pointnerf_amd/csrc/mlp_common.h:

```cpp
#pragma once
#include "pn_common.h"
#include <type_traits>
#include <utility>

#define PN_F      32
#define PN_IN1    284
#define PN_IN1P   288
#define PN_H      256
#define PN_IN3    263
#define PN_INC    280
#define PN_HC     128
#define PN_TILE   64
#define PN_MT     (PN_TILE / 32)
#define PN_NTHR   256
#define PN_NW     4
#define PN_NFB    2
static_assert(PN_NTHR == 64 * PN_NW && PN_NW == 4 && PN_NW * PN_NFB == 8, "the tile kernels are written for 4 waves x 2 of the 8 feature blocks each");
#define PN_TPR    (PN_NTHR / PN_TILE)
#define PN_EPT    (PN_F / PN_TPR)
#define PN_CTILE  64

enum : int {
    PO_W1 = 0, PO_B1 = PO_W1 + PN_H * PN_IN1, PO_W2 = PO_B1 + PN_H, PO_B2 = PO_W2 + PN_H * PN_H,
    PO_W3 = PO_B2 + PN_H, PO_B3 = PO_W3 + PN_H * PN_IN3, PO_W4 = PO_B3 + PN_H, PO_B4 = PO_W4 + PN_H * PN_H,
    PO_W5 = PO_B4 + PN_H, PO_B5 = PO_W5 + PN_H, PO_WC1 = PO_B5 + 1, PO_BC1 = PO_WC1 + PN_HC * PN_INC,
    PO_WC2 = PO_BC1 + PN_HC, PO_BC2 = PO_WC2 + PN_HC * PN_HC, PO_WC3 = PO_BC2 + PN_HC, PO_BC3 = PO_WC3 + PN_HC * PN_HC,
    PO_WC4 = PO_BC3 + PN_HC, PO_BC4 = PO_WC4 + 3 * PN_HC, PO_TOTAL = PO_BC4 + 3
};
static_assert(PO_TOTAL == 341764, "parameter count of the lego-script aggregator");

typedef float f32x16 __attribute__((ext_vector_type(16)));

typedef float pn_f4 __attribute__((ext_vector_type(4)));
typedef float pn_f2 __attribute__((ext_vector_type(2)));

__device__ __forceinline__ float pn_lrelu_grad(float post) { return post > 0.f ? 1.f : 0.01f; }

template <int... I, class F> __device__ __forceinline__ void pn_static_for_impl(std::integer_sequence<int, I...>, F &&f) { (f(std::integral_constant<int, I>{}), ...); }
template <int N, class F> __device__ __forceinline__ void pn_static_for(F &&f) { pn_static_for_impl(std::make_integer_sequence<int, N>{}, f); }

__device__ __forceinline__ void rot3(const float *M, float x, float y, float z, bool transpose, float &ox, float &oy, float &oz) {
    if (!transpose) { ox = x * M[0] + y * M[3] + z * M[6]; oy = x * M[1] + y * M[4] + z * M[7]; oz = x * M[2] + y * M[5] + z * M[8]; }
    else { ox = x * M[0] + y * M[1] + z * M[2]; oy = x * M[3] + y * M[4] + z * M[5]; oz = x * M[6] + y * M[7] + z * M[8]; }
}
template <int N> __device__ __forceinline__ float group_sum(float v) {
#pragma unroll
    for (int off = 1; off < N; off <<= 1) v += __shfl_xor(v, off, 64);
    return v;
}
template <int AF> __device__ __forceinline__ void pn_acc_zero(f32x16 (&acc)[AF][2]) {
#pragma unroll
    for (int i = 0; i < AF; ++i)
#pragma unroll
        for (int j = 0; j < 2; ++j)
#pragma unroll
            for (int r = 0; r < 16; ++r) acc[i][j][r] = 0.f;
}
__device__ __forceinline__ float pn_softplus(float x) {
#ifdef PN_EMU
    return x > 20.f ? x : log1pf(expf(x));
#else
    return x > 20.f ? x : __logf(1.0f + __expf(x));
#endif
}
__device__ __forceinline__ float pn_sigmoid(float x) {
#ifdef PN_EMU
    return x > 20.f ? 1.f : 1.0f / (1.0f + expf(-x));
#else
    return x > 20.f ? 1.f : __builtin_amdgcn_rcpf(1.0f + __expf(-x));
#endif
}

struct PnSaved {
    uint4 *x0k, *h1k, *h2k, *h3k;
    uint4 *dy1k, *dy2k, *dy3k, *dy4k;
    uint4 *h4r;
    float *arow;
    int4 *rmeta;
    unsigned *lmask;
    unsigned *gscale;
    float *fs, *dfs, *c3;
    uint4 *xck, *c1k, *c2k;
    uint4 *dc1k, *dc2k, *dc3k;
    unsigned *cmask;
    uint4 *x0m, *h1m, *h2m, *h3m, *dy1m, *dy2m, *dy3m, *dy4m;
    uint4 *xcm, *c1m, *c2m, *dc1m, *dc2m, *dc3m;
    int wg2;
    int *cls_list;
    int *cls_info;
    int *cls_tmp;
    long long rows, samples;
};
enum : int { PN_NCLS = 3, PN_CI_COUNT = 0, PN_CI_VBASE = 4, PN_CI_TBASE = 8, PN_CI_TILES = 12, PN_CI_CTILES = 13 , PN_CI_WORDS = 16 };
int pn_class_slots(int K, int kc[3]);
int pn_classify(const PnSaved &sv, const int32_t *d_valid_list, const int32_t *d_counters, const int32_t *d_pidx, int K, long long n_valid, bool train, bool save_x0, hipStream_t s);
size_t pn_saved_walk(void *base, long long n_valid, int K, PnSaved &s);
void pn_cls_walk(PnCarver &cv, PnSaved &s);
size_t pn_saved_bytes(long long n_valid, int K);
PnSaved pn_saved_carve(void *base, long long n_valid, int K);
int pn_agg_forward_launch(const pnerf_camera *cam, const pnerf_points *pts, const pnerf_step &st, float *d_decoded, float *d_weight,
                          const PnSaved &sv, bool train, bool save_x0, hipStream_t s);
int pn_agg_backward_launch(const pnerf_camera *cam, const pnerf_points *pts, const pnerf_step &st, const float *d_decoded, const float *d_weight,
                           const float *d_grad_decoded, const PnSaved &sv, float *d_grad_params, const pnerf_point_grads *pg,
                           float *d_partials, bool x0_saved, hipStream_t s);
size_t pn_wgrad_partials_bytes();
struct PnArith {
    int products;
    int wgrad_planes;
    int cross_terms;
    int mix_where;
    int mix_mask() const { return cross_terms == 8 ? mix_where : 0; }
};
PnArith pn_arith();

__host__ __device__ inline int pn_tile_samples(int K) { return PN_TILE / K; }
__device__ __forceinline__ unsigned pn_kinv(int K) { return (65536u + (unsigned)K - 1u) / (unsigned)K; }
__device__ __forceinline__ int pn_row_div(int row, unsigned kinv) { return (int)(((unsigned)row * kinv) >> 16); }


#ifdef PN_PHASE_TRACE
#define PN_TR_WGS   512
#define PN_TR_IT0   20
#define PN_TR_ITERS 6
#define PN_TR_SLOTS 24
#define PN_TR_DECL(name) __device__ unsigned long long name[PN_TR_WGS * PN_TR_ITERS * PN_TR_SLOTS]
#define PN_TR(buf, ph)                                                                                              \
    do {                                                                                                            \
        if (tid == 0 && blockIdx.x < PN_TR_WGS && titer >= PN_TR_IT0 && titer < PN_TR_IT0 + PN_TR_ITERS)           \
            buf[((size_t)blockIdx.x * PN_TR_ITERS + (titer - PN_TR_IT0)) * PN_TR_SLOTS + (ph)] = wall_clock64();    \
    } while (0)
#define PN_TR_HWID(buf)                                                                                             \
    do {                                                                                                            \
        if (tid == 0 && blockIdx.x < PN_TR_WGS && titer >= PN_TR_IT0 && titer < PN_TR_IT0 + PN_TR_ITERS)           \
            buf[((size_t)blockIdx.x * PN_TR_ITERS + (titer - PN_TR_IT0)) * PN_TR_SLOTS + PN_TR_SLOTS - 1] =         \
                (unsigned long long)__builtin_amdgcn_s_getreg((31 << 11) | 4) |                                    \
                ((unsigned long long)__builtin_amdgcn_s_getreg((31 << 11) | 20) << 32);                             \
    } while (0)
#define PN_TR_ITER_DECL int titer = -1
#define PN_TR_ITER_NEXT ++titer
#else
#define PN_TR(buf, ph)
#define PN_TR_HWID(buf)
#define PN_TR_ITER_DECL
#define PN_TR_ITER_NEXT
#endif
```

pointnerf_amd/ops.py:

```python
import ctypes
import math

import numpy as np
import torch

from . import _lib as L


def _stream():
    return ctypes.c_void_p(torch.cuda.current_stream().cuda_stream)


def _ptr(t):
    if t is None:
        return ctypes.c_void_p(0)
    assert t.is_cuda and t.is_contiguous(), "pointnerf_amd ops need contiguous device tensors"
    return ctypes.c_void_p(t.data_ptr())


def host_array(t):
    if not isinstance(t, torch.Tensor):
        return np.asarray(t)
    if not t.is_cuda:
        return t.detach().numpy()
# ... 396 lines not shown
                                      _ptr(fwd["saved"]), _ptr(grad_flat), ctypes.byref(pg), _ptr(ws), nws, _stream()), "pnerf_render_backward")


def agg_forward(cam, pts, st, train):
    f32 = dict(dtype=torch.float32, device=st._keep[0].device)
    decoded, weight = torch.empty(st.R, st.SR, 4, **f32), torch.empty(st.R, st.SR, st.K, **f32)
    saved, ws, nws = _forward_scratch(st.n_valid_max, st.K, train, f32["device"])
    L.check(L.lib().pnerf_agg_forward(ctypes.byref(cam), ctypes.byref(pts), ctypes.byref(st), _ptr(decoded), _ptr(weight),
                                      _ptr(saved), _ptr(ws), nws, _stream()), "pnerf_agg_forward")
    return dict(decoded=decoded, weight=weight, saved=saved)


def agg_backward(cam, pts, st, fwd, grad_decoded, grad_flat, grads):
    lib = L.lib()
    pg = _point_grads(grads)
    nws = lib.pnerf_render_backward_workspace_bytes(0, 1)
    ws = torch.empty(nws, dtype=torch.uint8, device=grad_flat.device)
    gd = grad_decoded.reshape(st.R, st.SR, 4).contiguous().float()
    L.check(lib.pnerf_agg_backward(ctypes.byref(cam), ctypes.byref(pts), ctypes.byref(st), _ptr(fwd["decoded"]), _ptr(fwd["weight"]), _ptr(gd),
                                   _ptr(fwd["saved"]), _ptr(grad_flat), ctypes.byref(pg), _ptr(ws), nws, _stream()), "pnerf_agg_backward")


class GatherRows(torch.autograd.Function):

    @staticmethod
    def forward(ctx, src, idx):
        _need_cuda(src, "src")
        s2 = src.detach().reshape(-1, src.shape[-1]).contiguous().float()
        i2 = idx.reshape(-1).contiguous().to(torch.int32)
        out = torch.empty(i2.numel(), s2.shape[1], dtype=torch.float32, device=src.device)
        L.check(L.lib().pnerf_gather_rows(_ptr(s2), s2.shape[0], s2.shape[1], _ptr(i2), i2.numel(), _ptr(out), _stream()),
                "pnerf_gather_rows")
        ctx.save_for_backward(i2)
        ctx.src_shape = tuple(src.shape)
        return out.view(tuple(idx.shape) + (s2.shape[1],))

    @staticmethod
    def backward(ctx, g):
        (i2,) = ctx.saved_tensors
        w = ctx.src_shape[-1]
        gs = torch.zeros(ctx.src_shape, dtype=torch.float32, device=g.device)
        g2 = g.reshape(-1, w).contiguous().float()
        n_src = gs.numel() // w
        L.check(L.lib().pnerf_scatter_add_rows(_ptr(g2), _ptr(i2), i2.numel(), w, _ptr(gs), n_src, _stream()),
                "pnerf_scatter_add_rows")
        return gs, None


def gather_rows(src, idx):
    return GatherRows.apply(src, idx)


def zero_one_sum(conf_flat, pidx, ray_hit, eps):
    lib = L.lib()
    R = 0 if ray_hit is None else int(pidx.shape[0])
    part = torch.empty(lib.pnerf_zero_one_blocks(pidx.numel() if ray_hit is None else R * 256), dtype=torch.float32, device=conf_flat.device)
    if ray_hit is None:
        L.check(lib.pnerf_zero_one_forward(_ptr(conf_flat), conf_flat.numel(), _ptr(pidx), pidx.numel(), float(eps), _ptr(part), _stream()), "pnerf_zero_one_forward")
    else:
        L.check(lib.pnerf_zero_one_forward_rays(_ptr(conf_flat), conf_flat.numel(), _ptr(pidx), _ptr(ray_hit), R, int(pidx.numel() // max(R, 1)), float(eps),
                                                _ptr(part), _stream()), "pnerf_zero_one_forward_rays")
    return part.sum()


def zero_one_add_grad(conf_flat, pidx, ray_hit, eps, gscale, grad_conf_flat):
    if ray_hit is None:
        L.check(L.lib().pnerf_zero_one_backward(_ptr(conf_flat), conf_flat.numel(), _ptr(pidx), pidx.numel(), float(eps), _ptr(gscale), _ptr(grad_conf_flat),
                                                _stream()), "pnerf_zero_one_backward")
    else:
        R = int(pidx.shape[0])
        L.check(L.lib().pnerf_zero_one_backward_rays(_ptr(conf_flat), conf_flat.numel(), _ptr(pidx), _ptr(ray_hit), R, int(pidx.numel() // max(R, 1)), float(eps),
                                                     _ptr(gscale), _ptr(grad_conf_flat), _stream()), "pnerf_zero_one_backward_rays")


class ZeroOneConf(torch.autograd.Function):

    @staticmethod
    def forward(ctx, conf, pidx, ray_hit, eps):
        c = conf.detach().reshape(-1)
        _need_cuda(c, "points_conf")
        ctx.save_for_backward(c, pidx, ray_hit)
        ctx.eps, ctx.shape = float(eps), conf.shape
        return zero_one_sum(c, pidx, ray_hit, eps)

    @staticmethod
    def backward(ctx, g):
        c, pidx, ray_hit = ctx.saved_tensors
        grad = torch.zeros_like(c)
        zero_one_add_grad(c, pidx, ray_hit, ctx.eps, g.detach().reshape(1).to(torch.float32).contiguous(), grad)
        return grad.view(ctx.shape), None, None, None


def zero_one_conf_sum(conf, pidx, eps):
    return ZeroOneConf.apply(conf, pidx.contiguous().reshape(-1), None, eps)


def zero_one_conf_sum_rays(conf, pidx_dense, ray_hit, eps):
    return ZeroOneConf.apply(conf, pidx_dense.contiguous(), ray_hit.contiguous(), eps)


class ColorLossRays(torch.autograd.Function):

    @staticmethod
    def forward(ctx, ray_color, gt, ray_hit):
        _need_cuda(ray_color, "ray_color")
        lib = L.lib()
        c, g = ray_color.detach().reshape(-1, 3).contiguous().float(), gt.detach().reshape(-1, 3).contiguous().float()
        R = c.shape[0]
        part = torch.empty(lib.pnerf_color_loss_blocks(R), dtype=torch.float32, device=c.device)
        L.check(lib.pnerf_color_loss_forward_rays(_ptr(c), _ptr(g), _ptr(ray_hit), R, _ptr(part), _stream()), "pnerf_color_loss_forward_rays")
        ctx.save_for_backward(c, g, ray_hit)
        ctx.shape = ray_color.shape
        return part.sum()

    @staticmethod
    def backward(ctx, gout):
        c, g, ray_hit = ctx.saved_tensors
        grad = torch.empty_like(c)
        gs = gout.detach().reshape(1).to(torch.float32).contiguous()
        L.check(L.lib().pnerf_color_loss_backward_rays(_ptr(c), _ptr(g), _ptr(ray_hit), c.shape[0], _ptr(gs), _ptr(grad), _stream()),
                "pnerf_color_loss_backward_rays")
        return grad.view(ctx.shape), None, None


def color_loss_sum_rays(ray_color, gt, ray_hit):
    return ColorLossRays.apply(ray_color, gt, ray_hit.contiguous())


def set_inference_products(n):
    old = L.lib().pnerf_set_inference_products(int(n))
    if old < 0:
        raise ValueError("inference products must be 2 or 3")
    return old


def set_wgrad_planes(n):
    old = L.lib().pnerf_set_wgrad_planes(int(n))
    if old < 0:
        raise ValueError("weight-gradient planes must be 1 or 2")
    ARENA._cap_cache = {}
    return old


def set_cross_terms(bits, where=None):
    old = L.lib().pnerf_set_cross_terms(int(bits))
    if old < 0:
        raise ValueError("cross terms must be 8 or 16")
    oldw = L.lib().pnerf_set_cross_terms_where(int(where)) if where is not None else None
    if where is not None and oldw < 0:
        raise ValueError("cross-term mask must be 0..7")
    return old, oldw


def arithmetic():
    out = (ctypes.c_int32 * 4)()
    L.check(L.lib().pnerf_get_arithmetic(out), "pnerf_get_arithmetic")
    return tuple(int(v) for v in out)


def cross_terms_state():
    _, _, bits, mask = arithmetic()
    return bits, (mask if bits == 8 else 0)


def image_metrics_sums(img, gt, win=11, data_range=2.0, quantize8=True):
    for name, t in (("img", img), ("gt", gt)):
        _need_cuda(t, name)
        if t.dtype != torch.float32:
            raise TypeError("pointnerf_amd: image_metrics needs float32 images, %s is %s" % (name, t.dtype))
        if t.dim() != 3 or t.shape[2] != 3:
            raise ValueError("pointnerf_amd: image_metrics needs [H, W, 3] images, %s is %s" % (name, list(t.shape)))
        if not t.is_contiguous():
            raise ValueError("pointnerf_amd: image_metrics needs contiguous images, %s has strides %s" % (name, list(t.stride())))
    if img.shape != gt.shape or img.device != gt.device:
        raise ValueError("pointnerf_amd: image_metrics: img %s on %s and gt %s on %s differ" % (list(img.shape), img.device, list(gt.shape), gt.device))
    H, W = int(img.shape[0]), int(img.shape[1])
    lib = L.lib()
    nbytes = lib.pnerf_image_metrics_workspace_bytes(H, W, int(win))
    ws = torch.empty(max(nbytes, 8), dtype=torch.uint8, device=img.device)
    out4 = torch.empty(4, dtype=torch.float64, device=img.device)
    L.check(lib.pnerf_image_metrics(_ptr(img.detach()), _ptr(gt.detach()), H, W, int(win), float(data_range), 1 if quantize8 else 0,
                                    _ptr(out4), _ptr(ws), nbytes, _stream()), "pnerf_image_metrics")
    return out4


def image_metrics(img, gt, win=11, data_range=2.0, quantize8=True):
    out4 = image_metrics_sums(img, gt, win, data_range, quantize8)
    H, W = int(img.shape[0]), int(img.shape[1])
    n_win = (H - int(win) + 1) * (W - int(win) + 1)
    return torch.stack([out4[0] / float(H * W * 3), out4[1:].sum() / float(3 * n_win)])


PROBE_RAY_KEYS = (("ray_max_shading_opacity", 1), ("ray_max_sample_loc_w", 3), ("ray_max_far_dist", 1), ("shading_avg_color", 3),
                  ("shading_avg_dir", 3), ("shading_avg_conf", 1), ("shading_avg_embedding", 32))


def probe_rays(pts, opacity, weight, sample_loc, sample_pidx, ray_hit, R, SR, K):
    R, SR, K = int(R), int(SR), int(K)
    f32, i32 = torch.float32, torch.int32
    _dense_arg(opacity, "opacity", f32, R * SR); _dense_arg(weight, "weight", f32, R * SR * K); _dense_arg(sample_loc, "sample_loc", f32, R * SR * 3)
    _dense_arg(sample_pidx, "sample_pidx", i32, R * SR * K); _dense_arg(ray_hit, "ray_hit", i32, R)
    out = {k: torch.empty(R, c, dtype=f32, device=opacity.device) for k, c in PROBE_RAY_KEYS}
    L.check(L.lib().pnerf_probe_rays(ctypes.byref(pts), _ptr(opacity), _ptr(weight), _ptr(sample_loc), _ptr(sample_pidx), _ptr(ray_hit), R, SR, K,
                                     *[_ptr(out[k]) for k, _ in PROBE_RAY_KEYS], _stream()), "pnerf_probe_rays")
    return out


def probe_hole_flags(ray_mask, max_opacity, far_dist, raycolor, gt, edge, bg, opacity_thresh, far_thresh=-1.0):
    H, W = int(edge.shape[0]), int(edge.shape[1])
    n = H * W
    _need_cuda(edge, "edge")
    if edge.dtype != torch.bool or not edge.is_contiguous() or edge.dim() != 2:
        raise ValueError("pointnerf_amd: edge must be a contiguous [H, W] bool tensor")
    _dense_arg(ray_mask, "ray_mask", torch.int8, n); _dense_arg(max_opacity, "max_opacity", torch.float32, n); _dense_arg(far_dist, "far_dist", torch.float32, n)
    _dense_arg(raycolor, "raycolor", torch.float32, n * 3); _dense_arg(gt, "gt", torch.float32, n * 3)
    bg3 = (ctypes.c_float * 3)(*[float(x) for x in np.asarray(host_array(bg), dtype=np.float64).reshape(-1)[:3]])
    flags = torch.empty(H, W, dtype=torch.int32, device=edge.device)
    L.check(L.lib().pnerf_probe_hole_mask(_ptr(ray_mask), _ptr(max_opacity), _ptr(far_dist), _ptr(raycolor), _ptr(gt), _ptr(edge.view(torch.uint8)), bg3,
                                          H, W, float(opacity_thresh), float(far_thresh), _ptr(flags), _stream()), "pnerf_probe_hole_mask")
    return flags


RAY_GEOMETRY_KEYS = ("acc", "depth_sum", "depth", "median_depth", "median_slot")


def ray_geometry(cam, sample_loc, sample_nn, ray_hit, opacity, blend_w):
    _need_cuda(sample_nn, "sample_nn")
    if sample_nn.dim() != 2:
        raise ValueError("pointnerf_amd: sample_nn must be [R, SR], got %s" % (list(sample_nn.shape),))
    R, SR = int(sample_nn.shape[0]), int(sample_nn.shape[1])
    f32, i32 = torch.float32, torch.int32
    _dense_arg(sample_loc, "sample_loc", f32, R * SR * 3); _dense_arg(sample_nn, "sample_nn", i32, R * SR); _dense_arg(ray_hit, "ray_hit", i32, R)
    _dense_arg(opacity, "opacity", f32, R * SR); _dense_arg(blend_w, "blend_w", f32, R * SR)
    dev = sample_nn.device
    for name, t in (("sample_loc", sample_loc), ("ray_hit", ray_hit), ("opacity", opacity), ("blend_w", blend_w)):
        if t.device != dev:
            raise ValueError("pointnerf_amd: %s is on %s, sample_nn on %s" % (name, t.device, dev))
    rows = torch.empty(4, R, dtype=f32, device=dev)
    out = {k: rows[i] for i, k in enumerate(RAY_GEOMETRY_KEYS[:4])}
    out["median_slot"] = torch.empty(R, dtype=i32, device=dev)
    L.check(L.lib().pnerf_ray_geometry(ctypes.byref(cam), _ptr(sample_loc), _ptr(sample_nn), _ptr(ray_hit), _ptr(opacity), _ptr(blend_w), R, SR,
                                       *[_ptr(out[k]) for k in RAY_GEOMETRY_KEYS], _stream()), "pnerf_ray_geometry")
    out["_rows"] = rows
    return out


def geometry_canvas(pixel_idx, ray_mask, depth, median_depth, acc, canvases, flag=None):
    _need_cuda(pixel_idx, "pixel_idx")
    n = int(pixel_idx.numel()) // 2
    if pixel_idx.dtype != torch.int32 or not pixel_idx.is_contiguous():
        pixel_idx = pixel_idx.to(torch.int32).contiguous()
    _dense_arg(pixel_idx, "pixel_idx", torch.int32, n * 2)
    if ray_mask is not None:
        _dense_arg(ray_mask, "ray_mask", torch.int8, n)
    f32 = torch.float32
    _dense_arg(depth, "depth", f32, n); _dense_arg(median_depth, "median_depth", f32, n); _dense_arg(acc, "acc", f32, n)
    if len(canvases) != 3 or canvases[0].dim() != 2:
        raise ValueError("pointnerf_amd: canvases must be three [H, W] tensors (depth, median_depth, acc)")
    H, W = int(canvases[0].shape[0]), int(canvases[0].shape[1])
    for name, t in zip(("depth canvas", "median_depth canvas", "acc canvas"), canvases):
        _dense_arg(t, name, f32, H * W)
    own = flag is None
    if own:
        flag = canvas_flag(pixel_idx.device)
    _dense_arg(flag, "flag", torch.int32, 1)
    L.check(L.lib().pnerf_geometry_canvas(_ptr(pixel_idx), _ptr(ray_mask), _ptr(depth), _ptr(median_depth), _ptr(acc), n, H, W,
                                          _ptr(canvases[0]), _ptr(canvases[1]), _ptr(canvases[2]), _ptr(flag), _stream()), "pnerf_geometry_canvas")
    if own:
        check_canvas_flag(flag)
    return flag


def canvas_flag(device):
    return torch.zeros(1, dtype=torch.int32, device=device)


def check_canvas_flag(flag):
    L.check(int(flag.cpu()[0]), "pnerf_geometry_canvas (a pixel_idx outside the canvas)")


def mfma_rate_tflops(mode=2, ms_target=60.0, device=None):
    import ctypes
    dev = torch.device("cuda", torch.cuda.current_device()) if device is None else device
    scratch = torch.zeros(256, dtype=torch.float32, device=dev)
    flop = ctypes.c_double(0.0)
    iters = max(int(ms_target / 1000.0 * 2.4e9 / (2 * 32 * 32)), 64)
    last = 0.0
    for _ in range(8):
        e0, e1 = torch.cuda.Event(enable_timing=True), torch.cuda.Event(enable_timing=True)
        e0.record()
        L.check(L.lib().pnerf_debug_mfma_rate(int(mode), int(iters), _ptr(scratch), ctypes.byref(flop), _stream()), "pnerf_debug_mfma_rate")
        e1.record()
        e1.synchronize()
        rate = flop.value / (e0.elapsed_time(e1) * 1e-3) / 1e12
        settled = last > 0.0 and abs(rate - last) <= 0.03 * last
        last = rate
        if settled:
            break
    return last


def prof_enable(on=True):
    L.lib().pnerf_prof_enable(1 if on else 0)


def prof_collect():
# ... 7 lines not shown
```

Measured before the change: 2.092 million.

## Replace static grid-stride tile loops with atomic dynamic tile claiming in aggregation kernels

The forward and backward aggregation kernels now hand out tiles dynamically. Each workgroup starts with a few statically assigned tiles, then claims later tiles through a global atomic counter and broadcasts the claimed index through LDS, keeping the one-ahead prefetch pipeline intact. The goal is to balance load across workgroups, since tile costs vary and the static grid-stride split leaves stragglers at the tail. The change adds a per-tile atomic and extra LDS traffic, enlarges the class-info and gscale buffers that hold the counters, and adds debug helpers for a grid cap and span tracing.

```diff
diff --git a/include/pnerf.h b/include/pnerf.h
--- a/include/pnerf.h
+++ b/include/pnerf.h
@@ -139,6 +139,7 @@
 int pnerf_set_cross_terms(int bits);
 int pnerf_set_cross_terms_where(int mask);
 int pnerf_get_arithmetic(int32_t out[4]);
+int pnerf_debug_set_tile_grid(int max_workgroups);
 
 int pnerf_render_backward(const pnerf_camera *cam, const pnerf_points *pts, const pnerf_step *step,
                           const float *d_decoded, const float *d_weight, const float *d_grad_ray_color,
diff --git a/pointnerf_amd/_lib.py b/pointnerf_amd/_lib.py
--- a/pointnerf_amd/_lib.py
+++ b/pointnerf_amd/_lib.py
@@ -8,7 +8,7 @@
 
 c_int, c_i64, c_f32, c_void_p, c_size_t = ctypes.c_int, ctypes.c_int64, ctypes.c_float, ctypes.c_void_p, ctypes.c_size_t
 
-ABI_VERSION = 1003
+ABI_VERSION = 1004
 PNERF_MAX_K = 16
 GI_N_IN_GRID, GI_N_OCC, GI_MAX_CNT, GI_CELL0, GI_FIRST_IDX, GI_LEN = 0, 1, 2, 3, 4, 8
 MLP_NTENSORS = 18
@@ -105,6 +105,7 @@
     "pnerf_set_cross_terms": (c_int, [c_int]),
     "pnerf_set_cross_terms_where": (c_int, [c_int]),
     "pnerf_get_arithmetic": (c_int, [ctypes.POINTER(ctypes.c_int32)]),
+    "pnerf_debug_set_tile_grid": (c_int, [c_int]),
     "pnerf_compact_workspace_bytes": (c_size_t, [c_i64]),
     "pnerf_touched_flags": (c_int, [c_void_p, c_i64, c_int, c_void_p, c_void_p]),
     "pnerf_compact_valid": (c_int, [c_void_p, c_i64, c_void_p, c_void_p, c_void_p, c_size_t, c_void_p]),
diff --git a/pointnerf_amd/csrc/aggregate.hip b/pointnerf_amd/csrc/aggregate.hip
--- a/pointnerf_amd/csrc/aggregate.hip
+++ b/pointnerf_amd/csrc/aggregate.hip
@@ -281,7 +281,7 @@
     s.h4r = cv.take<uint4>((size_t)s.rows * 32 * 2);
     s.arow = cv.take<float>((size_t)s.rows); s.rmeta = cv.take<int4>((size_t)s.rows);
     s.lmask = cv.take<unsigned>((size_t)tiles * 3 * 512);
-    s.gscale = cv.take<unsigned>(4);
+    s.gscale = cv.take<unsigned>(PN_GS_WORDS);
     s.fs = cv.take<float>((size_t)s.samples * PN_H); s.dfs = cv.take<float>((size_t)s.samples * PN_H);
     s.c3 = cv.take<float>((size_t)s.samples * PN_HC);
     cplanes(s.xck, s.c1k, s.c2k, s.dc1k, s.dc2k, s.dc3k);
@@ -413,7 +413,7 @@
 
 namespace {
 
-constexpr int FL_EX = PN_XBYTES, FL_W5 = FL_EX + PN_TILE * 8 * 4, FL_ROW = FL_W5 + PN_H * 4, FL_BYTES = FL_ROW + 4 * PN_TILE * 4;
+constexpr int FL_EX = PN_XBYTES, FL_W5 = FL_EX + PN_TILE * 8 * 4, FL_ROW = FL_W5 + PN_H * 4, FL_CLAIM = FL_ROW + 4 * PN_TILE * 4 , FL_BYTES = FL_CLAIM + 16;
 static_assert(2 * FL_BYTES <= 160 * 1024, "two forward workgroups must fit the 160 KB LDS");
 
 struct FGather {
@@ -663,6 +663,7 @@
 
 #ifdef PN_PHASE_TRACE
 PN_TR_DECL(pn_trace_fwd);
+PN_TR_SPAN_DECL(pn_span_fwd);
 #endif
 template <bool TRAIN, bool PERS, int NP, bool WG2 = false, bool FRAMES = false>
 __global__ __launch_bounds__(PN_NTHR, PN_NW / 2) void k_agg_forward(typename FwdArgsOf<FRAMES>::type a) {
@@ -691,16 +692,19 @@
     const char *img = reinterpret_cast<const char *>(a.packed);
     if (tid0 < PN_H) w5s[tid0] = P[PO_W5 + tid0];
     const float b5 = P[PO_B5];
-    const long long stride = gridDim.x, tile_first = blockIdx.x, tile_last = ntiles;
-    if (tile_first >= tile_last) return;
-
-    long long tile = tile_first;
+    const int tile_last = (int)ntiles, grid = gridDim.x;
+    int t0 = blockIdx.x, t1 = t0 + grid, t2 = t1 + grid;
+    if (t0 >= tile_last) return;
+    int *claim_ctr = a.sv.cls_info + PN_CI_CLAIM + a.cls, *claim_w = reinterpret_cast<int *>(smem_f + FL_CLAIM);
+    int nclaim = 0;
+
+    long long tile = t0;
     int si0, si1, si2, p0, p1;
     FGather G;
     {
         const int row = tid0 / PN_TPR, q = tid0 % PN_TPR, k = row - pn_row_div(row, kinv) * K;
-        si0 = f_sample_of(a, tile, row, Ns, kinv); si1 = tile + stride < tile_last ? f_sample_of(a, tile + stride, row, Ns, kinv) : -1;
-        si2 = tile + 2 * stride < tile_last ? f_sample_of(a, tile + 2 * stride, row, Ns, kinv) : -1;
+        si0 = f_sample_of(a, tile, row, Ns, kinv); si1 = t1 < tile_last ? f_sample_of(a, t1, row, Ns, kinv) : -1;
+        si2 = t2 < tile_last ? f_sample_of(a, t2, row, Ns, kinv) : -1;
         p0 = si0 >= 0 ? a.pidx[(long long)si0 * a.Kstride + k] : -1;
         p1 = si1 >= 0 ? a.pidx[(long long)si1 * a.Kstride + k] : -1;
         f_gather<PERS, FRAMES>(a, G, si0, p0, q, frames);
@@ -708,15 +712,16 @@
 
     f32x16 acc[PN_NFB][2];
     PN_TR_ITER_DECL;
-    for (; tile < tile_last; tile += stride) {
+    for (bool first = true; t0 < tile_last; first = false) {
         PN_TR_ITER_NEXT;
+        tile = t0;
         int tid = threadIdx.x;
         asm volatile("" : "+v"(tid));
         const int lane = tid & 63, wave = __builtin_amdgcn_readfirstlane(tid >> 6);
         const int row = tid / PN_TPR, q = tid % PN_TPR, k = row - pn_row_div(row, kinv) * K;
         const long long gtile = tb + tile;
         PN_LDS_BARRIER();
-        PN_TR(pn_trace_fwd, 0); PN_TR_HWID(pn_trace_fwd);
+        PN_TR(pn_trace_fwd, 0); PN_TR_HWID(pn_trace_fwd); PN_TR_SPAN(pn_span_fwd, a.cls, 0);
         f_build<PERS, MIX, FRAMES>(a, G, X, exb, wraw, sidx, si0, p0, row, q);
         f_acc_bias(P + PO_B1, wave, lane, acc);
         PnTileW<MIX, 2, 8, NP> W1;
@@ -800,10 +805,14 @@
             else pn_copy_out_kmajor<PN_H, WG2>(X, a.sv.h3k, gtile * 8, tid, a.sv.h3m);
         }
         PN_TR(pn_trace_fwd, 12);
+        const int t3 = first ? t2 + grid : pn_claim_tile(PN_CLAIM_STATIC_FWD, grid, __builtin_amdgcn_readfirstlane(*claim_w), nclaim - 1);
+        const bool claims = nclaim % PN_CLAIM_TILES == 0;
+        int claimed = 0;
+        if (tid == 0 && claims) claimed = atomicAdd(claim_ctr, 1);
         const int si_next = si1, p_next = p1;
-        if (tile + stride < tile_last) f_gather<PERS, FRAMES>(a, G, si1, p1, q, frames);
+        if (t1 < tile_last) f_gather<PERS, FRAMES>(a, G, si1, p1, q, frames);
         const int p2 = si2 >= 0 ? a.pidx[(long long)si2 * a.Kstride + k] : -1;
-        const int si3 = tile + 3 * stride < tile_last ? f_sample_of(a, tile + 3 * stride, row, Ns, kinv) : -1;
+        const int si3 = t3 < tile_last ? f_sample_of(a, t3, row, Ns, kinv) : -1;
         PN_LDS_BARRIER();
         PN_TR(pn_trace_fwd, 13);
         f_epilogue<false>(acc, X, wave, lane, mask);
@@ -846,7 +855,9 @@
         }
         }
         si0 = si_next; p0 = p_next; si1 = si2; p1 = p2; si2 = si3;
-        PN_TR(pn_trace_fwd, 16);
+        if (tid == 0 && claims) *claim_w = claimed;
+        t0 = t1; t1 = t2; t2 = t3; ++nclaim;
+        PN_TR(pn_trace_fwd, 16); PN_TR_SPAN(pn_span_fwd, a.cls, 1);
     }
 }
 
@@ -1008,6 +1019,14 @@
 extern "C" int pnerf_set_wgrad_planes(int n) { return pn_arith_set(&PnArith::wgrad_planes, n, n == 1 || n == 2); }
 extern "C" int pnerf_set_cross_terms(int bits) { return pn_arith_set(&PnArith::cross_terms, bits, bits == 8 || bits == 16); }
 extern "C" int pnerf_set_cross_terms_where(int mask) { return pn_arith_set(&PnArith::mix_where, mask, mask >= 0 && mask <= 7); }
+static int pn_tile_grid_cap = 0;
+int pn_tile_grid(long long tiles, long long dflt) { return pn_capped_grid(tiles, pn_tile_grid_cap > 0 && pn_tile_grid_cap < dflt ? pn_tile_grid_cap : dflt); }
+extern "C" int pnerf_debug_set_tile_grid(int max_workgroups) {
+    if (max_workgroups < 0) return PNERF_E_INVAL;
+    const int old = pn_tile_grid_cap;
+    pn_tile_grid_cap = max_workgroups;
+    return old;
+}
 extern "C" int pnerf_get_arithmetic(int32_t out[4]) {
     if (!out) return PNERF_E_INVAL;
     const PnArith a = pn_arith();
@@ -1035,7 +1054,7 @@
     if (frames && train) return PNERF_E_INVAL;
     const int ncu = pn_cu_count();
     if (!ncu) return PNERF_E_LAUNCH;
-    const int grid_c = pn_capped_grid((cap_samples + PN_CTILE - 1) / PN_CTILE, 2LL * ncu);
+    const int grid_c = pn_tile_grid((cap_samples + PN_CTILE - 1) / PN_CTILE, 2LL * ncu);
     const size_t lds_a = FL_BYTES, lds_c = CL_BYTES;
     const bool pers = st.xyz_pers != nullptr;
     const bool np2 = !train && ar.products == 2;
@@ -1063,7 +1082,7 @@
         PnProfScope prof(PNK_AGG_FWD, s);
         for (int j = 0; j < ncls; ++j) {
             a.cls = j; a.K = kc[j]; a.TS = pn_tile_samples(kc[j]);
-            const int grid_a = pn_capped_grid((cap_samples + a.TS - 1) / a.TS, 2LL * ncu);
+            const int grid_a = pn_tile_grid((cap_samples + a.TS - 1) / a.TS, 2LL * ncu);
             if (frames) { FwdArgsF af; static_cast<FwdArgs &>(af) = a; af.frames = pts->frames; hipLaunchKernelGGL(kfnf, dim3(grid_a), dim3(PN_NTHR), lds_a, s, af); }
             else hipLaunchKernelGGL(kfn, dim3(grid_a), dim3(PN_NTHR), lds_a, s, a);
         }
@@ -1082,4 +1101,7 @@
 extern "C" int pnerf_debug_trace_fwd(void *host, size_t bytes) {
     return hipMemcpyFromSymbol(host, HIP_SYMBOL(pn_trace_fwd), bytes < sizeof(pn_trace_fwd) ? bytes : sizeof(pn_trace_fwd)) == hipSuccess ? 0 : -1;
 }
+extern "C" int pnerf_debug_span_fwd(void *host, size_t bytes) {
+    return hipMemcpyFromSymbol(host, HIP_SYMBOL(pn_span_fwd), bytes < sizeof(pn_span_fwd) ? bytes : sizeof(pn_span_fwd)) == hipSuccess ? 0 : -1;
+}
 #endif
diff --git a/pointnerf_amd/csrc/backward.hip b/pointnerf_amd/csrc/backward.hip
--- a/pointnerf_amd/csrc/backward.hip
+++ b/pointnerf_amd/csrc/backward.hip
@@ -293,7 +293,7 @@
     }
 }
 
-constexpr int BL_ROW = PN_XBYTES, BL_RSC = BL_ROW + 10 * PN_TILE * 4, BL_W5 = BL_RSC + PN_RSC_BYTES, BL_BYTES = BL_W5 + PN_H * 4;
+constexpr int BL_ROW = PN_XBYTES, BL_RSC = BL_ROW + 10 * PN_TILE * 4, BL_W5 = BL_RSC + PN_RSC_BYTES, BL_CLAIM = BL_W5 + PN_H * 4 , BL_BYTES = BL_CLAIM + 16;
 constexpr int LDDX = 228;
 static_assert(2 * BL_BYTES <= 160 * 1024, "two backward workgroups must fit the 160 KB LDS");
 static_assert(PN_TILE * LDDX * 4 <= PN_XBYTES, "d X0 tile");
@@ -372,7 +372,9 @@
                 const float x = xrow[r], dotf = pd[0] * rs.S(r);
                 const float alpha = pn_softplus(x), sg = pn_sigmoid(x);
                 const int rp = prow[r];
-                if (rp >= 0) atomicAdd(&a.g_conf[rp], (dsg[r] * alpha + dotf) * wnrm[r] * rs.inv(r) + (a.zo_gs ? PnZeroOne(zo_conf, a.zo_eps).grad(a.zo_gs[0]) : 0.f));
+                float zo_eps = a.zo_eps;
+                asm volatile("" : "+s"(zo_eps));
+                if (rp >= 0) atomicAdd(&a.g_conf[rp], (dsg[r] * alpha + dotf) * wnrm[r] * rs.inv(r) + (a.zo_gs ? PnZeroOne(zo_conf, zo_eps).grad(a.zo_gs[0]) : 0.f));
                 if (XG && rp >= 0) gw = dsg[r] * alpha + dotf;
                 dr = dsg[r] * wrow[r] * sg;
             }
@@ -464,6 +466,7 @@
 
 #ifdef PN_PHASE_TRACE
 PN_TR_DECL(pn_trace_bwd);
+PN_TR_SPAN_DECL(pn_span_bwd);
 #endif
 template <bool WG2, bool MIX = false, bool XYZG = false>
 __global__ __launch_bounds__(PN_NTHR, PN_NW / 2) void k_agg_backward(typename BwdArgsOf<XYZG>::T a) {
@@ -494,7 +497,13 @@
     float gw5[8] = {0.f, 0.f, 0.f, 0.f, 0.f, 0.f, 0.f, 0.f};
     float gb5t = 0.f;
     f32x16 acc[PN_NFB][2];
-    const long long stride = gridDim.x, tile_first = blockIdx.x, tile_last = ntiles;
+    constexpr bool CLAIM = !(XYZG && !MIX);
+    using tile_t = std::conditional_t<CLAIM, int, long long>;
+    const tile_t tile_first = blockIdx.x, tile_last = (tile_t)ntiles, grid = gridDim.x;
+    tile_t t_cur = tile_first;
+    [[maybe_unused]] tile_t t_nxt = t_cur + grid;
+    int nclaim = 0;
+    int *claim_ctr = reinterpret_cast<int *>(a.sv.gscale) + PN_GS_CLAIM + a.cls, *claim_w = reinterpret_cast<int *>(smem_b + BL_CLAIM);
     int4 rm_cur = make_int4(-1, -1, 0, 0);
     float ar_cur = 0.f;
     if (tid0 < PN_TILE && tile_first < tile_last) {
@@ -502,15 +511,16 @@
         ar_cur = a.sv.arow[(tb + tile_first) * PN_TILE + tid0];
     }
     PN_TR_ITER_DECL;
-    for (long long tile = tile_first; tile < tile_last; tile += stride) {
+    for (; t_cur < tile_last; ++nclaim) {
         PN_TR_ITER_NEXT;
+        const long long tile = t_cur;
         int tid = threadIdx.x;
         asm volatile("" : "+v"(tid));
         const int lane = tid & 63, wave = __builtin_amdgcn_readfirstlane(tid >> 6);
         const int row = tid / PN_TPR, q = tid % PN_TPR;
         const long long gtile = tb + tile;
         PN_LDS_BARRIER();
-        PN_TR(pn_trace_bwd, 0); PN_TR_HWID(pn_trace_bwd);
+        PN_TR(pn_trace_bwd, 0); PN_TR_HWID(pn_trace_bwd); PN_TR_SPAN(pn_span_bwd, a.cls, 0);
         unsigned m1[PN_NFB], m2[PN_NFB], m3[PN_NFB];
 #pragma unroll
         for (int fb = 0; fb < PN_NFB; ++fb) {
@@ -532,9 +542,16 @@
         }
         int4 rm_nxt = make_int4(-1, -1, 0, 0);
         float ar_nxt = 0.f;
-        if (tid < PN_TILE && tile + stride < tile_last) {
-            rm_nxt = a.sv.rmeta[(gtile + stride) * PN_TILE + tid];
-            ar_nxt = a.sv.arow[(gtile + stride) * PN_TILE + tid];
+        if constexpr (CLAIM) {
+            if (tid < PN_TILE && t_nxt < tile_last) {
+                rm_nxt = a.sv.rmeta[(tb + t_nxt) * PN_TILE + tid];
+                ar_nxt = a.sv.arow[(tb + t_nxt) * PN_TILE + tid];
+            }
+        } else {
+            if (tid < PN_TILE && tile + grid < tile_last) {
+                rm_nxt = a.sv.rmeta[(gtile + grid) * PN_TILE + tid];
+                ar_nxt = a.sv.arow[(gtile + grid) * PN_TILE + tid];
+            }
         }
         __builtin_amdgcn_sched_barrier(0);
         if (tid < PN_TILE) {
@@ -563,6 +580,9 @@
         rm_cur = rm_nxt; ar_cur = ar_nxt;
         PN_LDS_BARRIER();
         PN_TR(pn_trace_bwd, 1);
+        [[maybe_unused]] const bool claims = nclaim % PN_CLAIM_TILES == 0;
+        [[maybe_unused]] int claimed = 0;
+        if constexpr (CLAIM) { if (tid == 0 && claims) claimed = atomicAdd(claim_ctr, 1); }
         const int rp = prow[row];
         float4 e0 = make_float4(0.f, 0.f, 0.f, 0.f), e1 = e0;
         if (rp >= 0) {
@@ -579,8 +599,13 @@
         }
         PnTileW<MIX, 0, 8> W4;
         W4.prefetch(img, PKH_D4, PKM_D4, PN_NFB * wave, lane);
+        if constexpr (CLAIM) { if (tid == 0 && claims) *claim_w = claimed; }
         PN_LDS_BARRIER();
         PN_TR(pn_trace_bwd, 3);
+        if constexpr (CLAIM) {
+            t_cur = t_nxt;
+            t_nxt = pn_claim_tile(PN_CLAIM_STATIC_BWD, grid, __builtin_amdgcn_readfirstlane(*claim_w), nclaim);
+        }
         pn_acc_zero(acc);
         PN_TR(pn_trace_bwd, 4);
         W4.run(X, lane, acc);
@@ -743,7 +768,8 @@
             if (p >= 0) atomicAdd(&a.g_emb[(long long)p * PN_F + col], dx[r * LDX + col]);
         }
         if constexpr (XYZG) b_xyz_row(a, dx + row * LDX, gwf, wrow, wnrm, sidx, rp, row, q, K, kinv, rs.inv(row));
-        PN_TR(pn_trace_bwd, 16);
+        if constexpr (!CLAIM) t_cur += grid;
+        PN_TR(pn_trace_bwd, 16); PN_TR_SPAN(pn_span_bwd, a.cls, 1);
     }
     if (tile_first >= tile_last) return;
     {
@@ -1225,7 +1251,7 @@
     if (xg && (!ax.xyz || !ax.sample_loc)) return PNERF_E_INVAL;
     const int ncu = pn_cu_count();
     if (!ncu) return PNERF_E_LAUNCH;
-    const int grid_c = pn_capped_grid((n_valid + PN_CTILE - 1) / PN_CTILE, 3LL * ncu);
+    const int grid_c = pn_tile_grid((n_valid + PN_CTILE - 1) / PN_CTILE, 3LL * ncu);
     const size_t lds_c = CB_BYTES, lds_a = xg ? BL_BYTES_X : BL_BYTES;
     const bool wg2 = sv.wg2 != 0;
     if (wg2) x0_saved = true;
@@ -1236,7 +1262,7 @@
     if (hipFuncSetAttribute(reinterpret_cast<const void *>(kcb), hipFuncAttributeMaxDynamicSharedMemorySize, (int)lds_c) != hipSuccess) return PNERF_E_LAUNCH;
     if (hipFuncSetAttribute(xg ? reinterpret_cast<const void *>(kax) : reinterpret_cast<const void *>(kab), hipFuncAttributeMaxDynamicSharedMemorySize, (int)lds_a) != hipSuccess) return PNERF_E_LAUNCH;
     a.cls_list = sv.cls_list; a.cls_info = sv.cls_info; a.valid_list = sv.cls_list;
-    if (hipMemsetAsync(sv.gscale, 0, 4 * sizeof(unsigned), s) != hipSuccess) return PNERF_E_LAUNCH;
+    if (hipMemsetAsync(sv.gscale, 0, PN_GS_WORDS * sizeof(unsigned), s) != hipSuccess) return PNERF_E_LAUNCH;
     hipLaunchKernelGGL(k_grad_max, dim3(pn_capped_grid((n_valid + 255) / 256, 1024)), dim3(256), 0, s, sv.cls_list, st.counters, n_valid, d_grad_decoded, sv.gscale);
     if (a.zo_gs) hipLaunchKernelGGL(k_zero_one_empty, dim3(1), dim3(1), 0, s, a.conf, st.counters, (long long)st.SR * K, a.zo_gs, a.zo_eps, a.g_conf);
     { PnProfScope prof(PNK_COLOR_BWD, s);
@@ -1246,7 +1272,7 @@
     { PnProfScope prof(PNK_AGG_BWD, s);
       for (int j = 0; j < ncls; ++j) {
           a.cls = j; a.K = kc[j]; a.TS = pn_tile_samples(kc[j]);
-          const int grid_a = pn_capped_grid((n_valid + a.TS - 1) / a.TS, 2LL * ncu);
+          const int grid_a = pn_tile_grid((n_valid + a.TS - 1) / a.TS, 2LL * ncu);
           if (xg) { static_cast<BwdArgs &>(ax) = a; hipLaunchKernelGGL(kax, dim3(grid_a), dim3(PN_NTHR), lds_a, s, ax); }
           else hipLaunchKernelGGL(kab, dim3(grid_a), dim3(PN_NTHR), lds_a, s, a);
       } }
@@ -1281,4 +1307,7 @@
 extern "C" int pnerf_debug_trace_bwd(void *host, size_t bytes) {
     return hipMemcpyFromSymbol(host, HIP_SYMBOL(pn_trace_bwd), bytes < sizeof(pn_trace_bwd) ? bytes : sizeof(pn_trace_bwd)) == hipSuccess ? 0 : -1;
 }
+extern "C" int pnerf_debug_span_bwd(void *host, size_t bytes) {
+    return hipMemcpyFromSymbol(host, HIP_SYMBOL(pn_span_bwd), bytes < sizeof(pn_span_bwd) ? bytes : sizeof(pn_span_bwd)) == hipSuccess ? 0 : -1;
+}
 #endif
diff --git a/pointnerf_amd/csrc/grid.hip b/pointnerf_amd/csrc/grid.hip
--- a/pointnerf_amd/csrc/grid.hip
+++ b/pointnerf_amd/csrc/grid.hip
@@ -266,5 +266,5 @@
     return 0;
 }
 
-extern "C" int pnerf_version(void) { return 1003; }
+extern "C" int pnerf_version(void) { return 1004; }
 extern "C" const char *pnerf_arch(void) { return "gfx950"; }
diff --git a/pointnerf_amd/csrc/mlp_common.h b/pointnerf_amd/csrc/mlp_common.h
--- a/pointnerf_amd/csrc/mlp_common.h
+++ b/pointnerf_amd/csrc/mlp_common.h
@@ -91,7 +91,14 @@
     int *cls_tmp;
     long long rows, samples;
 };
-enum : int { PN_NCLS = 3, PN_CI_COUNT = 0, PN_CI_VBASE = 4, PN_CI_TBASE = 8, PN_CI_TILES = 12, PN_CI_CTILES = 13 , PN_CI_WORDS = 16 };
+enum : int { PN_NCLS = 3, PN_CI_COUNT = 0, PN_CI_VBASE = 4, PN_CI_TBASE = 8, PN_CI_TILES = 12, PN_CI_CTILES = 13 ,
+              PN_CI_CLAIM = 16 , PN_CI_WORDS = 20 };
+#ifndef PN_CLAIM_TILES
+#define PN_CLAIM_TILES 1
+#endif
+enum : int { PN_CLAIM_STATIC_FWD = 4, PN_CLAIM_STATIC_BWD = 2, PN_GS_CLAIM = 4, PN_GS_WORDS = 8 };
+__device__ __forceinline__ int pn_claim_tile(int nstatic, int grid, int v, int m) { return nstatic * grid + v * PN_CLAIM_TILES + m % PN_CLAIM_TILES; }
+int pn_tile_grid(long long tiles, long long dflt);
 int pn_class_slots(int K, int kc[3]);
 int pn_classify(const PnSaved &sv, const int32_t *d_valid_list, const int32_t *d_counters, const int32_t *d_pidx, int K, long long n_valid, bool train, bool save_x0, hipStream_t s);
 size_t pn_saved_walk(void *base, long long n_valid, int K, PnSaved &s);
@@ -138,9 +145,18 @@
     } while (0)
 #define PN_TR_ITER_DECL int titer = -1
 #define PN_TR_ITER_NEXT ++titer
+#define PN_TR_SPAN_DECL(name) __device__ unsigned long long name[PN_TR_WGS * 4]
+#define PN_TR_SPAN(buf, cls, end)                                                                                   \
+    do {                                                                                                            \
+        if (tid == 0 && (cls) == 0 && blockIdx.x < PN_TR_WGS && ((end) || titer == 0)) {                            \
+            buf[(size_t)blockIdx.x * 4 + (end)] = wall_clock64();                                                   \
+            if (end) buf[(size_t)blockIdx.x * 4 + 2] = (unsigned long long)(titer + 1);                             \
+        }                                                                                                           \
+    } while (0)
 #else
 #define PN_TR(buf, ph)
 #define PN_TR_HWID(buf)
 #define PN_TR_ITER_DECL
 #define PN_TR_ITER_NEXT
+#define PN_TR_SPAN(buf, cls, end)
 #endif
diff --git a/pointnerf_amd/ops.py b/pointnerf_amd/ops.py
--- a/pointnerf_amd/ops.py
+++ b/pointnerf_amd/ops.py
@@ -572,6 +572,13 @@
     return old, oldw
 
 
+def set_tile_grid(max_workgroups=0):
+    old = L.lib().pnerf_debug_set_tile_grid(int(max_workgroups))
+    if old < 0:
+        raise ValueError("the grid cap must be >= 0")
+    return old
+
+
 def arithmetic():
     out = (ctypes.c_int32 * 4)()
     L.check(L.lib().pnerf_get_arithmetic(out), "pnerf_get_arithmetic")
```

After: 2.168 million, median of 6. 1.04x the previous value.
